# ViTAE-Transformer/MTP

Hardware: AMD Instinct MI355X
Metric: images/sec pretrain step (ViT-L+RVSA, 224^2, bf16) (higher is better)
Workload: dtype bf16; 1 GPU; ViT-L + RVSA backbone fwd+bwd + grad all-reduce + clip + AdamW, 224x224, batch 64 per GPU (BASELINE configs[2]/[3]); global_batch=64, parallelism=dp1, activation_checkpointing=False, heads=sum_i mean(f_i)

## Files before the change

### include/mtp_hip.h

```cpp
#ifndef MTP_HIP_H_
#define MTP_HIP_H_

#include <stddef.h>
#include <stdint.h>

#ifdef __cplusplus
extern "C" {
#endif

typedef void* mtp_stream_t;

typedef enum { MTP_F32 = 0, MTP_BF16 = 1, MTP_F64 = 2  } mtp_dtype;

enum { MTP_OK = 0, MTP_ERR_ARG = -1, MTP_ERR_UNSUPPORTED = -2 };

typedef enum {
    MTP_EPI_BIAS = 0,
    MTP_EPI_BIAS_GELU = 1,
    MTP_EPI_BIAS_RES = 2,
    MTP_EPI_DGELU = 3,
    MTP_EPI_BIAS_GELU_DG = 4,
    MTP_EPI_MUL = 5
} mtp_epilogue;

// ... 66 lines not shown
int mtp_preprocess_patchify(const uint8_t* img, void* cols, int dtype, int64_t B, int64_t H, int64_t W, int64_t P, int64_t pad_divisor,
                            const float* mean, const float* std, int bgr_to_rgb, float pad_value, mtp_stream_t stream);
int mtp_cast(const void* src, int src_dtype, void* dst, int dst_dtype, int64_t n, mtp_stream_t stream);
int mtp_transpose_cast(const float* src, void* dst, int dst_dtype, int64_t R, int64_t C, mtp_stream_t stream);
typedef struct {
    const float* src;
    void* w;
    void* wt;
    int64_t R, C;
    int64_t tile0;
    int32_t f32_out;
    float wd;
} mtp_wimg_desc;
int mtp_weight_images(const mtp_wimg_desc* descs_dev, int n, int64_t total_tiles, int act_dtype, mtp_stream_t stream);
int mtp_adamw_weight_images(const mtp_wimg_desc* descs_dev, int n, int64_t total_tiles, int act_dtype, float* p_base, const float* g_base, float* m_base, float* v_base,
                            const float* hyper, const float* sqnorm, float max_norm, float grad_scale, mtp_stream_t stream);
int mtp_adamw_weight_images_lr(const mtp_wimg_desc* descs_dev, const float* desc_lr, int n, int64_t total_tiles, int act_dtype, float* p_base, const float* g_base,
                               float* m_base, float* v_base, const float* hyper, const float* sqnorm, float max_norm, float grad_scale, mtp_stream_t stream);
int mtp_convt_pack(const float* w, void* wg, void* wgT, int dtype, int64_t Cin, int64_t Cout, mtp_stream_t stream);
int mtp_convt_unpack_grad(const float* dwg, float* dw, int64_t Cin, int64_t Cout, mtp_stream_t stream);
int mtp_tokens_to_nchw(const void* x, int x_dtype, void* out, int out_dtype, int64_t B, int64_t Hp, int64_t Wp, int64_t C, int levels, mtp_stream_t stream);
int mtp_nchw_to_tokens(const void* f, int f_dtype, void* out, int out_dtype, int64_t B, int64_t Hp, int64_t Wp, int64_t C, int levels, mtp_stream_t stream);
int mtp_maxpool2_tokens_fwd(const float* x, void* y, int y_dtype, int64_t B, int64_t Hp, int64_t Wp, int64_t C, mtp_stream_t stream);
int mtp_maxpool2_tokens_bwd(const float* x, const void* dy, int dy_dtype, float* dx, int accumulate, int64_t B, int64_t Hp, int64_t Wp, int64_t C, mtp_stream_t stream);
int mtp_axpy_f32(float* y, const float* x, float alpha, int64_t n, mtp_stream_t stream);
#define MTP_MAX_SEGMENTS 12
int mtp_copy_segments_f32(const float* const* src, float* const* dst, const int64_t* count, int n, mtp_stream_t stream);
int mtp_scale_rows_cast(const float* src, void* dst, int dst_dtype, const float* scale, int64_t rows_per_sample, int64_t rows, int64_t C, mtp_stream_t stream);

int mtp_im2col3x3(const void* x, int x_dtype, int64_t sN, int64_t sH, int64_t sW, int64_t sC, void* cols, int cols_dtype,
                  int64_t N, int64_t H, int64_t W, int64_t Cin, int64_t stride, int64_t Kp, mtp_stream_t stream);
int mtp_col2im3x3(const void* dcols, int cols_dtype, float* dx, int64_t sN, int64_t sH, int64_t sW, int64_t sC,
                  int64_t N, int64_t H, int64_t W, int64_t Cin, int64_t stride, int64_t Kp, int accumulate, mtp_stream_t stream);
int mtp_conv3x3_pack(const float* w, void* w2, void* w2t, int dtype, int64_t Cout, int64_t Cin, int64_t Kp, mtp_stream_t stream);
int mtp_conv3x3_unpack_grad(const float* dw2, float* dw, int64_t Cout, int64_t Cin, int64_t Kp, mtp_stream_t stream);
int mtp_pack_rows_padded(const float* w, void* wp, void* wpt, int dtype, int64_t R, int64_t C, int64_t Rp, mtp_stream_t stream);
int mtp_cast_pad_rows(const float* src, int64_t n, void* dst, int dst_dtype, int64_t ld, int64_t rows, mtp_stream_t stream);
int mtp_copy_rows(const void* src, int64_t src_ld, void* dst, int64_t dst_ld, int dtype, int64_t n, int64_t rows, mtp_stream_t stream);
int mtp_dwconv3x3_fwd(const void* x, const float* w, const float* bias, void* y, int dtype, int64_t N, int64_t H, int64_t W, int64_t C, mtp_stream_t stream);
int mtp_dwconv3x3_bwd_dx(const void* dy, int dtype, const float* w, float* dx, int accumulate, int64_t N, int64_t H, int64_t W, int64_t C, mtp_stream_t stream);
int64_t mtp_dwconv3x3_bwd_dw_partial_rows(int64_t N, int64_t H, int64_t W);
int mtp_dwconv3x3_bwd_dw(const void* dy, const void* x, int dtype, float* part, int64_t N, int64_t H, int64_t W, int64_t C, mtp_stream_t stream);
int mtp_dwconv_fwd(const void* x, const float* w, const float* bias, void* y, int dtype, int64_t N, int64_t H, int64_t W, int64_t C, int k, mtp_stream_t stream);
int mtp_dwconv_bwd_dx(const void* dy, int dtype, const float* w, float* dx, int accumulate, int64_t N, int64_t H, int64_t W, int64_t C, int k, mtp_stream_t stream);
int mtp_dwconv_bwd_dw(const void* dy, const void* x, int dtype, float* dw, float* db, int64_t N, int64_t H, int64_t W, int64_t C, int k, mtp_stream_t stream);
int mtp_center_feature_scale_fwd(const void* y, const void* xp, const void* logits, int64_t ld, void* out, int dtype, int64_t rows, int64_t G, int64_t GC, mtp_stream_t stream);
int mtp_center_feature_scale_bwd(const void* dout, const void* y, const void* xp, const void* logits, int64_t ld, void* dy, float* dxp, void* dlogits, int dtype, int64_t rows,
                                 int64_t G, int64_t GC, mtp_stream_t stream);
int mtp_softmax_groups_fwd(const void* logits, int64_t ld, void* prob, int dtype, int64_t rows, int64_t G, int64_t P, mtp_stream_t stream);
int mtp_softmax_groups_bwd(const void* prob, const float* dprob, void* dlogits, int64_t ld, int dtype, int64_t rows, int64_t G, int64_t P, mtp_stream_t stream);
int mtp_scale_residual_fwd(const float* x, const void* z, int dtype, const float* gamma, const float* sample_scale, int64_t rows_per_sample,
                           float* out, void* out_act, int64_t rows, int64_t C, mtp_stream_t stream);
int64_t mtp_scale_residual_bwd_partial_rows(int64_t rows);
int mtp_scale_residual_bwd(const float* dout, const void* z, int dtype, const float* gamma, const float* sample_scale, int64_t rows_per_sample,
                           void* dz, float* part, int64_t rows, int64_t C, mtp_stream_t stream);

int mtp_full_attn_fwd(const void* qkv, void* o, float* lse, int dtype, const float* rel_h, const float* rel_w,
                      int64_t B, int64_t Hp, int64_t Wp, int64_t heads, int64_t hd, float scale, mtp_stream_t stream);
int64_t mtp_full_attn_bwd_workspace_floats(int64_t B, int64_t Hp, int64_t Wp, int64_t heads);
int mtp_full_attn_bwd(const void* qkv, const void* o, const void* dout, const float* lse, void* dqkv, int dtype,
                      const float* rel_h, const float* rel_w, float* drel_part, float* workspace,
                      int64_t B, int64_t Hp, int64_t Wp, int64_t heads, int64_t hd, float scale, mtp_stream_t stream);

int mtp_rvsa_pool_fwd(const void* x, int dtype, float* avg, float* pooled, int64_t B, int64_t Hp, int64_t Wp, int64_t C, mtp_stream_t stream);
int mtp_rvsa_pool_bwd(const float* dpooled, const float* avg, void* dx, int dtype, int accumulate, int64_t B, int64_t Hp, int64_t Wp, int64_t C, mtp_stream_t stream);
int mtp_rvsa_sampling_fwd(const void* x, int dtype, const float* w, const float* bias, float* avg, float* pooled, float* samp,
                          int64_t B, int64_t Hp, int64_t Wp, int64_t C, int64_t N, mtp_stream_t stream);
int mtp_rvsa_sampling_bwd(const float* dsamp, const float* w, const float* avg, void* dx, int dtype,
                          int64_t B, int64_t Hp, int64_t Wp, int64_t C, int64_t N, mtp_stream_t stream);
int mtp_rvsa_sampling_bwd_win(const float* dsamp, const float* w, const float* avg, float* g, int64_t windows, int64_t C, int64_t N, mtp_stream_t stream);
int mtp_small_linear_fwd(const float* x, const float* w, const float* b, float* y, int64_t R, int64_t N, int64_t K, mtp_stream_t stream);
int mtp_small_linear_bwd(const float* x, const float* w, const float* dy, float* dx, float* dw, float* db, int64_t R, int64_t N, int64_t K, mtp_stream_t stream);
int mtp_small_linear_dw_segments(const float* x, const float* dy, int64_t R, int64_t N, int64_t K, int nseg, const int64_t* seg_rows,
                                 float* const* dw, float* const* db, mtp_stream_t stream);
int mtp_small_linear_dw_segments_batched(const float* const* xs, const float* const* dys, int count, int64_t R, int64_t N, int64_t K, int nseg,
                                         const int64_t* seg_rows, float* const* dw, float* const* db, mtp_stream_t stream);
int mtp_rvsa_attn_fwd(const void* qkv, const float* samp, void* o, float* lse, int dtype,
                      const float* rel_h, const float* rel_w, const float* bias_table,
                      int64_t B, int64_t Hp, int64_t Wp, int64_t heads, int64_t hd, float scale, mtp_stream_t stream);
int mtp_rvsa_attn_bwd(const void* qkv, const float* samp, const void* o, const void* dout, const float* lse,
                      void* dqkv, float* dkv_f32, float* dsamp, float* rel_part, float* tab_part, int dtype,
                      const float* rel_h, const float* rel_w, const float* bias_table,
                      int64_t B, int64_t Hp, int64_t Wp, int64_t heads, int64_t hd, float scale, mtp_stream_t stream);

int mtp_zero_segments_f32(float* base, const int64_t* start, const int64_t* count, int n, mtp_stream_t stream);
int mtp_sqnorm_f32(const float* g, float* out, int64_t n, mtp_stream_t stream);
int mtp_sqnorm_segments_f32(const float* base, const int64_t* start, const int64_t* count, int n, float* out, mtp_stream_t stream);
int mtp_adamw_flat(float* p, const float* g, float* m, float* v, int64_t n, const int64_t* seg_start, const float* seg_wd, int nseg,
                   const float* hyper, const float* sqnorm, float max_norm, float grad_scale, mtp_stream_t stream);
int mtp_adamw_flat_lr(float* p, const float* g, float* m, float* v, int64_t n, const int64_t* seg_start, const float* seg_wd, const float* seg_lr, int nseg,
                      const float* hyper, const float* sqnorm, float max_norm, float grad_scale, mtp_stream_t stream);

typedef struct {
    int64_t N, H, W;
    int kernel_h, kernel_w, stride_h, stride_w, pad_h, pad_w, dilation_h, dilation_w;
    int group, group_channels;
    float offset_scale;
    int im2col_step;
    int remove_center;
    int variant;
} mtp_dcnv3_geom;
int mtp_dcnv3_out_size(const mtp_dcnv3_geom* geom, int64_t* Ho, int64_t* Wo);
int mtp_dcnv3_fwd(const void* input, const void* offset, const void* mask, void* output, int dtype, const mtp_dcnv3_geom* geom, mtp_stream_t stream);
int mtp_dcnv3_bwd(const void* input, const void* offset, const void* mask, const void* grad_output, int dtype, float* grad_input, float* grad_offset,
                  float* grad_mask, const mtp_dcnv3_geom* geom, mtp_stream_t stream);
int mtp_dcnv3_bwd_act(const void* input, const void* offset, const void* mask, const void* grad_output, int dtype, float* grad_input, float* grad_offset,
                      float* grad_mask, void* grad_offset_act, int64_t act_ld, const mtp_dcnv3_geom* geom, mtp_stream_t stream);

const char* mtp_version(void);

int mtp_stream_create_low_priority(mtp_stream_t* stream);
int mtp_stream_create_cu_mask(const uint32_t* mask, int words, mtp_stream_t* stream);
int mtp_probe_placement(int32_t* out, int blocks, int64_t spin_clocks, mtp_stream_t stream);
int mtp_stream_destroy(mtp_stream_t stream);

int mtp_comm_unique_id(void* id128);
int mtp_comm_init(const void* id128, int rank, int world, void** comm);
int mtp_comm_allreduce_bucket(void* comm, float* bucket, int64_t count, mtp_stream_t stream);
int mtp_comm_allreduce_bucket_dt(void* comm, void* bucket, int64_t count, int dtype, mtp_stream_t stream);
int mtp_comm_reduce_scatter_bucket(void* comm, void* bucket, int64_t count_per_rank, int rank, int dtype, mtp_stream_t stream);
int mtp_comm_allgather_bucket(void* comm, void* bucket, int64_t count_per_rank, int rank, int dtype, mtp_stream_t stream);
int mtp_comm_info(void* comm, int* info4);
int mtp_comm_destroy(void* comm);

int64_t mtp_bn_partial_rows(int64_t rows);
int mtp_bn_stats(const void* x, int dtype, int64_t ldx, const float* center, float* part, float* sums, int64_t rows, int64_t C, mtp_stream_t stream);
int mtp_bn_finalize(const float* sums, const float* center, double count, float* running_mean, float* running_var, float momentum, float eps, float* mean, float* rstd,
                    int64_t C, mtp_stream_t stream);
int mtp_bn_apply(const void* x, int x_dtype, int64_t ldx, const float* mean, const float* rstd, const float* gamma, const float* beta, int relu,
                 void* y, int y_dtype, int64_t ldy, int64_t rows, int64_t C, mtp_stream_t stream);
int mtp_bn_bwd_stats(const void* dy, int dy_dtype, int64_t lddy, const void* x, int x_dtype, int64_t ldx, const float* mean, const float* rstd,
                     const float* gamma, const float* beta, int relu, float* part, float* sums, int64_t rows, int64_t C, mtp_stream_t stream);
int mtp_bn_bwd_dx(const void* dy, int dy_dtype, int64_t lddy, const void* x, int x_dtype, int64_t ldx, const float* mean, const float* rstd,
                  const float* gamma, const float* beta, int relu, const float* sums, double count, void* dx, int dx_dtype, int64_t lddx,
                  int64_t rows, int64_t C, mtp_stream_t stream);
int mtp_resize_bilinear_fwd(const void* x, int x_dtype, int64_t ldx, void* y, int y_dtype, int64_t ldy, int64_t N, int64_t Hi, int64_t Wi,
                            int64_t Ho, int64_t Wo, int64_t C, int accumulate, mtp_stream_t stream);
int mtp_resize_bilinear_bwd(const void* dy, int dy_dtype, int64_t lddy, float* dx, int64_t lddx, int64_t N, int64_t Hi, int64_t Wi, int64_t Ho,
                            int64_t Wo, int64_t C, int accumulate, mtp_stream_t stream);
int mtp_adaptive_avg_pool_fwd(const void* x, int x_dtype, int64_t ldx, void* y, int y_dtype, int64_t N, int64_t H, int64_t W, int64_t C,
                              int64_t S, mtp_stream_t stream);
int mtp_adaptive_avg_pool_bwd(const void* dy, int dy_dtype, float* dx, int64_t lddx, int64_t N, int64_t H, int64_t W, int64_t C, int64_t S,
                              int accumulate, mtp_stream_t stream);
int mtp_channel_scale(const void* x, int x_dtype, int64_t ldx, const float* mask, int64_t rows_per_sample, void* y, int y_dtype, int64_t ldy,
                      int64_t rows, int64_t C, mtp_stream_t stream);
int64_t mtp_seg_ce_workspace_bytes(int64_t N, int64_t H, int64_t W, int64_t K);
int mtp_seg_ce(const void* logits, int dtype, int64_t ld, int64_t N, int64_t h, int64_t w, int64_t K, const void* labels, int label_bytes, int64_t H,
               int64_t W, int ignore_index, float loss_weight, float* loss, float* dlogits, int64_t ldd, void* workspace, int64_t workspace_bytes,
               mtp_stream_t stream);

#ifdef __cplusplus
}
#endif
#endif
```

### mtp_amd/_lib.py

```python
import ctypes as C
import os

_HERE = os.path.dirname(os.path.abspath(__file__))
LIB_PATH = os.environ.get("MTP_HIP_LIB") or os.path.join(_HERE, "libmtp_hip.so")

MTP_F32, MTP_BF16, MTP_F64 = 0, 1, 2
EPI_BIAS, EPI_BIAS_GELU, EPI_BIAS_RES, EPI_DGELU, EPI_BIAS_GELU_DG, EPI_MUL = 0, 1, 2, 3, 4, 5

p, i64, i32, f32 = C.c_void_p, C.c_int64, C.c_int, C.c_float


class GemmArgs(C.Structure):
    _fields_ = [("A", p), ("B", p), ("C", p), ("M", i64), ("N", i64), ("K", i64),
                ("lda", i64), ("ldb", i64), ("ldc", i64),
                ("in_dtype", i32), ("out_dtype", i32), ("epilogue", i32),
                ("bias", p), ("bias_mod", i64), ("res", p), ("res_ld", i64), ("res_mod", i64),
                ("rowscale", p), ("rows_per_sample", i64), ("aux", p), ("aux_ld", i64),
                ("split_k", i32), ("variant", i32), ("colsum", p), ("defer_sum", i32), ("pad_", i32),
                ("workspace", p), ("workspace_bytes", i64)]


class WimgDesc(C.Structure):
    _fields_ = [("src", p), ("w", p), ("wt", p), ("R", i64), ("C", i64), ("tile0", i64), ("f32_out", C.c_int32), ("wd", C.c_float)]

# ... 5 lines not shown


SIGNATURES = {
    "mtp_weight_images": (i32, [p, i32, i64, i32, p]),
    "mtp_dwconv_fwd": (i32, [p, p, p, p, i32, i64, i64, i64, i64, i32, p]),
    "mtp_dwconv_bwd_dx": (i32, [p, i32, p, p, i32, i64, i64, i64, i64, i32, p]),
    "mtp_dwconv_bwd_dw": (i32, [p, p, i32, p, p, i64, i64, i64, i64, i32, p]),
    "mtp_center_feature_scale_fwd": (i32, [p, p, p, i64, p, i32, i64, i64, i64, p]),
    "mtp_center_feature_scale_bwd": (i32, [p, p, p, p, i64, p, p, p, i32, i64, i64, i64, p]),
    "mtp_dcnv3_out_size": (i32, [C.POINTER(Dcnv3Geom), C.POINTER(i64), C.POINTER(i64)]),
    "mtp_dcnv3_fwd": (i32, [p, p, p, p, i32, C.POINTER(Dcnv3Geom), p]),
    "mtp_dcnv3_bwd": (i32, [p, p, p, p, i32, p, p, p, C.POINTER(Dcnv3Geom), p]),
    "mtp_dcnv3_bwd_act": (i32, [p, p, p, p, i32, p, p, p, p, i64, C.POINTER(Dcnv3Geom), p]),
    "mtp_gemm_nt": (i32, [C.POINTER(GemmArgs), p]),
    "mtp_gemm_nt_tile": (i32, [C.POINTER(GemmArgs)]),
    "mtp_gemm_nt_workspace_bytes": (i64, []),
    "mtp_gemm_tn": (i32, [C.POINTER(GemmArgs), p]),
    "mtp_gemm_tn_grouped": (i32, [C.POINTER(GemmArgs), i32, p]),
    "mtp_sum_partials_batch": (i32, [p, p, p, p, i32, p]),
    "mtp_layernorm_fwd": (i32, [p, i32, p, p, p, i32, p, p, i64, i64, f32, i32, p]),
    "mtp_layernorm_bwd_partial_rows": (i64, [i64]),
    "mtp_layernorm_bwd": (i32, [p, i32, p, i32, p, p, p, p, i32, p, p, p, i32, p, i32, p, i64, p, p, i64, i64, i64, p]),
    "mtp_reduce_rows_f32": (i32, [p, i64, p, i64, i64, i32, p]),
    "mtp_reduce_rows_batched_f32": (i32, [p, p, i32, i64, i64, i64, i32, p]),
    "mtp_reduce_rows_t_f32": (i32, [p, i64, p, i64, i64, i64, i32, p]),
    "mtp_reduce_rows_t_batched_f32": (i32, [p, p, i32, i64, i64, i64, i64, i32, p]),
    "mtp_copy_segments_f32": (i32, [p, p, p, i32, p]),
    "mtp_colsum": (i32, [p, i32, i64, p, i64, i64, p]),
    "mtp_colsum_acc": (i32, [p, i32, i64, p, i64, i64, p]),
    "mtp_patchify": (i32, [p, p, i32, i64, i64, i64, i64, i64, p]),
    "mtp_preprocess_patchify": (i32, [p, p, i32, i64, i64, i64, i64, i64, C.POINTER(f32), C.POINTER(f32), i32, f32, p]),
    "mtp_unpatchify": (i32, [p, i32, p, i64, i64, i64, i64, i64, p]),
    "mtp_cast": (i32, [p, i32, p, i32, i64, p]),
    "mtp_transpose_cast": (i32, [p, p, i32, i64, i64, p]),
    "mtp_convt_pack": (i32, [p, p, p, i32, i64, i64, p]),
    "mtp_convt_unpack_grad": (i32, [p, p, i64, i64, p]),
    "mtp_tokens_to_nchw": (i32, [p, i32, p, i32, i64, i64, i64, i64, i32, p]),
    "mtp_nchw_to_tokens": (i32, [p, i32, p, i32, i64, i64, i64, i64, i32, p]),
    "mtp_maxpool2_tokens_fwd": (i32, [p, p, i32, i64, i64, i64, i64, p]),
    "mtp_maxpool2_tokens_bwd": (i32, [p, p, i32, p, i32, i64, i64, i64, i64, p]),
    "mtp_axpy_f32": (i32, [p, p, f32, i64, p]),
    "mtp_scale_rows_cast": (i32, [p, p, i32, p, i64, i64, i64, p]),
    "mtp_im2col3x3": (i32, [p, i32, i64, i64, i64, i64, p, i32, i64, i64, i64, i64, i64, i64, p]),
    "mtp_col2im3x3": (i32, [p, i32, p, i64, i64, i64, i64, i64, i64, i64, i64, i64, i64, i32, p]),
    "mtp_conv3x3_pack": (i32, [p, p, p, i32, i64, i64, i64, p]),
    "mtp_conv3x3_unpack_grad": (i32, [p, p, i64, i64, i64, p]),
    "mtp_pack_rows_padded": (i32, [p, p, p, i32, i64, i64, i64, p]),
    "mtp_cast_pad_rows": (i32, [p, i64, p, i32, i64, i64, p]),
    "mtp_copy_rows": (i32, [p, i64, p, i64, i32, i64, i64, p]),
    "mtp_dwconv3x3_fwd": (i32, [p, p, p, p, i32, i64, i64, i64, i64, p]),
    "mtp_dwconv3x3_bwd_dx": (i32, [p, i32, p, p, i32, i64, i64, i64, i64, p]),
    "mtp_dwconv3x3_bwd_dw_partial_rows": (i64, [i64, i64, i64]),
    "mtp_dwconv3x3_bwd_dw": (i32, [p, p, i32, p, i64, i64, i64, i64, p]),
    "mtp_softmax_groups_fwd": (i32, [p, i64, p, i32, i64, i64, i64, p]),
    "mtp_softmax_groups_bwd": (i32, [p, p, p, i64, i32, i64, i64, i64, p]),
    "mtp_scale_residual_fwd": (i32, [p, p, i32, p, p, i64, p, p, i64, i64, p]),
    "mtp_scale_residual_bwd_partial_rows": (i64, [i64]),
    "mtp_scale_residual_bwd": (i32, [p, p, i32, p, p, i64, p, p, i64, i64, p]),
    "mtp_comm_unique_id": (i32, [p]),
    "mtp_comm_init": (i32, [p, i32, i32, C.POINTER(C.c_void_p)]),
    "mtp_comm_allreduce_bucket": (i32, [p, p, i64, p]),
    "mtp_comm_allreduce_bucket_dt": (i32, [p, p, i64, i32, p]),
    "mtp_comm_reduce_scatter_bucket": (i32, [p, p, i64, i32, i32, p]),
    "mtp_comm_allgather_bucket": (i32, [p, p, i64, i32, i32, p]),
    "mtp_comm_info": (i32, [p, p]),
    "mtp_comm_destroy": (i32, [p]),
    "mtp_full_attn_fwd": (i32, [p, p, p, i32, p, p, i64, i64, i64, i64, i64, f32, p]),
    "mtp_full_attn_bwd_workspace_floats": (i64, [i64, i64, i64, i64]),
    "mtp_full_attn_bwd": (i32, [p, p, p, p, p, i32, p, p, p, p, i64, i64, i64, i64, i64, f32, p]),
    "mtp_rvsa_pool_fwd": (i32, [p, i32, p, p, i64, i64, i64, i64, p]),
    "mtp_rvsa_pool_bwd": (i32, [p, p, p, i32, i32, i64, i64, i64, i64, p]),
    "mtp_rvsa_sampling_fwd": (i32, [p, i32, p, p, p, p, p, i64, i64, i64, i64, i64, p]),
    "mtp_rvsa_sampling_bwd": (i32, [p, p, p, p, i32, i64, i64, i64, i64, i64, p]),
    "mtp_rvsa_sampling_bwd_win": (i32, [p, p, p, p, i64, i64, i64, p]),
    "mtp_layernorm_residual_fwd": (i32, [p, i32, p, p, p, p, p, i64, p, p, p, p, i64, i64, f32, p]),
    "mtp_layernorm_residual_bwd": (i32, [p, p, i32, p, p, p, p, p, p, i64, p, p, i64, i64, p]),
    "mtp_layernorm_bwd_win": (i32, [p, i32, p, i32, p, p, p, p, p, p, i32, p, i32, p, i64, p, p, i64, i64, i64, p, i64, i64, i64, p]),
    "mtp_small_linear_fwd": (i32, [p, p, p, p, i64, i64, i64, p]),
    "mtp_small_linear_bwd": (i32, [p, p, p, p, p, p, i64, i64, i64, p]),
    "mtp_small_linear_dw_segments": (i32, [p, p, i64, i64, i64, i32, p, p, p, p]),
    "mtp_small_linear_dw_segments_batched": (i32, [p, p, i32, i64, i64, i64, i32, p, p, p, p]),
    "mtp_rvsa_attn_fwd": (i32, [p, p, p, p, i32, p, p, p, i64, i64, i64, i64, i64, f32, p]),
    "mtp_rvsa_attn_bwd": (i32, [p, p, p, p, p, p, p, p, p, p, i32, p, p, p, i64, i64, i64, i64, i64, f32, p]),
    "mtp_zero_segments_f32": (i32, [p, p, p, i32, p]),
    "mtp_sqnorm_f32": (i32, [p, p, i64, p]),
    "mtp_sqnorm_segments_f32": (i32, [p, p, p, i32, p, p]),
    "mtp_adamw_flat": (i32, [p, p, p, p, i64, p, p, i32, p, p, f32, f32, p]),
    "mtp_adamw_weight_images": (i32, [p, i32, i64, i32, p, p, p, p, p, p, f32, f32, p]),
    "mtp_adamw_flat_lr": (i32, [p, p, p, p, i64, p, p, p, i32, p, p, f32, f32, p]),
    "mtp_adamw_weight_images_lr": (i32, [p, p, i32, i64, i32, p, p, p, p, p, p, f32, f32, p]),
    "mtp_bn_partial_rows": (i64, [i64]),
    "mtp_bn_stats": (i32, [p, i32, i64, p, p, p, i64, i64, p]),
    "mtp_bn_finalize": (i32, [p, p, C.c_double, p, p, f32, f32, p, p, i64, p]),
    "mtp_bn_apply": (i32, [p, i32, i64, p, p, p, p, i32, p, i32, i64, i64, i64, p]),
    "mtp_bn_bwd_stats": (i32, [p, i32, i64, p, i32, i64, p, p, p, p, i32, p, p, i64, i64, p]),
    "mtp_bn_bwd_dx": (i32, [p, i32, i64, p, i32, i64, p, p, p, p, i32, p, C.c_double, p, i32, i64, i64, i64, p]),
    "mtp_resize_bilinear_fwd": (i32, [p, i32, i64, p, i32, i64, i64, i64, i64, i64, i64, i64, i32, p]),
    "mtp_resize_bilinear_bwd": (i32, [p, i32, i64, p, i64, i64, i64, i64, i64, i64, i64, i32, p]),
    "mtp_adaptive_avg_pool_fwd": (i32, [p, i32, i64, p, i32, i64, i64, i64, i64, i64, p]),
    "mtp_adaptive_avg_pool_bwd": (i32, [p, i32, p, i64, i64, i64, i64, i64, i64, i32, p]),
    "mtp_channel_scale": (i32, [p, i32, i64, p, i64, p, i32, i64, i64, i64, p]),
    "mtp_seg_ce_workspace_bytes": (i64, [i64, i64, i64, i64]),
    "mtp_seg_ce": (i32, [p, i32, i64, i64, i64, i64, i64, p, i32, i64, i64, i32, f32, p, p, i64, p, i64, p]),
    "mtp_version": (C.c_char_p, []),
    "mtp_stream_create_low_priority": (i32, [p]),
    "mtp_stream_create_cu_mask": (i32, [p, i32, p]),
    "mtp_probe_placement": (i32, [p, i32, i64, p]),
    "mtp_stream_destroy": (i32, [p]),
}

_lib = None


class MtpHipError(RuntimeError):
    pass


def load():
    global _lib
    if _lib is not None:
        return _lib
    if not os.path.exists(LIB_PATH):
        raise MtpHipError("libmtp_hip.so not found at %s -- build it first (__graft_entry__.build() or make -C mtp_amd/csrc); "
                          "mtp_amd has no CPU/PyTorch fallback" % LIB_PATH)
    lib = C.CDLL(LIB_PATH)
    ab = bool(os.environ.get("MTP_HIP_LIB"))
    for name, (res, args) in SIGNATURES.items():
        if ab and not hasattr(lib, name):
            continue
        fn = getattr(lib, name)
        fn.restype = res
        fn.argtypes = args
    _lib = lib
    return lib


def check(rc, what):
    if rc != 0:
        kind = {-1: "invalid argument", -2: "unsupported configuration"}.get(rc, "hipError_t %d" % rc)
        raise MtpHipError("%s failed: %s" % (what, kind))
```

### mtp_amd/csrc/attn.hip

```cpp
#include <stdlib.h>

#include "attn_mfma.h"
#include "common.h"

namespace {

constexpr int HD = 64;
constexpr int KT = 32;

template <typename T>
__device__ __forceinline__ void load_row(const T* p, float (&r)[HD], float mul = 1.0f) {
#pragma unroll
    for (int i = 0; i < HD / 8; ++i) {
        float t[8];
        load8(p + 8 * i, t);
#pragma unroll
        for (int e = 0; e < 8; ++e) r[8 * i + e] = t[e] * mul;
    }
}
template <typename T>
__device__ __forceinline__ void store_row(T* p, const float (&r)[HD], float mul = 1.0f) {
#pragma unroll
    for (int i = 0; i < HD / 8; ++i) {
        float t[8];
// ... 804 lines not shown
        if (dtype == MTP_BF16) {
            (void)hipFuncSetAttribute((const void*)full_attn_bwdN_q_kernel<bf16_t>, hipFuncAttributeMaxDynamicSharedMemorySize, (int)lds_q);
            hipLaunchKernelGGL((full_attn_bwdN_q_kernel<bf16_t>), gq, block, lds_q, s, (const bf16_t*)qkv, (const bf16_t*)o, (const bf16_t*)dout, lse, (bf16_t*)dqkv,
                               rel_h, rel_w, workspace, N, (int)Hp, (int)Wp, (int)heads, scale);
            hipLaunchKernelGGL((full_attn_bwdN_t_kernel<bf16_t>), gt, block, 0, s, (const bf16_t*)qkv, (const float*)workspace, drel_part, N, (int)Hp, (int)Wp, (int)heads, scale);
            hipLaunchKernelGGL((full_attn_bwdN_k_kernel<bf16_t>), gq, block, lds_k, s, (const bf16_t*)qkv, (const bf16_t*)dout, lse, (bf16_t*)dqkv,
                               (const float*)workspace, N, (int)Hp, (int)Wp, (int)heads, scale);
        } else {
            (void)hipFuncSetAttribute((const void*)full_attn_bwdN_q_kernel<float>, hipFuncAttributeMaxDynamicSharedMemorySize, (int)lds_q);
            hipLaunchKernelGGL((full_attn_bwdN_q_kernel<float>), gq, block, lds_q, s, (const float*)qkv, (const float*)o, (const float*)dout, lse, (float*)dqkv,
                               rel_h, rel_w, workspace, N, (int)Hp, (int)Wp, (int)heads, scale);
            hipLaunchKernelGGL((full_attn_bwdN_t_kernel<float>), gt, block, 0, s, (const float*)qkv, (const float*)workspace, drel_part, N, (int)Hp, (int)Wp, (int)heads, scale);
            hipLaunchKernelGGL((full_attn_bwdN_k_kernel<float>), gq, block, lds_k, s, (const float*)qkv, (const float*)dout, lse, (float*)dqkv,
                               (const float*)workspace, N, (int)Hp, (int)Wp, (int)heads, scale);
        }
        return mtp_launch_status();
    }
    if ((2 * Hp - 1) + (2 * Wp - 1) > 4 * MAXR) return MTP_ERR_UNSUPPORTED;
    const size_t lds = sizeof(float) * (size_t)(2 * (Hp + Wp) * 256 + 512 + 2 * KT * HD);
    if (lds > 160 * 1024) return MTP_ERR_UNSUPPORTED;
    dim3 grid((unsigned)(B * heads)), block(256);
    hipStream_t s = (hipStream_t)stream;
    if (dtype == MTP_BF16) {
        (void)hipFuncSetAttribute((const void*)full_attn_bwd_kernel<bf16_t>, hipFuncAttributeMaxDynamicSharedMemorySize, (int)lds);
        hipLaunchKernelGGL((full_attn_bwd_kernel<bf16_t>), grid, block, lds, s, (const bf16_t*)qkv, (const bf16_t*)o, (const bf16_t*)dout, lse, (bf16_t*)dqkv,
                           rel_h, rel_w, drel_part, N, (int)Hp, (int)Wp, (int)heads, scale);
    } else {
        (void)hipFuncSetAttribute((const void*)full_attn_bwd_kernel<float>, hipFuncAttributeMaxDynamicSharedMemorySize, (int)lds);
        hipLaunchKernelGGL((full_attn_bwd_kernel<float>), grid, block, lds, s, (const float*)qkv, (const float*)o, (const float*)dout, lse, (float*)dqkv,
                           rel_h, rel_w, drel_part, N, (int)Hp, (int)Wp, (int)heads, scale);
    }
    return mtp_launch_status();
}

extern "C" int mtp_rvsa_attn_fwd(const void* qkv, const float* samp, void* o, float* lse, int dtype,
                                 const float* rel_h, const float* rel_w, const float* bias_table,
                                 int64_t B, int64_t Hp, int64_t Wp, int64_t heads, int64_t hd, float scale, mtp_stream_t stream) {
    if (!qkv || !samp || !o || !lse || !rel_h || !rel_w || !bias_table || B <= 0 || Hp < 7 || Wp < 7 || heads <= 0) return MTP_ERR_ARG;
    if (hd != HD) return MTP_ERR_UNSUPPORTED;
    const RvsaGeom g = make_geom(Hp, Wp, heads);
    dim3 grid((unsigned)(B * g.nh * g.nw * heads)), block(64);
    hipStream_t s = (hipStream_t)stream;
    if (dtype == MTP_BF16 && mtp_use_mfma_attn())
        return mtp_rvsa_fwd_mfma_launch(qkv, samp, o, lse, rel_h, rel_w, bias_table, B, Hp, Wp, heads, scale, s);
    if (dtype == MTP_BF16)
        hipLaunchKernelGGL((rvsa_attn_fwd_kernel<bf16_t>), grid, block, 0, s, (const bf16_t*)qkv, samp, (bf16_t*)o, lse, rel_h, rel_w, bias_table, g, scale);
    else
        hipLaunchKernelGGL((rvsa_attn_fwd_kernel<float>), grid, block, 0, s, (const float*)qkv, samp, (float*)o, lse, rel_h, rel_w, bias_table, g, scale);
    return mtp_launch_status();
}

extern "C" int mtp_rvsa_attn_bwd(const void* qkv, const float* samp, const void* o, const void* dout, const float* lse,
                                 void* dqkv, float* dkv_f32, float* dsamp, float* rel_part, float* tab_part, int dtype,
                                 const float* rel_h, const float* rel_w, const float* bias_table,
                                 int64_t B, int64_t Hp, int64_t Wp, int64_t heads, int64_t hd, float scale, mtp_stream_t stream) {
    if (!qkv || !samp || !o || !dout || !lse || !dqkv || !dkv_f32 || !dsamp || !rel_part || !tab_part || !rel_h || !rel_w || !bias_table) return MTP_ERR_ARG;
    if (B <= 0 || Hp < 7 || Wp < 7 || heads <= 0) return MTP_ERR_ARG;
    if (hd != HD) return MTP_ERR_UNSUPPORTED;
    const RvsaGeom g = make_geom(Hp, Wp, heads);
    const int64_t Ttok = B * Hp * Wp, C = heads * HD;
    hipStream_t s = (hipStream_t)stream;
    if (dtype == MTP_BF16 && mtp_use_mfma_attn() && mtp_rvsa_bwd_mfma_scatter_mode(Hp, Wp, heads) == 4)
        return mtp_rvsa_bwd_mfma_launch(qkv, samp, o, dout, lse, dqkv, dkv_f32, dsamp, rel_part, tab_part, rel_h, rel_w, bias_table, B, Hp, Wp, heads, scale, s);
    hipError_t e = hipMemsetAsync(dkv_f32, 0, sizeof(float) * (size_t)(Ttok * 2 * C), s);
    if (e != hipSuccess) return (int)e;
    dim3 grid((unsigned)(B * g.nh * g.nw * heads)), block(64);
    int64_t cb = (Ttok * 2 * C / 4 + 255) / 256;
    dim3 cgrid((unsigned)(cb > 8192 ? 8192 : cb)), cblock(256);
    if (dtype == MTP_BF16 && mtp_use_mfma_attn()) {
        const int rc = mtp_rvsa_bwd_mfma_launch(qkv, samp, o, dout, lse, dqkv, dkv_f32, dsamp, rel_part, tab_part, rel_h, rel_w, bias_table, B, Hp, Wp, heads, scale, s);
        if (rc) return rc;
        hipLaunchKernelGGL((dkv_convert_kernel<bf16_t>), cgrid, cblock, 0, s, dkv_f32, (bf16_t*)dqkv, Ttok, (int)C);
    } else if (dtype == MTP_BF16) {
        hipLaunchKernelGGL((rvsa_attn_bwd_kernel<bf16_t>), grid, block, 0, s, (const bf16_t*)qkv, samp, (const bf16_t*)o, (const bf16_t*)dout, lse, (bf16_t*)dqkv,
                           dkv_f32, dsamp, rel_part, tab_part, rel_h, rel_w, bias_table, g, scale);
        hipLaunchKernelGGL((dkv_convert_kernel<bf16_t>), cgrid, cblock, 0, s, dkv_f32, (bf16_t*)dqkv, Ttok, (int)C);
    } else {
        hipLaunchKernelGGL((rvsa_attn_bwd_kernel<float>), grid, block, 0, s, (const float*)qkv, samp, (const float*)o, (const float*)dout, lse, (float*)dqkv,
                           dkv_f32, dsamp, rel_part, tab_part, rel_h, rel_w, bias_table, g, scale);
        hipLaunchKernelGGL((dkv_convert_kernel<float>), cgrid, cblock, 0, s, dkv_f32, (float*)dqkv, Ttok, (int)C);
    }
    return mtp_launch_status();
}
```

### mtp_amd/csrc/attn_mfma.h

```cpp
#pragma once
#include <hip/hip_runtime.h>
#include <stdint.h>

int mtp_rvsa_fwd_mfma_launch(const void* qkv, const float* samp, void* o, float* lse, const float* rel_h, const float* rel_w, const float* bias_table,
                             int64_t B, int64_t Hp, int64_t Wp, int64_t heads, float scale, hipStream_t s);
int mtp_rvsa_bwd_mfma_launch(const void* qkv, const float* samp, const void* o, const void* dout, const float* lse, void* dqkv, float* dkv, float* dsamp,
                             float* rel_part, float* tab_part, const float* rel_h, const float* rel_w, const float* bias_table,
                             int64_t B, int64_t Hp, int64_t Wp, int64_t heads, float scale, hipStream_t s);
int mtp_rvsa_bwd_mfma_scatter_mode(int64_t Hp, int64_t Wp, int64_t heads);
int mtp_full_fwd_mfma_launch(const void* qkv, void* o, float* lse, const float* rel_h, const float* rel_w,
                             int64_t B, int64_t Hp, int64_t Wp, int64_t heads, float scale, hipStream_t s);
int mtp_full_bwd_mfma_launch(const void* qkv, const void* o, const void* dout, const float* lse, void* dqkv, const float* rel_h, const float* rel_w,
                             float* drel_part, int64_t B, int64_t Hp, int64_t Wp, int64_t heads, float scale, hipStream_t s);
bool mtp_full_v3_fits(int64_t Hp, int64_t Wp);
int mtp_full_v3_fwd_launch(const void* qkv, void* o, float* lse, const float* rel_h, const float* rel_w, int64_t B, int64_t Hp, int64_t Wp, int64_t heads,
                           float scale, hipStream_t s);
int mtp_full_v3_bwd_launch(const void* qkv, const void* o, const void* dout, const float* lse, void* dqkv, const float* rel_h, const float* rel_w,
                           float* drel_part, int64_t B, int64_t Hp, int64_t Wp, int64_t heads, float scale, hipStream_t s);
int mtp_full_bwd_flash_launch(const void* qkv, const void* o, const void* dout, const float* lse, void* dqkv, const float* rel_h, const float* rel_w,
                              float* drel_part, float* workspace, int64_t B, int64_t Hp, int64_t Wp, int64_t heads, float scale, hipStream_t s);

static inline bool mtp_use_mfma_attn() { return true; }
```

### mtp_amd/csrc/attn_rvsa_bwd4.hip

```cpp
#include <stdlib.h>

#include "attn_mfma.h"
#include "common.h"

namespace {

constexpr int HD = 64;
typedef __attribute__((ext_vector_type(2))) __bf16 bf16x2v_t;
constexpr int TP = 136;

struct RvsaGeom {
    int Hp, Wp, He, We, pad_t, pad_l, nh, nw, heads;
    float inv_div_x, inv_div_y;
};
struct Sample {
    float fx, fy;
    int x0, y0;
    float rx, ry, cs, sn, relx, rely;
};

__device__ __forceinline__ Sample make_sample(const RvsaGeom& g, const float* __restrict__ sp, int h, int wi, int wj, int a, int bb) {
    Sample s;
    const int H = g.heads;
    const float offx = sp[2 * h] * g.inv_div_x, offy = sp[2 * h + 1] * g.inv_div_y;
// ... 866 lines not shown
                v3 += (-dgx * sn + dgy * cs) * smp[9 * 64 + kc];
                v4 += dgx * (-rx * sn - ry * cs) + dgy * (-ry * sn + rx * cs);
            }
        }
    }
    v0 = wave_sum(v0); v1 = wave_sum(v1); v2 = wave_sum(v2); v3 = wave_sum(v3); v4 = wave_sum(v4);
    if (lane == 0) {
        vsum[8 * wave + 0] = v0; vsum[8 * wave + 1] = v1; vsum[8 * wave + 2] = v2; vsum[8 * wave + 3] = v3; vsum[8 * wave + 4] = v4;
    }
    __syncthreads();
    if (tid < 5) {
        float* dp = dsamp + (int64_t)bw * 5 * H;
        const float sum = (vsum[tid] + vsum[8 + tid]) + (vsum[16 + tid] + vsum[24 + tid]);
        dp[tid < 2 ? 2 * h + tid : tid < 4 ? 2 * H + 2 * h + (tid - 2) : 4 * H + h] = sum;
    }
    if constexpr (dense_scatter != 4) {
        const char* dKt = R2;
        const char* dVt = R2 + 64 * TP;
        float kx[16], ky[16];
#pragma unroll
        for (int kk = 0; kk < 2; ++kk)
#pragma unroll
            for (int e4 = 0; e4 < 2; ++e4) {
                const int k0 = 32 * kk + 8 * gq + 4 * e4;
                const float4 fxv = *reinterpret_cast<const float4*>(smp + 0 * 64 + k0), fyv = *reinterpret_cast<const float4*>(smp + 1 * 64 + k0);
                const float4 x0v = *reinterpret_cast<const float4*>(smp + 2 * 64 + k0), y0v = *reinterpret_cast<const float4*>(smp + 3 * 64 + k0);
                const int i = 8 * kk + 4 * e4;
                kx[i] = (float)__float_as_int(x0v.x) + fxv.x; kx[i + 1] = (float)__float_as_int(x0v.y) + fxv.y;
                kx[i + 2] = (float)__float_as_int(x0v.z) + fxv.z; kx[i + 3] = (float)__float_as_int(x0v.w) + fxv.w;
                ky[i] = (float)__float_as_int(y0v.x) + fyv.x; ky[i + 1] = (float)__float_as_int(y0v.y) + fyv.y;
                ky[i + 2] = (float)__float_as_int(y0v.z) + fyv.z; ky[i + 3] = (float)__float_as_int(y0v.w) + fyv.w;
            }
        const float iy = (float)__float_as_int(smp[3 * 64 + lane]) + smp[1 * 64 + lane];
        const float ymin = -wave_max(lane < 49 ? -iy : -1e30f), ymax = wave_max(lane < 49 ? iy : -1e30f);
        const int ty_lo = min(max((int)floorf(ymin) - g.pad_t, 0), g.Hp - 1), ty_hi = min(max((int)floorf(ymax) + 1 - g.pad_t, 0), g.Hp - 1);
        const int t_lo = __builtin_amdgcn_readfirstlane((ty_lo * g.Wp) >> 4), t_hi = __builtin_amdgcn_readfirstlane(((ty_hi + 1) * g.Wp - 1) >> 4);
        uint4 bk[4][2], bv[4][2];
#pragma unroll
        for (int dt = 0; dt < 4; ++dt)
#pragma unroll
            for (int kk = 0; kk < 2; ++kk) {
                const int o = (16 * dt + fr) * TP + (32 * kk + 8 * gq) * 2;
                bk[dt][kk] = ld8x2(dKt + o, dKt + o + 8);
                bv[dt][kk] = ld8x2(dVt + o, dVt + o + 8);
            }
        for (int ti = t_lo + wave; ti <= t_hi; ti += 4) {
            const int tok = 16 * ti + fr, tyy = tok / g.Wp, txx = tok - tyy * g.Wp;
            const float X = (float)(txx + g.pad_l), Y = (float)(tyy + g.pad_t);
            const float live = tok < N ? 1.f : 0.f;
            uint4 af[2];
#pragma unroll
            for (int kk = 0; kk < 2; ++kk) {
                float w[8];
#pragma unroll
                for (int e = 0; e < 8; ++e)
                    w[e] = live * fmaxf(0.f, 1.f - fabsf(kx[8 * kk + e] - X)) * fmaxf(0.f, 1.f - fabsf(ky[8 * kk + e] - Y));
                af[kk] = pack_bf16x8(w[0], w[1], w[2], w[3], w[4], w[5], w[6], w[7]);
            }
#pragma unroll
            for (int dt = 0; dt < 4; ++dt) {
                f32x4_t ak = {0.f, 0.f, 0.f, 0.f}, av = {0.f, 0.f, 0.f, 0.f};
#pragma unroll
                for (int kk = 0; kk < 2; ++kk) {
                    ak = mma(af[kk], bk[dt][kk], ak);
                    av = mma(af[kk], bv[dt][kk], av);
                }
#pragma unroll
                for (int r = 0; r < 4; ++r) {
                    const int t2 = 16 * ti + 4 * gq + r;
                    if (t2 < N) {
                        float* drow = dkv + ((int64_t)b * N + t2) * (2 * C) + h * HD + 16 * dt + fr;
                        if (ak[r] != 0.f) atomicAdd(drow, ak[r]);
                        if (av[r] != 0.f) atomicAdd(drow + C, av[r]);
                    }
                }
            }
        }
    }
}

constexpr int SCB = 224;

__global__ __launch_bounds__(256, 2) void rvsa_scatter_gemm_kernel(const bf16_t* __restrict__ dsel, const float* __restrict__ samp, bf16_t* __restrict__ dqkv,
                                                                  RvsaGeom g) {
    __shared__ __attribute__((aligned(16))) char Kimg[SCB * 128];
    __shared__ __attribute__((aligned(16))) char Vimg[SCB * 128];
    __shared__ __attribute__((aligned(16))) float xs[SCB];
    __shared__ __attribute__((aligned(16))) float ys[SCB];
    const int tid = threadIdx.x, lane = tid & 63, wave = tid >> 6, fr = lane & 15, gq = lane >> 4;
    const int H = g.heads, nW = g.nh * g.nw, S = nW * 49;
    const int h = blockIdx.x % H, b = blockIdx.x / H;
    const int C = H * HD, N = g.Hp * g.Wp;
    const int t0 = blockIdx.y * SCB, nt = (N - t0) < SCB ? (N - t0) : SCB;
    const int64_t ld = 3 * (int64_t)C;
    float X[4], Y[4], live[4];
    f32x4_t dk[4][4], dv[4][4];
#pragma unroll
    for (int i = 0; i < 4; ++i) {
        const int tl = 16 * (wave + 4 * i) + fr;
        const int tc = t0 + (tl < nt ? tl : nt - 1);
        const int ty = tc / g.Wp, tx = tc - ty * g.Wp;
        X[i] = (float)(tx + g.pad_l);
        Y[i] = (float)(ty + g.pad_t);
        live[i] = tl < nt ? 1.f : 0.f;
#pragma unroll
        for (int dt = 0; dt < 4; ++dt) {
            dk[i][dt] = f32x4_t{0.f, 0.f, 0.f, 0.f};
            dv[i][dt] = f32x4_t{0.f, 0.f, 0.f, 0.f};
        }
    }
    const int ntile = (nt + 15) / 16;
    const float ylo = (float)(t0 / g.Wp + g.pad_t) - 1.0f, yhi = (float)((t0 + nt - 1) / g.Wp + g.pad_t) + 1.0f;
    for (int c0 = 0; c0 < S; c0 += SCB) {
        __syncthreads();
        int hit = 0;
        if (tid < SCB) {
            const int sg = c0 + tid;
            float x = -1.0e4f, y = -1.0e4f;
            if (sg < S) {
                const int w = sg / 49, k = sg - 49 * w;
                const Sample sa = make_sample(g, samp + (int64_t)(b * nW + w) * 5 * H, h, w / g.nw, w % g.nw, k / 7, k % 7);
                x = (float)sa.x0 + sa.fx;
                y = (float)sa.y0 + sa.fy;
            }
            xs[tid] = x;
            ys[tid] = y;
            hit = (y > ylo && y < yhi) ? 1 : 0;
        }
        if (!__syncthreads_or(hit)) continue;
#pragma unroll
        for (int half = 0; half < 2; ++half) {
            constexpr int IT = 4;
            uint4 kv[IT], vv[IT];
#pragma unroll
            for (int i = 0; i < IT; ++i) {
                const int idx = tid + 256 * (IT * half + i), sl = idx >> 3, ch = idx & 7, sg = c0 + sl;
                const int sc = sg < S ? sg : S - 1;
                const int w = sc / 49, k = sc - 49 * w;
                const bf16_t* src = dsel + ((int64_t)(b * nW + w) * H + h) * (2 * 49 * HD) + k * HD + 8 * ch;
                kv[i] = ldg16(src);
                vv[i] = ldg16(src + 49 * HD);
            }
#pragma unroll
            for (int i = 0; i < IT; ++i) {
                const int idx = tid + 256 * (IT * half + i), sl = idx >> 3, ch = idx & 7, sg = c0 + sl;
                if (idx < SCB * 8) {
                    const bool ok = sg < S;
                    *reinterpret_cast<uint4*>(Kimg + swz(sl, ch)) = ok ? kv[i] : make_uint4(0u, 0u, 0u, 0u);
                    *reinterpret_cast<uint4*>(Vimg + swz(sl, ch)) = ok ? vv[i] : make_uint4(0u, 0u, 0u, 0u);
                }
            }
        }
        __syncthreads();
        for (int kk = 0; kk < SCB / 32; ++kk) {
            const int s0 = 32 * kk + 4 * gq;
            const float4 xa = *reinterpret_cast<const float4*>(xs + s0), xb = *reinterpret_cast<const float4*>(xs + s0 + 16);
            const float4 ya = *reinterpret_cast<const float4*>(ys + s0), yb = *reinterpret_cast<const float4*>(ys + s0 + 16);
            const float sx[8] = {xa.x, xa.y, xa.z, xa.w, xb.x, xb.y, xb.z, xb.w}, sy[8] = {ya.x, ya.y, ya.z, ya.w, yb.x, yb.y, yb.z, yb.w};
            uint4 kf[4], vf[4];
#pragma unroll
            for (int dt = 0; dt < 4; ++dt) {
                kf[dt] = rows_frag_tr(Kimg, s0, dt, fr);
                vf[dt] = rows_frag_tr(Vimg, s0, dt, fr);
            }
#pragma unroll
            for (int i = 0; i < 4; ++i) {
                if (wave + 4 * i < ntile) {
                    float w[8];
#pragma unroll
                    for (int e = 0; e < 8; ++e) w[e] = live[i] * fmaxf(0.f, 1.f - fabsf(sx[e] - X[i])) * fmaxf(0.f, 1.f - fabsf(sy[e] - Y[i]));
                    const uint4 wf = pack_bf16x8(w[0], w[1], w[2], w[3], w[4], w[5], w[6], w[7]);
#pragma unroll
                    for (int dt = 0; dt < 4; ++dt) {
                        dk[i][dt] = mma(kf[dt], wf, dk[i][dt]);
                        dv[i][dt] = mma(vf[dt], wf, dv[i][dt]);
                    }
                }
            }
        }
    }
    __syncthreads();
#pragma unroll
    for (int i = 0; i < 4; ++i) {
        const int tl = 16 * (wave + 4 * i) + fr;
        if (tl < nt) {
#pragma unroll
            for (int dt = 0; dt < 4; ++dt) {
                const int o = tl * 128 + (((2 * dt + (gq >> 1)) ^ (tl & 7)) << 4) + (gq & 1) * 8;
                *reinterpret_cast<uint2*>(Kimg + o) = make_uint2(pack_bf16x2(dk[i][dt][0], dk[i][dt][1]), pack_bf16x2(dk[i][dt][2], dk[i][dt][3]));
                *reinterpret_cast<uint2*>(Vimg + o) = make_uint2(pack_bf16x2(dv[i][dt][0], dv[i][dt][1]), pack_bf16x2(dv[i][dt][2], dv[i][dt][3]));
            }
        }
    }
    __syncthreads();
    for (int idx = tid; idx < nt * 16; idx += 256) {
        const int tl = idx >> 4, m = (idx >> 3) & 1, ch = idx & 7;
        const uint4 v = *reinterpret_cast<const uint4*>((m ? Vimg : Kimg) + swz(tl, ch));
        *reinterpret_cast<uint4*>(dqkv + ((int64_t)b * N + t0 + tl) * ld + (1 + m) * C + h * HD + 8 * ch) = v;
    }
}

RvsaGeom make_geom(int64_t Hp, int64_t Wp, int64_t heads) {
    RvsaGeom g;
    const int pad_h = (int)((7 - Hp % 7) % 7), pad_w = (int)((7 - Wp % 7) % 7);
    g.Hp = (int)Hp; g.Wp = (int)Wp;
    g.pad_t = pad_h / 2; g.pad_l = pad_w / 2;
    g.He = (int)Hp + pad_h; g.We = (int)Wp + pad_w;
    g.nh = g.He / 7; g.nw = g.We / 7;
    g.heads = (int)heads;
    g.inv_div_x = 1.0f / (float)(Hp / 7);
    g.inv_div_y = 1.0f / (float)(Wp / 7);
    return g;
}

}

int mtp_rvsa_bwd_mfma_scatter_mode(int64_t Hp, int64_t Wp, int64_t heads) {
    static const bool dense = []() { const char* e = getenv("MTP_RVSA_SCATTER"); return e && e[0] == 'd'; }();
    if (dense) return 1;
    const RvsaGeom g = make_geom(Hp, Wp, heads);
    const int64_t N = Hp * Wp, nW = (int64_t)g.nh * g.nw;
    const bool fits = Hp <= 64 && Wp <= 64 && nW * (2 * 49 * HD * 2) <= N * 2 * HD * 4;
    return fits ? 4 : 1;
}

int mtp_rvsa_bwd_mfma_launch(const void* qkv, const float* samp, const void* o, const void* dout, const float* lse, void* dqkv, float* dkv, float* dsamp,
                             float* rel_part, float* tab_part, const float* rel_h, const float* rel_w, const float* bias_table,
                             int64_t B, int64_t Hp, int64_t Wp, int64_t heads, float scale, hipStream_t s) {
    const RvsaGeom g = make_geom(Hp, Wp, heads);
    const int mode = mtp_rvsa_bwd_mfma_scatter_mode(Hp, Wp, heads);
    const dim3 grid((unsigned)(B * g.nh * g.nw * heads));
    if (mode == 4) {
        static const bool old4 = []() { const char* e = getenv("MTP_RVSA_BWD"); return e && e[0] == '4'; }();
        if (old4)
            hipLaunchKernelGGL(rvsa_bwd4_mfma_kernel<4>, grid, dim3(256), 0, s, (const bf16_t*)qkv, samp, (const bf16_t*)o, (const bf16_t*)dout, lse,
                               (bf16_t*)dqkv, dkv, dsamp, rel_part, tab_part, rel_h, rel_w, bias_table, g, scale);
        else
            hipLaunchKernelGGL(rvsa_bwd5_mfma_kernel, grid, dim3(256), 0, s, (const bf16_t*)qkv, samp, (const bf16_t*)o, (const bf16_t*)dout, lse,
                               (bf16_t*)dqkv, dkv, dsamp, rel_part, tab_part, rel_h, rel_w, bias_table, g, scale);
        const int64_t N = Hp * Wp;
        hipLaunchKernelGGL(rvsa_scatter_gemm_kernel, dim3((unsigned)(B * heads), (unsigned)((N + SCB - 1) / SCB)), dim3(256), 0, s, (const bf16_t*)dkv, samp, (bf16_t*)dqkv, g);
    } else {
        hipLaunchKernelGGL(rvsa_bwd4_mfma_kernel<1>, grid, dim3(256), 0, s, (const bf16_t*)qkv, samp, (const bf16_t*)o, (const bf16_t*)dout, lse,
                           (bf16_t*)dqkv, dkv, dsamp, rel_part, tab_part, rel_h, rel_w, bias_table, g, scale);
    }
    return mtp_launch_status();
}
```

### mtp_amd/csrc/common.h

```cpp
#pragma once
#include <hip/hip_runtime.h>
#include <stdint.h>

#include "../../include/mtp_hip.h"

#define MTP_WAVE 64

typedef __attribute__((ext_vector_type(8))) __bf16 bf16x8_t;
typedef __attribute__((ext_vector_type(4))) float f32x4_t;

struct bf16_t {
    uint16_t bits;
};

__device__ __forceinline__ float bf16_bits_to_f32(uint32_t b) { return __uint_as_float(b << 16); }
__device__ __forceinline__ uint32_t f32_to_bf16_bits(float f) {
    uint32_t u = __float_as_uint(f);
    if ((u & 0x7fffffffu) > 0x7f800000u) return (u >> 16) | 0x40u;
    return (u + 0x7fffu + ((u >> 16) & 1u)) >> 16;
}
typedef __attribute__((ext_vector_type(2))) __bf16 bf16x2_t;
typedef __attribute__((ext_vector_type(2))) float f32x2_t;
__device__ __forceinline__ uint32_t pack_bf16x2(float lo, float hi) {
    f32x2_t v = {lo, hi};
    return __builtin_bit_cast(uint32_t, __builtin_convertvector(v, bf16x2_t));
}
__device__ __forceinline__ uint4 pack_bf16x8(float a, float b, float c, float d, float e, float f, float g, float h) {
    return make_uint4(pack_bf16x2(a, b), pack_bf16x2(c, d), pack_bf16x2(e, f), pack_bf16x2(g, h));
}

template <typename T>
struct Elem;
template <>
struct Elem<float> {
    static constexpr int kPerChunk = 4;
    static constexpr int kDtype = MTP_F32;
    __device__ static __forceinline__ float load(const float* p) { return *p; }
    __device__ static __forceinline__ void store(float* p, float v) { *p = v; }
};
template <>
struct Elem<bf16_t> {
    static constexpr int kPerChunk = 8;
    static constexpr int kDtype = MTP_BF16;
    __device__ static __forceinline__ float load(const bf16_t* p) { return bf16_bits_to_f32(p->bits); }
    __device__ static __forceinline__ void store(bf16_t* p, float v) { p->bits = (uint16_t)f32_to_bf16_bits(v); }
};

__device__ __forceinline__ float4 load4(const float* p) { return *reinterpret_cast<const float4*>(p); }
__device__ __forceinline__ float4 load4(const bf16_t* p) {
    uint2 v = *reinterpret_cast<const uint2*>(p);
    return make_float4(bf16_bits_to_f32(v.x & 0xffffu), bf16_bits_to_f32(v.x >> 16), bf16_bits_to_f32(v.y & 0xffffu), bf16_bits_to_f32(v.y >> 16));
}
__device__ __forceinline__ void store4(float* p, float4 v) { *reinterpret_cast<float4*>(p) = v; }
__device__ __forceinline__ void store4(bf16_t* p, float4 v) {
    *reinterpret_cast<uint2*>(p) = make_uint2(pack_bf16x2(v.x, v.y), pack_bf16x2(v.z, v.w));
}
__device__ __forceinline__ void load8(const float* p, float (&o)[8]) {
    float4 a = load4(p), b = load4(p + 4);
    o[0] = a.x; o[1] = a.y; o[2] = a.z; o[3] = a.w; o[4] = b.x; o[5] = b.y; o[6] = b.z; o[7] = b.w;
}
__device__ __forceinline__ void load8(const bf16_t* p, float (&o)[8]) {
    uint4 v = *reinterpret_cast<const uint4*>(p);
    o[0] = bf16_bits_to_f32(v.x & 0xffffu); o[1] = bf16_bits_to_f32(v.x >> 16);
    o[2] = bf16_bits_to_f32(v.y & 0xffffu); o[3] = bf16_bits_to_f32(v.y >> 16);
    o[4] = bf16_bits_to_f32(v.z & 0xffffu); o[5] = bf16_bits_to_f32(v.z >> 16);
    o[6] = bf16_bits_to_f32(v.w & 0xffffu); o[7] = bf16_bits_to_f32(v.w >> 16);
}
__device__ __forceinline__ void store8(float* p, const float (&o)[8]) {
    store4(p, make_float4(o[0], o[1], o[2], o[3]));
    store4(p + 4, make_float4(o[4], o[5], o[6], o[7]));
}
__device__ __forceinline__ void store8(bf16_t* p, const float (&o)[8]) {
    *reinterpret_cast<uint4*>(p) = make_uint4(pack_bf16x2(o[0], o[1]), pack_bf16x2(o[2], o[3]), pack_bf16x2(o[4], o[5]), pack_bf16x2(o[6], o[7]));
}

__device__ __forceinline__ uint4 ldg16(const void* p) {
#if defined(__HIP_DEVICE_COMPILE__)
    typedef __attribute__((ext_vector_type(4))) unsigned int u32x4_t;
    const u32x4_t v = *(const __attribute__((address_space(1))) u32x4_t*)(uintptr_t)p;
    return make_uint4(v[0], v[1], v[2], v[3]);
#else
    return *reinterpret_cast<const uint4*>(p);
#endif
}

__device__ __forceinline__ uint4 ldg16_at(const void* base, uint32_t byte_off) {
#if defined(__HIP_DEVICE_COMPILE__)
    typedef __attribute__((ext_vector_type(4))) unsigned int u32x4_t;
    const u32x4_t v = *(const __attribute__((address_space(1))) u32x4_t*)((uintptr_t)base + (uintptr_t)byte_off);
    return make_uint4(v[0], v[1], v[2], v[3]);
#else
    return *reinterpret_cast<const uint4*>(reinterpret_cast<const char*>(base) + byte_off);
#endif
}

__device__ __forceinline__ float erf_as(float z, float& e) {
    const float az = fabsf(z);
    const float t = __builtin_amdgcn_rcpf(1.0f + 0.3275911f * az);
    const float y = ((((1.061405429f * t - 1.453152027f) * t + 1.421413741f) * t - 0.284496736f) * t + 0.254829592f) * t;
    e = __builtin_amdgcn_exp2f(-1.4426950408889634f * az * az);
    return copysignf(1.0f - y * e, z);
}
__device__ __forceinline__ float gelu_f(float x) {
    float e;
    return 0.5f * x * (1.0f + erf_as(x * 0.70710678118654752440f, e));
}
__device__ __forceinline__ void gelu_pair_f(float x, float& g, float& dg) {
    float e;
    const float cdf = 0.5f * (1.0f + erf_as(x * 0.70710678118654752440f, e));
    g = x * cdf;
    dg = cdf + x * 0.39894228040143267794f * e;
}
__device__ __forceinline__ float dgelu_f(float x) {
    float e;
    const float er = erf_as(x * 0.70710678118654752440f, e);
    return 0.5f * (1.0f + er) + x * 0.39894228040143267794f * e;
}

template <int CTRL>
__device__ __forceinline__ float dpp_mov(float v) {
    return __int_as_float(__builtin_amdgcn_update_dpp(0, __float_as_int(v), CTRL, 0xF, 0xF, true));
}
template <int M>
__device__ __forceinline__ float lane_xor(float v) {
    static_assert(M == 1 || M == 2 || M == 4 || M == 8, "in-row partners only");
    if constexpr (M == 1) return dpp_mov<0xB1>(v);
    else if constexpr (M == 2) return dpp_mov<0x4E>(v);
    else if constexpr (M == 4) return dpp_mov<0x1B>(dpp_mov<0x141>(v));
    else return dpp_mov<0x141>(dpp_mov<0x140>(v));
}
__device__ __forceinline__ float xor16_sum(float v) {
    const auto r = __builtin_amdgcn_permlane16_swap(__float_as_uint(v), __float_as_uint(v), false, false);
    return __uint_as_float(r[0]) + __uint_as_float(r[1]);
}
__device__ __forceinline__ float xor32_sum(float v) {
    const auto r = __builtin_amdgcn_permlane32_swap(__float_as_uint(v), __float_as_uint(v), false, false);
    return __uint_as_float(r[0]) + __uint_as_float(r[1]);
}
__device__ __forceinline__ float xor16_max(float v) {
    const auto r = __builtin_amdgcn_permlane16_swap(__float_as_uint(v), __float_as_uint(v), false, false);
    return fmaxf(__uint_as_float(r[0]), __uint_as_float(r[1]));
}
__device__ __forceinline__ float xor32_max(float v) {
    const auto r = __builtin_amdgcn_permlane32_swap(__float_as_uint(v), __float_as_uint(v), false, false);
    return fmaxf(__uint_as_float(r[0]), __uint_as_float(r[1]));
}
__device__ __forceinline__ float rows_sum(float v) { return xor32_sum(xor16_sum(v)); }
__device__ __forceinline__ float rows_max(float v) { return xor32_max(xor16_max(v)); }
__device__ __forceinline__ float wave_sum(float v) {
    v = xor32_sum(v); v = xor16_sum(v);
    v += lane_xor<8>(v); v += lane_xor<4>(v); v += lane_xor<2>(v); v += lane_xor<1>(v);
    return v;
}
__device__ __forceinline__ float wave_max(float v) {
    v = xor32_max(v); v = xor16_max(v);
    v = fmaxf(v, lane_xor<8>(v)); v = fmaxf(v, lane_xor<4>(v)); v = fmaxf(v, lane_xor<2>(v)); v = fmaxf(v, lane_xor<1>(v));
    return v;
}
// ... 23 lines not shown
```

### mtp_amd/csrc/elementwise.hip

```cpp
#include "common.h"
#include <atomic>
#include <mutex>

namespace {

inline unsigned blocks_for(int64_t n, int per_block, int64_t cap = 1 << 20) {
    int64_t b = (n + per_block - 1) / per_block;
    return (unsigned)(b < 1 ? 1 : (b > cap ? cap : b));
}

template <typename T, bool INVERSE>
__global__ __launch_bounds__(256) void patchify_kernel(float* __restrict__ img, T* __restrict__ cols, int B, int Cin, int H, int W, int P, int Hp, int Wp) {
    const int K4 = Cin * P * P / 4, P4 = P / 4;
    const int64_t total = (int64_t)B * Hp * Wp * K4;
    for (int64_t i = (int64_t)blockIdx.x * 256 + threadIdx.x; i < total; i += (int64_t)gridDim.x * 256) {
        const int k4 = (int)(i % K4);
        const int64_t t = i / K4;
        const int kx4 = k4 % P4, ky = (k4 / P4) % P, c = k4 / (P4 * P);
        const int px = (int)(t % Wp), py = (int)((t / Wp) % Hp), b = (int)(t / ((int64_t)Wp * Hp));
        float* ip = img + (((int64_t)b * Cin + c) * H + py * P + ky) * W + px * P + kx4 * 4;
        T* cp = cols + t * (K4 * 4) + k4 * 4;
        if (INVERSE)
            *reinterpret_cast<float4*>(ip) = load4(cp);
        else
// ... 1051 lines not shown
        *reinterpret_cast<float4*>(pl + 4 * c4) = p;
    }
    __syncthreads();
    const int nper = ((N + (int)gridDim.y - 1) / (int)gridDim.y + 3) / 4 * 4, nlo = (int)blockIdx.y * nper, nhi = (nlo + nper) < N ? (nlo + nper) : N;
    for (int n0 = nlo + 4 * wave; n0 < nhi; n0 += 16) {
        float acc[4] = {0.f, 0.f, 0.f, 0.f};
        for (int k0 = lane * 4; k0 < C; k0 += 1024) {
            float4 ww[4][4], a[4];
#pragma unroll
            for (int kk = 0; kk < 4; ++kk) {
                const int k = k0 + 256 * kk, kc = k < C ? k : 0;
                a[kk] = k < C ? *reinterpret_cast<const float4*>(pl + kc) : make_float4(0.f, 0.f, 0.f, 0.f);
#pragma unroll
                for (int q = 0; q < 4; ++q) {
                    const int n = n0 + q < N ? n0 + q : N - 1;
                    ww[kk][q] = load4(w + (int64_t)n * C + kc);
                }
            }
#pragma unroll
            for (int kk = 0; kk < 4; ++kk)
#pragma unroll
                for (int q = 0; q < 4; ++q) acc[q] += a[kk].x * ww[kk][q].x + a[kk].y * ww[kk][q].y + a[kk].z * ww[kk][q].z + a[kk].w * ww[kk][q].w;
        }
#pragma unroll
        for (int q = 0; q < 4; ++q) {
            const float t = wave_sum(acc[q]);
            if (lane == 0 && n0 + q < nhi) samp[(int64_t)win * N + n0 + q] = t + (bias ? bias[n0 + q] : 0.f);
        }
    }
}

template <typename T>
__global__ __launch_bounds__(256) void rvsa_sampling_bwd_kernel(const float* __restrict__ dsamp, const float* __restrict__ w, const float* __restrict__ avg,
                                                               T* __restrict__ dx, int Hp, int Wp, int C, int N, int pad_t, int pad_l, int nh, int nw) {
    extern __shared__ __attribute__((aligned(16))) float ds[];
    __shared__ float4 part[4][64];
    const int win = blockIdx.x;
    const int j = win % nw, i = (win / nw) % nh, b = win / (nw * nh);
    const int lane = threadIdx.x & 63, q = threadIdx.x >> 6;
    const int c4 = blockIdx.y * 64 + lane;
    const bool live = c4 < C / 4;
    for (int n = threadIdx.x; n < N; n += 256) ds[n] = dsamp[(int64_t)win * N + n];
    __syncthreads();
    const int nq = (N + 3) / 4, n0 = q * nq, n1 = (n0 + nq) < N ? (n0 + nq) : N;
    float4 d = make_float4(0, 0, 0, 0);
    if (live) {
#pragma unroll 4
        for (int n = n0; n < n1; ++n) {
            const float4 ww = load4(w + (int64_t)n * C + 4 * c4);
            const float t = ds[n];
            d.x += t * ww.x; d.y += t * ww.y; d.z += t * ww.z; d.w += t * ww.w;
        }
    }
    part[q][lane] = d;
    __syncthreads();
    if (!live) return;
    const float4 p0 = part[0][lane], p1 = part[1][lane], p2 = part[2][lane], p3 = part[3][lane];
    d = make_float4((p0.x + p1.x) + (p2.x + p3.x), (p0.y + p1.y) + (p2.y + p3.y), (p0.z + p1.z) + (p2.z + p3.z), (p0.w + p1.w) + (p2.w + p3.w));
    const float4 a = load4(avg + (int64_t)win * C + 4 * c4);
    const float k = 1.0f / 49.0f;
    const float4 g = make_float4(d.x * (a.x > 0 ? k : 0.01f * k), d.y * (a.y > 0 ? k : 0.01f * k), d.z * (a.z > 0 ? k : 0.01f * k), d.w * (a.w > 0 ? k : 0.01f * k));
#pragma unroll 1
    for (int aa = q; aa < 7; aa += 4) {
        const int y = i * 7 + aa - pad_t;
        if (y < 0 || y >= Hp) continue;
        float4 o[7];
#pragma unroll
        for (int bb = 0; bb < 7; ++bb) {
            const int xx = j * 7 + bb - pad_l;
            const int xc = (xx >= 0 && xx < Wp) ? xx : 0;
            o[bb] = load4(dx + (((int64_t)b * Hp + y) * Wp + xc) * C + 4 * c4);
        }
#pragma unroll
        for (int bb = 0; bb < 7; ++bb) {
            const int xx = j * 7 + bb - pad_l;
            if (xx >= 0 && xx < Wp)
                store4(dx + (((int64_t)b * Hp + y) * Wp + xx) * C + 4 * c4, make_float4(o[bb].x + g.x, o[bb].y + g.y, o[bb].z + g.z, o[bb].w + g.w));
        }
    }
}

__global__ __launch_bounds__(256) void rvsa_sampling_bwd_win_kernel(const float* __restrict__ dsamp, const float* __restrict__ w, const float* __restrict__ avg,
                                                                   float* __restrict__ g, int C, int N) {
    extern __shared__ __attribute__((aligned(16))) float ds[];
    __shared__ float4 part[4][64];
    const int win = blockIdx.x;
    const int lane = threadIdx.x & 63, q = threadIdx.x >> 6;
    const int c4 = blockIdx.y * 64 + lane;
    const bool live = c4 < C / 4;
    for (int n = threadIdx.x; n < N; n += 256) ds[n] = dsamp[(int64_t)win * N + n];
    __syncthreads();
    const int nq = (N + 3) / 4, n0 = q * nq, n1 = (n0 + nq) < N ? (n0 + nq) : N;
    float4 d = make_float4(0, 0, 0, 0);
    if (live) {
#pragma unroll 10
        for (int n = n0; n < n1; ++n) {
            const float4 ww = load4(w + (int64_t)n * C + 4 * c4);
            const float t = ds[n];
            d.x += t * ww.x; d.y += t * ww.y; d.z += t * ww.z; d.w += t * ww.w;
        }
    }
    part[q][lane] = d;
    __syncthreads();
    if (!live || q) return;
    const float4 p0 = part[0][lane], p1 = part[1][lane], p2 = part[2][lane], p3 = part[3][lane];
    d = make_float4((p0.x + p1.x) + (p2.x + p3.x), (p0.y + p1.y) + (p2.y + p3.y), (p0.z + p1.z) + (p2.z + p3.z), (p0.w + p1.w) + (p2.w + p3.w));
    const float4 a = load4(avg + (int64_t)win * C + 4 * c4);
    const float k = 1.0f / 49.0f;
    *reinterpret_cast<float4*>(g + (int64_t)win * C + 4 * c4) =
        make_float4(d.x * (a.x > 0 ? k : 0.01f * k), d.y * (a.y > 0 ? k : 0.01f * k), d.z * (a.z > 0 ? k : 0.01f * k), d.w * (a.w > 0 ? k : 0.01f * k));
}

extern "C" int mtp_rvsa_sampling_bwd_win(const float* dsamp, const float* w, const float* avg, float* g, int64_t windows, int64_t C, int64_t N, mtp_stream_t stream) {
    if (!dsamp || !w || !avg || !g || windows <= 0 || C <= 0 || (C % 4) || N <= 0 || N > 4096) return MTP_ERR_ARG;
    const dim3 grid((unsigned)windows, (unsigned)((C / 4 + 63) / 64)), block(256);
    hipLaunchKernelGGL(rvsa_sampling_bwd_win_kernel, grid, block, sizeof(float) * (size_t)N, (hipStream_t)stream, dsamp, w, avg, g, (int)C, (int)N);
    return mtp_launch_status();
}

extern "C" int mtp_rvsa_sampling_fwd(const void* x, int dtype, const float* w, const float* bias, float* avg, float* pooled, float* samp,
                                     int64_t B, int64_t Hp, int64_t Wp, int64_t C, int64_t N, mtp_stream_t stream) {
    if (!x || !w || !avg || !pooled || !samp || B <= 0 || Hp <= 0 || Wp <= 0 || C <= 0 || (C % 4) || C > 8192 || N <= 0) return MTP_ERR_ARG;
    int pt, pl, nh, nw;
    rvsa_geom(Hp, Wp, pt, pl, nh, nw);
    constexpr int ysplit = 2;
    const dim3 grid((unsigned)(B * nh * nw), (unsigned)(N >= 16 * ysplit ? ysplit : 1)), block(256);
    const size_t lds = sizeof(float) * (size_t)C;
    if (dtype == MTP_BF16)
        hipLaunchKernelGGL((rvsa_sampling_fwd_kernel<bf16_t>), grid, block, lds, (hipStream_t)stream, (const bf16_t*)x, w, bias, avg, pooled, samp, (int)Hp, (int)Wp, (int)C, (int)N, pt, pl, nh, nw);
    else if (dtype == MTP_F32)
        hipLaunchKernelGGL((rvsa_sampling_fwd_kernel<float>), grid, block, lds, (hipStream_t)stream, (const float*)x, w, bias, avg, pooled, samp, (int)Hp, (int)Wp, (int)C, (int)N, pt, pl, nh, nw);
    else return MTP_ERR_UNSUPPORTED;
    return mtp_launch_status();
}
extern "C" int mtp_rvsa_sampling_bwd(const float* dsamp, const float* w, const float* avg, void* dx, int dtype,
                                     int64_t B, int64_t Hp, int64_t Wp, int64_t C, int64_t N, mtp_stream_t stream) {
    if (!dsamp || !w || !avg || !dx || B <= 0 || Hp <= 0 || Wp <= 0 || C <= 0 || (C % 4) || N <= 0 || N > 4096) return MTP_ERR_ARG;
    int pt, pl, nh, nw;
    rvsa_geom(Hp, Wp, pt, pl, nh, nw);
    const dim3 grid((unsigned)(B * nh * nw), (unsigned)((C / 4 + 63) / 64)), block(256);
    const size_t lds = sizeof(float) * (size_t)N;
    if (dtype == MTP_BF16)
        hipLaunchKernelGGL((rvsa_sampling_bwd_kernel<bf16_t>), grid, block, lds, (hipStream_t)stream, dsamp, w, avg, (bf16_t*)dx, (int)Hp, (int)Wp, (int)C, (int)N, pt, pl, nh, nw);
    else if (dtype == MTP_F32)
        hipLaunchKernelGGL((rvsa_sampling_bwd_kernel<float>), grid, block, lds, (hipStream_t)stream, dsamp, w, avg, (float*)dx, (int)Hp, (int)Wp, (int)C, (int)N, pt, pl, nh, nw);
    else return MTP_ERR_UNSUPPORTED;
    return mtp_launch_status();
}

extern "C" int mtp_rvsa_pool_fwd(const void* x, int dtype, float* avg, float* pooled, int64_t B, int64_t Hp, int64_t Wp, int64_t C, mtp_stream_t stream) {
    if (!x || !avg || !pooled || B <= 0 || (C % 4)) return MTP_ERR_ARG;
    int pt, pl, nh, nw;
    rvsa_geom(Hp, Wp, pt, pl, nh, nw);
    dim3 grid((unsigned)(B * nh * nw), (unsigned)((C / 4 + 255) / 256)), block(256);
    if (dtype == MTP_BF16)
        hipLaunchKernelGGL((rvsa_pool_fwd_kernel<bf16_t>), grid, block, 0, (hipStream_t)stream, (const bf16_t*)x, avg, pooled, (int)Hp, (int)Wp, (int)C, pt, pl, nh, nw);
    else
        hipLaunchKernelGGL((rvsa_pool_fwd_kernel<float>), grid, block, 0, (hipStream_t)stream, (const float*)x, avg, pooled, (int)Hp, (int)Wp, (int)C, pt, pl, nh, nw);
    return mtp_launch_status();
}
extern "C" int mtp_rvsa_pool_bwd(const float* dpooled, const float* avg, void* dx, int dtype, int accumulate, int64_t B, int64_t Hp, int64_t Wp, int64_t C, mtp_stream_t stream) {
    if (!dpooled || !avg || !dx || B <= 0 || (C % 4)) return MTP_ERR_ARG;
    int pt, pl, nh, nw;
    rvsa_geom(Hp, Wp, pt, pl, nh, nw);
    dim3 grid(blocks_for(B * Hp * Wp * C / 4, 256, 8192)), block(256);
    if (dtype == MTP_BF16)
        hipLaunchKernelGGL((rvsa_pool_bwd_kernel<bf16_t>), grid, block, 0, (hipStream_t)stream, dpooled, avg, (bf16_t*)dx, accumulate, (int)B, (int)Hp, (int)Wp, (int)C, pt, pl, nh, nw);
    else
        hipLaunchKernelGGL((rvsa_pool_bwd_kernel<float>), grid, block, 0, (hipStream_t)stream, dpooled, avg, (float*)dx, accumulate, (int)B, (int)Hp, (int)Wp, (int)C, pt, pl, nh, nw);
    return mtp_launch_status();
}

extern "C" int mtp_small_linear_fwd(const float* x, const float* w, const float* b, float* y, int64_t R, int64_t N, int64_t K, mtp_stream_t stream) {
    if (!x || !w || !y || R <= 0 || N <= 0 || (K % 4)) return MTP_ERR_ARG;
    if (K <= 1024)
        hipLaunchKernelGGL((small_linear_fwd_kernel<4, 4>), dim3((unsigned)((R + 3) / 4)), dim3(256), 0, (hipStream_t)stream, x, w, b, y, (int)R, (int)N, (int)K);
    else if (K <= 2048)
        hipLaunchKernelGGL((small_linear_fwd_kernel<2, 8>), dim3((unsigned)((R + 1) / 2)), dim3(256), 0, (hipStream_t)stream, x, w, b, y, (int)R, (int)N, (int)K);
    else
        hipLaunchKernelGGL(small_linear_fwd_generic_kernel, dim3((unsigned)R), dim3(256), 0, (hipStream_t)stream, x, w, b, y, (int)N, (int)K);
    return mtp_launch_status();
}
extern "C" int mtp_small_linear_bwd(const float* x, const float* w, const float* dy, float* dx, float* dw, float* db, int64_t R, int64_t N, int64_t K, mtp_stream_t stream) {
    if (!x || !w || !dy || R <= 0 || N <= 0 || (K % 4)) return MTP_ERR_ARG;
    hipStream_t s = (hipStream_t)stream;
    if (dx) hipLaunchKernelGGL(small_linear_dx_kernel, dim3((unsigned)((K + 1023) / 1024), (unsigned)((R + 3) / 4)), dim3(256), 0, s, dy, w, dx, (int)R, (int)N, (int)K);
    if (dw) {
        if (db == dw + N * K) {
            (void)hipMemsetAsync(dw, 0, sizeof(float) * (size_t)(N * K + N), s);
        } else {
            (void)hipMemsetAsync(dw, 0, sizeof(float) * (size_t)(N * K), s);
            if (db) (void)hipMemsetAsync(db, 0, sizeof(float) * (size_t)N, s);
        }
        hipLaunchKernelGGL(small_linear_dw_kernel<false>, dim3((unsigned)((K + 255) / 256), (unsigned)((N + 7) / 8), (unsigned)((R + 4 * SL_DW_ROWS - 1) / (4 * SL_DW_ROWS))), dim3(256), 0, s,
                           dy, x, dw, db, (int)R, (int)N, (int)K, SlSegs{});
    }
    return mtp_launch_status();
}
extern "C" int mtp_small_linear_dw_segments(const float* x, const float* dy, int64_t R, int64_t N, int64_t K, int nseg, const int64_t* seg_rows,
// ... 223 lines not shown
```

### mtp_amd/csrc/gemm.hip

```cpp
#include "gemm_common.h"

namespace {

constexpr int BM = 128;
constexpr int BN = 128;
constexpr int NT_THREADS = 256;
constexpr int ROW_BYTES = 128;
constexpr int OPER_BYTES = BM * ROW_BYTES;
constexpr int STAGE_BYTES = 2 * OPER_BYTES;
constexpr int LDS_BYTES = 2 * STAGE_BYTES;

__device__ __forceinline__ int lds_off(int row, int chunk) { return row * ROW_BYTES + ((chunk ^ (row & 7)) << 4); }

__global__ __launch_bounds__(256) void sum_partials_kernel(const float* __restrict__ part, float* __restrict__ out, int64_t n4, int split) {
    for (int64_t i = (int64_t)blockIdx.x * 256 + threadIdx.x; i < n4; i += (int64_t)gridDim.x * 256) {
        float4 s = *reinterpret_cast<const float4*>(part + 4 * i);
        for (int z = 1; z < split; ++z) {
            const float4 v = *reinterpret_cast<const float4*>(part + 4 * (i + (int64_t)z * n4));
            s.x += v.x; s.y += v.y; s.z += v.z; s.w += v.w;
        }
        *reinterpret_cast<float4*>(out + 4 * i) = s;
    }
}

// ... 387 lines not shown
        const char* ga = p.A + (t * p.lda + ca) * 2;
        const char* gb = p.B + (t * p.ldb + cb) * 2;
        __builtin_amdgcn_global_load_lds((const __attribute__((address_space(1))) void*)ga,
                                         (__attribute__((address_space(3))) void*)(sA + rbase * TR_ROW_BYTES), 16, 0, 0);
        __builtin_amdgcn_global_load_lds((const __attribute__((address_space(1))) void*)gb,
                                         (__attribute__((address_space(3))) void*)(sB + rbase * TR_ROW_BYTES), 16, 0, 0);
    }
}

__device__ __forceinline__ uint4 tr_frag(const char* s, int off) {
    const tr_v4s lo = __builtin_amdgcn_ds_read_tr16_b64_v4i16((__attribute__((address_space(3))) tr_v4s*)(s + off));
    const tr_v4s hi = __builtin_amdgcn_ds_read_tr16_b64_v4i16((__attribute__((address_space(3))) tr_v4s*)(s + off + 4 * TR_ROW_BYTES));
    const uint2 l = __builtin_bit_cast(uint2, lo), h = __builtin_bit_cast(uint2, hi);
    return make_uint4(l.x, l.y, h.x, h.y);
}

__device__ __forceinline__ void compute_stage_tr(const char* sA, const char* sB, f32x4_t (&acc)[4][4], int wm, int wn, int lane) {
    const int i = lane & 15, g = lane >> 4;
    const int f = (i >> 2) | ((g & 1) << 2);
    const int rowoff = (8 * g + (i >> 2)) * TR_ROW_BYTES + ((i >> 1) & 1) * 16 + (i & 1) * 8;
#pragma unroll
    for (int ks = 0; ks < 2; ++ks) {
        uint4 a[4], b[4];
#pragma unroll
        for (int q = 0; q < 4; ++q) {
            a[q] = tr_frag(sA, rowoff + (((q | (wm << 2)) ^ f) << 5) + ks * 32 * TR_ROW_BYTES);
            b[q] = tr_frag(sB, rowoff + (((q | (wn << 2)) ^ f) << 5) + ks * 32 * TR_ROW_BYTES);
        }
#pragma unroll
        for (int ni = 0; ni < 4; ++ni)
#pragma unroll
            for (int mi = 0; mi < 4; ++mi) Mma<bf16_t>::run(acc[ni][mi], b[ni], a[mi]);
    }
}

__global__ __launch_bounds__(NT_THREADS) __attribute__((amdgpu_waves_per_eu(4, 4))) void gemm_tn_tr_kernel(KArgs p) {
    extern __shared__ __attribute__((aligned(16))) char smem[];
    const int tid = threadIdx.x, lane = tid & 63, wave = __builtin_amdgcn_readfirstlane(tid >> 6);
    const int wm = wave >> 1, wn = wave & 1;
    const int tile = (p.order & 1) ? (int)blockIdx.x : xcd_remap(blockIdx.x, gridDim.x);
    const int tiles_m = (int)gridDim.x / p.tiles_n;
    const int m0 = ((p.order & 2) ? tile % tiles_m : tile / p.tiles_n) * BM, n0 = ((p.order & 2) ? tile / tiles_m : tile % p.tiles_n) * BN;
    const int kt0 = blockIdx.y * p.k_tiles_per_split;
    int kt1 = kt0 + p.k_tiles_per_split;
    kt1 = kt1 < p.k_tiles ? kt1 : p.k_tiles;
    if (kt0 >= kt1) return;
    p.C += (int64_t)blockIdx.y * p.split_stride * (int64_t)sizeof(float);
    f32x4_t acc[4][4];
#pragma unroll
    for (int i = 0; i < 4; ++i)
#pragma unroll
        for (int j = 0; j < 4; ++j) acc[i][j] = f32x4_t{0.f, 0.f, 0.f, 0.f};
    const bool do_colsum = p.colsum != nullptr && n0 == 0;
    float cs[8] = {0.f, 0.f, 0.f, 0.f, 0.f, 0.f, 0.f, 0.f};
    for (int kt = kt0; kt < kt1; ++kt) {
        stage_tn_glds(p, smem, smem + OPER_BYTES, m0, n0, kt, wave, lane);
        asm volatile("s_waitcnt vmcnt(0)" ::: "memory");
        __syncthreads();
        compute_stage_tr(smem, smem + OPER_BYTES, acc, wm, wn, lane);
        if (do_colsum) {
#pragma unroll
            for (int j = 0; j < 4; ++j) {
                const uint4 v = *reinterpret_cast<const uint4*>(smem + ((tid >> 4) + 16 * j) * TR_ROW_BYTES + (tid & 15) * 16);
                const uint32_t w[4] = {v.x, v.y, v.z, v.w};
#pragma unroll
                for (int e = 0; e < 4; ++e) {
                    cs[2 * e] += __uint_as_float(w[e] << 16);
                    cs[2 * e + 1] += __uint_as_float(w[e] & 0xffff0000u);
                }
            }
        }
        __syncthreads();
    }
    if (do_colsum) {
        float* red = reinterpret_cast<float*>(smem);
        const int rg = tid >> 4, f = (rg & 3) | ((rg >> 1) & 4), chunk = (tid & 15) ^ (f << 1);
        *reinterpret_cast<float4*>(red + rg * BM + chunk * 8) = make_float4(cs[0], cs[1], cs[2], cs[3]);
        *reinterpret_cast<float4*>(red + rg * BM + chunk * 8 + 4) = make_float4(cs[4], cs[5], cs[6], cs[7]);
        __syncthreads();
        if (tid < BM) {
            float s = 0.f;
#pragma unroll
            for (int r = 0; r < 16; ++r) s += red[r * BM + tid];
            if (m0 + tid < p.M) atomicAdd(p.colsum + m0 + tid, s);
        }
    }
    epilogue<float, MTP_EPI_BIAS, 4>(p, acc, m0 + wm * 64, n0 + wn * 64, lane);
}

template <typename T>
int fill_common(const mtp_gemm_args* a, KArgs& k) {
    constexpr int E = Elem<T>::kPerChunk;
    if (!a->A || !a->B || !a->C || a->M <= 0 || a->N <= 0 || a->K <= 0) return MTP_ERR_ARG;
    if (a->M > INT32_MAX || a->N > INT32_MAX || a->K > INT32_MAX) return MTP_ERR_ARG;
    if ((a->lda % E) || (a->ldb % E) || (a->ldc % 4) || (a->N % 4)) return MTP_ERR_ARG;
    if (((uintptr_t)a->A | (uintptr_t)a->B | (uintptr_t)a->C) & 15) return MTP_ERR_ARG;
    k.A = (const char*)a->A; k.B = (const char*)a->B; k.C = (char*)a->C;
    k.M = (int)a->M; k.N = (int)a->N; k.K = (int)a->K;
    k.lda = a->lda; k.ldb = a->ldb; k.ldc = a->ldc;
    k.bias = a->bias; k.bias_mod = (int)a->bias_mod;
    k.res = a->res; k.res_ld = a->res_ld; k.res_mod = (int)a->res_mod;
    k.rowscale = a->rowscale; k.rows_per_sample = (int)(a->rows_per_sample > 0 ? a->rows_per_sample : 1);
    k.aux = (char*)a->aux; k.aux_ld = a->aux_ld;
    k.tiles_n = (int)((a->N + BN - 1) / BN);
    k.k_tiles = (int)((a->K + 8 * E - 1) / (8 * E));
    k.k_tiles_per_split = k.k_tiles;
    k.atomic_out = 0;
    k.order = (a->variant >> 1) & 3;
    k.split_stride = 0;
    k.colsum = nullptr;
    return 0;
}

int nt_p8_mode(const mtp_gemm_args* a, const KArgs& k, int cus) {
    if (a->in_dtype != MTP_BF16 || (a->variant & 1024) || !mtp_nt_p8_fits(k, a->out_dtype, a->epilogue)) return 0;
    const int forced = (a->variant >> 8) & 3;
    if (forced) return forced;
    const int64_t tiles = ((a->M + 255) / 256) * ((a->N + 255) / 256) * 256 / cus;
    return (tiles >= 72 || (tiles >= 40 && a->K >= 1536)) ? 1 : 0;
}

int nt_s8_mode(const mtp_gemm_args* a, const KArgs& k, int cus) {
    if (a->in_dtype != MTP_BF16 || (a->variant & (1024 | (1 << 18))) || ((a->variant >> 8) & 3) || !mtp_nt_s8_fits(k, a->out_dtype, a->epilogue)) return 0;
    if (a->variant & (1 << 17)) return 1;
    const int64_t tiles = ((a->M + 255) / 256) * ((a->N + 255) / 256) * 256 / cus;
    return tiles >= 40 && tiles <= 128;
}

template <typename T, typename Tout, int EPI>
int launch_nt(const mtp_gemm_args* a, hipStream_t stream) {
    constexpr int E = Elem<T>::kPerChunk;
    KArgs k;
    int rc = fill_common<T>(a, k);
    if (rc) return rc;
    if (a->K % E) return MTP_ERR_ARG;
    if (EPI == MTP_EPI_BIAS_RES && (!a->res || (a->res_ld % 4))) return MTP_ERR_ARG;
    if ((EPI == MTP_EPI_BIAS_GELU || EPI == MTP_EPI_DGELU || EPI == MTP_EPI_BIAS_GELU_DG || EPI == MTP_EPI_MUL) && (!a->aux || (a->aux_ld % 4))) return MTP_ERR_ARG;
    if (a->bias && a->bias_mod > 0 && (a->bias_mod % 4)) return MTP_ERR_ARG;
    if constexpr (sizeof(T) == 2) {
        const int cus = mtp_stream_cus(stream);
        if (nt_s8_mode(a, k, cus)) return mtp_nt_s8_launch(k, a->out_dtype, EPI, ((((a->variant >> 1) & 3) == 1) ? 2 : 0), stream);
        const int p8 = nt_p8_mode(a, k, cus);
        if (p8) return mtp_nt_p8_launch(k, a->out_dtype, EPI, (p8 == 2 ? 1 : p8 == 3 ? 4 : 0) | ((((a->variant >> 1) & 3) == 1) ? 2 : 0) | (((a->variant >> 15) & 3) << 8) | (((a->variant >> 20) & 3) << 13), stream);
    }
    const int tiles_m = (k.M + BM - 1) / BM;
    dim3 grid(tiles_m * k.tiles_n), block(NT_THREADS);
    const bool glds = ((a->variant & 1) == 0) && (a->K % (8 * E) == 0);
    const int ord = (a->variant >> 1) & 3;
    k.order = ord == 0 ? (k.tiles_n > 8 ? 2 : 0) : ord == 1 ? 1 : ord == 2 ? 2 : 0;
    if (!glds) k.order = ord;
    const int tiles_m8 = (k.M + NT8_BM - 1) / NT8_BM;
    const bool one_round = tiles_m8 * k.tiles_n >= 256 && tiles_m8 * k.tiles_n <= 512;
    if (glds && ((a->variant & 32) || (one_round && !(a->variant & 64)))) {
        if (ord == 0) k.order = k.tiles_n > 8 ? 2 : 0;
        hipLaunchKernelGGL((gemm_nt_sb8_kernel<T, Tout, EPI>), dim3(tiles_m8 * k.tiles_n), dim3(NT8_THREADS), NT8_STAGE_BYTES, stream, k);
        return mtp_launch_status();
    }
    if (glds)
        hipLaunchKernelGGL((gemm_nt_sb_kernel<T, Tout, EPI>), grid, block, STAGE_BYTES, stream, k);
    else
        hipLaunchKernelGGL((gemm_nt_kernel<T, Tout, EPI, false>), grid, block, LDS_BYTES, stream, k);
    return mtp_launch_status();
}

template <typename T>
int launch_tn(const mtp_gemm_args* a, hipStream_t stream) {
    constexpr int E = Elem<T>::kPerChunk;
    KArgs k;
    int rc = fill_common<T>(a, k);
    if (rc) return rc;
    if (a->out_dtype != MTP_F32 || (a->M % E) || (a->N % E)) return MTP_ERR_ARG;
    k.bias = nullptr;
    int split = a->split_k > 1 ? a->split_k : 1;
    if (split > k.k_tiles) split = k.k_tiles;
    k.k_tiles_per_split = (k.k_tiles + split - 1) / split;
    split = (k.k_tiles + k.k_tiles_per_split - 1) / k.k_tiles_per_split;
    const bool use_ws = split > 1 && a->aux != nullptr;
    k.atomic_out = split > 1 && !use_ws;
    k.split_stride = 0;
    if (split > 1) {
        if (a->ldc != a->N) return MTP_ERR_ARG;
        if (use_ws) {
            if ((uintptr_t)a->aux & 15) return MTP_ERR_ARG;
            k.C = (char*)a->aux;
            k.split_stride = (int64_t)a->M * a->N;
        } else {
            hipError_t e = hipMemsetAsync(a->C, 0, sizeof(float) * (size_t)a->M * (size_t)a->N, stream);
            if (e != hipSuccess) return (int)e;
        }
    }
    const int tiles_m = (k.M + BM - 1) / BM;
    dim3 grid(tiles_m * k.tiles_n, split), block(NT_THREADS);
    const bool full = (a->K % (8 * E) == 0) && (a->M % BM == 0) && (a->N % BN == 0);
    const bool tr = sizeof(T) == 2 && !(a->variant & 16) && (full || ((a->K % 64 == 0) && (a->M % 8 == 0) && (a->N % 8 == 0) && a->M >= 8 && a->N >= 8 && !(a->variant & 32768)));
    if (a->colsum && !tr) {
        rc = mtp_colsum_acc(a->A, a->in_dtype, a->lda, a->colsum, a->K, a->M, stream);
        if (rc) return rc;
    }
    if (tr) {
        k.colsum = a->colsum;
        const int ord = (a->variant >> 1) & 3;
        k.order = ord == 0 ? (a->N > a->M ? 2 : 0) : ord == 1 ? 1 : ord == 2 ? 2 : 0;
        hipLaunchKernelGGL(gemm_tn_tr_kernel, grid, block, STAGE_BYTES, stream, k);
    } else if (full && (a->variant & 8))
        hipLaunchKernelGGL((gemm_tn_sb_kernel<T, true>), grid, block, STAGE_BYTES, stream, k);
    else if (full)
        hipLaunchKernelGGL((gemm_tn_kernel<T, true>), grid, block, LDS_BYTES, stream, k);
    else
        hipLaunchKernelGGL((gemm_tn_kernel<T, false>), grid, block, LDS_BYTES, stream, k);
    if (use_ws && !a->defer_sum) {
        const int64_t n4 = (int64_t)a->M * a->N / 4;
        int64_t nb = (n4 + 255) / 256;
        hipLaunchKernelGGL(sum_partials_kernel, dim3((unsigned)(nb > 4096 ? 4096 : nb)), dim3(256), 0, stream, (const float*)a->aux, (float*)a->C, n4, split);
    }
    return mtp_launch_status();
}

struct SumJobs {
    const float* part[MTP_MAX_SEGMENTS];
    float* out[MTP_MAX_SEGMENTS];
    int64_t n4[MTP_MAX_SEGMENTS];
    int split[MTP_MAX_SEGMENTS];
};
__global__ __launch_bounds__(256) void sum_partials_batch_kernel(SumJobs t) {
    const int j = blockIdx.y;
    const float* __restrict__ part = t.part[j];
    float* __restrict__ out = t.out[j];
    const int64_t n4 = t.n4[j];
    const int split = t.split[j];
    for (int64_t i = (int64_t)blockIdx.x * 256 + threadIdx.x; i < n4; i += (int64_t)gridDim.x * 256) {
        float4 s = *reinterpret_cast<const float4*>(part + 4 * i);
        for (int z = 1; z < split; ++z) {
            const float4 v = *reinterpret_cast<const float4*>(part + 4 * (i + (int64_t)z * n4));
            s.x += v.x; s.y += v.y; s.z += v.z; s.w += v.w;
        }
        *reinterpret_cast<float4*>(out + 4 * i) = s;
    }
}

template <typename T, typename Tout>
int dispatch_epi(const mtp_gemm_args* a, hipStream_t s) {
    switch (a->epilogue) {
        case MTP_EPI_BIAS: return launch_nt<T, Tout, MTP_EPI_BIAS>(a, s);
        case MTP_EPI_BIAS_GELU: return launch_nt<T, Tout, MTP_EPI_BIAS_GELU>(a, s);
        case MTP_EPI_DGELU: return launch_nt<T, Tout, MTP_EPI_DGELU>(a, s);
        case MTP_EPI_BIAS_GELU_DG: return launch_nt<T, Tout, MTP_EPI_BIAS_GELU_DG>(a, s);
        case MTP_EPI_MUL: return launch_nt<T, Tout, MTP_EPI_MUL>(a, s);
        default: return MTP_ERR_UNSUPPORTED;
    }
}

}

extern "C" int mtp_gemm_nt(const mtp_gemm_args* a, mtp_stream_t stream) {
    if (!a) return MTP_ERR_ARG;
    hipStream_t s = (hipStream_t)stream;
    if (a->epilogue == MTP_EPI_BIAS_RES) {
        if (a->out_dtype != MTP_F32) return MTP_ERR_ARG;
        return a->in_dtype == MTP_BF16 ? launch_nt<bf16_t, float, MTP_EPI_BIAS_RES>(a, s)
                                      : launch_nt<float, float, MTP_EPI_BIAS_RES>(a, s);
    }
    if (a->in_dtype == MTP_BF16 && a->out_dtype == MTP_BF16) return dispatch_epi<bf16_t, bf16_t>(a, s);
    if (a->in_dtype == MTP_F32 && a->out_dtype == MTP_F32) return dispatch_epi<float, float>(a, s);
    if (a->in_dtype == MTP_BF16 && a->out_dtype == MTP_F32 && a->epilogue == MTP_EPI_BIAS) return launch_nt<bf16_t, float, MTP_EPI_BIAS>(a, s);
    return MTP_ERR_UNSUPPORTED;
}

extern "C" int64_t mtp_gemm_nt_workspace_bytes(void) { return 0; }

extern "C" int mtp_gemm_nt_tile(const mtp_gemm_args* a) {
    if (!a || !a->A || !a->B || !a->C || a->M <= 0 || a->N <= 0 || a->K <= 0) return MTP_ERR_ARG;
    if (a->in_dtype != MTP_BF16) return 128;
    KArgs k;
    if (fill_common<bf16_t>(a, k)) return MTP_ERR_ARG;
    const int cus = mtp_stream_cus(nullptr);
    if (nt_s8_mode(a, k, cus)) return 64;
    return nt_p8_mode(a, k, cus) ? 256 : 128;
}

// ... 20 lines not shown
```

### mtp_amd/csrc/gemm_tn_p8.hip

```cpp
#include "gemm_p8.h"

namespace {

typedef short tr_v4s_t __attribute__((ext_vector_type(4)));
typedef __attribute__((address_space(3))) char lds_char_t;
constexpr int TN_MAX_PROBLEMS = MTP_MAX_GROUPED_GEMMS;

struct TnProb {
    const char* A;
    const char* B;
    float* C;
    float* colsum;
    float* sqn;
    int M, N, K;
    int lda, ldb, ldc;
    int tile0, tiles_m, tiles_n;
    int splits;
    int kchunk;
    int pad_;
};
struct TnGroup {
    TnProb p[TN_MAX_PROBLEMS];
    int nprob, ntiles, plain;
};

struct T8Ctx {
    lds_char_t* smem;
    uint32_t offA[2][4];
    uint32_t offB[2][2];
    uint32_t voffA[2], voffB[2];
    uint32_t kstepA, kstepB;
    const char* pA[2][2];
    const char* pB[2][2];
    uint32_t m0base;
    bool colsum;
    uint32_t csoff;
    float cs[2][8];
};

__device__ __forceinline__ u32x4_t tr_frag8(lds_char_t* s) {
    const tr_v4s_t lo = __builtin_amdgcn_ds_read_tr16_b64_v4i16((__attribute__((address_space(3))) tr_v4s_t*)(s));
    const tr_v4s_t hi = __builtin_amdgcn_ds_read_tr16_b64_v4i16((__attribute__((address_space(3))) tr_v4s_t*)(s + 1024));
    const uint2 l = __builtin_bit_cast(uint2, lo), h = __builtin_bit_cast(uint2, hi);
    return u32x4_t{l.x, l.y, h.x, h.y};
}

struct TnOps {
    typedef T8Ctx Ctx;
    static constexpr int kLoadsPerPiecePair = 2;
    static constexpr int kMi1 = 4;
    template <int K, int BUF>
    static __device__ __forceinline__ void read_a(Ctx& c, u32x4_t (&a)[2][4]) {
        lds_char_t* s = c.smem + K * P8_HALF;
#pragma unroll
        for (int ks = 0; ks < 2; ++ks)
#pragma unroll
            for (int mi = 0; mi < 4; ++mi) a[ks][mi] = tr_frag8(s + c.offA[BUF][mi] + ks * 8192);
    }
    template <int K, int BUF>
    static __device__ __forceinline__ void read_b(Ctx& c, u32x4_t (&b)[2][2]) {
        lds_char_t* s = c.smem + K * P8_HALF;
#pragma unroll
        for (int ks = 0; ks < 2; ++ks)
#pragma unroll
            for (int ni = 0; ni < 2; ++ni) b[ks][ni] = tr_frag8(s + c.offB[BUF][ni] + ks * 8192);
    }
    template <int K, int BUF, int KS, int MI>
    static __device__ __forceinline__ void read_a_frag(Ctx& c, u32x4_t (&a)[2][4]) { a[KS][MI] = tr_frag8(c.smem + K * P8_HALF + c.offA[BUF][MI] + KS * 8192); }
    template <int K, int BUF, int KS, int NI>
    static __device__ __forceinline__ void read_b_frag(Ctx& c, u32x4_t (&b)[2][2]) { b[KS][NI] = tr_frag8(c.smem + K * P8_HALF + c.offB[BUF][NI] + KS * 8192); }
    template <int SK, int SBUF>
    static __device__ __forceinline__ void stage(Ctx& c) {
        constexpr int h = (SK == KA1 || SK == KB1) ? 1 : 0;
        const uint32_t l0 = c.m0base + SBUF * P8_BUF + SK * P8_HALF;
        if constexpr (SK == KA0 || SK == KA1)
            glds2(c.voffA[h], c.pA[h][0], c.pA[h][1], l0, l0 + 1024);
        else
            glds2(c.voffB[h], c.pB[h][0], c.pB[h][1], l0, l0 + 1024);
    }
    template <int K, int BUF>
    static __device__ __forceinline__ void retire_a(Ctx& c, u32x4_t (&)[2][4]) {
        if (c.colsum) {
            constexpr int h = K == KA1 ? 1 : 0;
            typedef __attribute__((address_space(3))) const u32x4_t lds_u32x4_t;
            const u32x4_t w0 = *reinterpret_cast<lds_u32x4_t*>(c.smem + BUF * P8_BUF + K * P8_HALF + c.csoff);
            const u32x4_t w1 = *reinterpret_cast<lds_u32x4_t*>(c.smem + BUF * P8_BUF + K * P8_HALF + c.csoff + 8192);
#pragma unroll
            for (int e = 0; e < 4; ++e) {
                c.cs[h][2 * e] += __uint_as_float(w0[e] << 16) + __uint_as_float(w1[e] << 16);
                c.cs[h][2 * e + 1] += __uint_as_float(w0[e] & 0xffff0000u) + __uint_as_float(w1[e] & 0xffff0000u);
            }
        }
        asm volatile("s_waitcnt lgkmcnt(0)" ::: "memory");
    }
    static __device__ __forceinline__ void retire_b(u32x4_t (&)[2][2]) { asm volatile("s_waitcnt lgkmcnt(0)" ::: "memory"); }
    static __device__ __forceinline__ void next_ktile(Ctx& c) {
        c.voffA[0] += c.kstepA; c.voffA[1] += c.kstepA;
        c.voffB[0] += c.kstepB; c.voffB[1] += c.kstepB;
    }
};

template <int XP, int RA = 1>
// ... 26 lines not shown
        for (int b = 0; b < 2; ++b) {
#pragma unroll
            for (int mi = 0; mi < 4; ++mi) c.offA[b][mi] = b * P8_BUF + rowoff + (uint32_t)((((wr * 4 + mi) ^ fr_)) << 5);
#pragma unroll
            for (int ni = 0; ni < 2; ++ni) c.offB[b][ni] = b * P8_BUF + rowoff + (uint32_t)((((wc * 2 + ni) ^ fr_)) << 5);
        }
        c.m0base = lds0 + wave * 2048;
        const int fd = (lane >> 4) | ((wave & 1) << 2);
        const int ch = (lane & 15) ^ (fd << 1);
        const int cbA[2] = {m0, m0 + 128 < q.M ? m0 + 128 : m0}, cbB[2] = {n0, n0 + 128 < q.N ? n0 + 128 : n0};
#pragma unroll
        for (int h = 0; h < 2; ++h) {
            c.voffA[h] = (uint32_t)((lane >> 4) * q.lda * 2 + (cbA[h] + ch * 8 < q.M ? ch * 16 : 0));
            c.voffB[h] = (uint32_t)((lane >> 4) * q.ldb * 2 + (cbB[h] + ch * 8 < q.N ? ch * 16 : 0));
        }
        c.kstepA = (uint32_t)(64 * q.lda * 2);
        c.kstepB = (uint32_t)(64 * q.ldb * 2);
#pragma unroll
        for (int h = 0; h < 2; ++h)
#pragma unroll
            for (int pc = 0; pc < 2; ++pc) {
                c.pA[h][pc] = q.A + ((int64_t)(k0 + wave * 8 + pc * 4) * q.lda + cbA[h]) * 2;
                c.pB[h][pc] = q.B + ((int64_t)(k0 + wave * 8 + pc * 4) * q.ldb + cbB[h]) * 2;
            }
        c.colsum = q.colsum != nullptr && tn == 0;
        c.csoff = (uint32_t)((tid >> 4) * 256 + (tid & 15) * 16);
#pragma unroll
        for (int h = 0; h < 2; ++h)
#pragma unroll
            for (int e = 0; e < 8; ++e) c.cs[h][e] = 0.f;
    }

    u32x4_t a[2][4], b0[2][2], b1[2][2];
    f32x4_t acc[4][8];
#pragma unroll
    for (int i = 0; i < 4; ++i)
#pragma unroll
        for (int j = 0; j < 8; ++j) acc[i][j] = f32x4_t{0.f, 0.f, 0.f, 0.f};

    TnOps::stage<KB1, 0>(c); TnOps::stage<KA0, 0>(c); TnOps::stage<KB0, 0>(c); TnOps::stage<KA1, 0>(c);
    TnOps::next_ktile(c);
    TnOps::stage<KB0, 1>(c); TnOps::stage<KA0, 1>(c); TnOps::stage<KB1, 1>(c); TnOps::stage<KA1, 1>(c);
    TnOps::next_ktile(c);
    if constexpr (RA) wait_vm<10>(); else wait_vm<12>();
    __builtin_amdgcn_sched_barrier(0);
    __builtin_amdgcn_s_barrier();
    __builtin_amdgcn_sched_barrier(0);
    TnOps::read_b<KB1, 0>(c, b1);
    if constexpr (RA) TnOps::read_a<KA0, 0>(c, a);
    TnOps::retire_b(b1);
    __builtin_amdgcn_sched_barrier(0);
    __builtin_amdgcn_s_barrier();
    if (!(XP & 2) && wr == 1) __builtin_amdgcn_s_barrier();
    __builtin_amdgcn_sched_barrier(0);

    if constexpr (RA) {
        for (int it = 0; it < pairs - 1; ++it) two_tiles_ra<TnOps, false>(c, a, b0, b1, acc);
        two_tiles_ra<TnOps, true>(c, a, b0, b1, acc);
    } else {
        for (int it = 0; it < pairs - 1; ++it) two_tiles<TnOps, false, XP>(c, a, b0, b1, acc);
        two_tiles<TnOps, true, XP>(c, a, b0, b1, acc);
    }

    __builtin_amdgcn_sched_barrier(0);
    if (!(XP & 2) && wr == 0) __builtin_amdgcn_s_barrier();
    __builtin_amdgcn_sched_barrier(0);

    if (c.colsum) {
        float* red = reinterpret_cast<float*>(smem);
        const int rg = tid >> 4;
        const int f = (rg & 3) | ((rg >> 1) & 4);
        const int ch = (tid & 15) ^ (f << 1);
#pragma unroll
        for (int h = 0; h < 2; ++h) {
            *reinterpret_cast<float4*>(red + (h * 32 + rg) * 128 + ch * 8) = make_float4(c.cs[h][0], c.cs[h][1], c.cs[h][2], c.cs[h][3]);
            *reinterpret_cast<float4*>(red + (h * 32 + rg) * 128 + ch * 8 + 4) = make_float4(c.cs[h][4], c.cs[h][5], c.cs[h][6], c.cs[h][7]);
        }
        __syncthreads();
        if (tid < 256) {
            const int h = tid >> 7, x = tid & 127;
            float s = 0.f;
#pragma unroll 8
            for (int r = 0; r < 32; ++r) s += red[(h * 32 + r) * 128 + x];
            if (m0 + h * 128 + x < q.M) atomicAdd(q.colsum + m0 + h * 128 + x, s);
        }
        __syncthreads();
    }

    if (q.sqn) {
        const int fr = lane & 15, gq = lane >> 4;
        const bool full = m0 + P8_BM <= q.M && n0 + P8_BN <= q.N;
        float ss = 0.f;
#pragma unroll
        for (int nf = 0; nf < 4; ++nf)
#pragma unroll
            for (int hm = 0; hm < 8; ++hm)
#pragma unroll
                for (int e = 0; e < 4; ++e) {
                    const float v = acc[nf][hm][e];
                    if (full) {
                        ss += v * v;
                    } else {
                        const int row = m0 + wr * 64 + (hm >> 2) * 128 + (hm & 3) * 16 + fr;
                        const int cc = nf * 16 + gq * 4 + e, col = n0 + wc * 32 + (cc >> 5) * 128 + (cc & 31);
                        ss += (row < q.M && col < q.N) ? v * v : 0.f;
                    }
                }
        ss = wave_sum(ss);
        if (lane == 0) atomicAdd(q.sqn, ss);
    }

    KArgs o = {};
    o.C = reinterpret_cast<char*>(q.C + (int64_t)piece * q.M * q.ldc);
    o.M = q.M; o.N = q.N; o.ldc = q.ldc;
    epilogue_lds<float, MTP_EPI_BIAS, 128, 128>(o, acc, smem + wave * P8_HALF, m0 + wr * 64, n0 + wc * 32, lane);
}

}

extern "C" int mtp_gemm_tn_grouped(const mtp_gemm_args* args, int count, mtp_stream_t stream) {
    if (!args || count <= 0) return MTP_ERR_ARG;
    if (count > TN_MAX_PROBLEMS) return MTP_ERR_UNSUPPORTED;
    TnGroup g = {};
    int64_t tiles = 0;
    for (int i = 0; i < count; ++i) {
        const mtp_gemm_args& a = args[i];
        if (!a.A || !a.B || !a.C || a.M <= 0 || a.N <= 0 || a.K <= 0) return MTP_ERR_ARG;
        if (((uintptr_t)a.A | (uintptr_t)a.B | (uintptr_t)a.C) & 15) return MTP_ERR_ARG;
        if (a.in_dtype != MTP_BF16 || a.out_dtype != MTP_F32) return MTP_ERR_UNSUPPORTED;
        if ((a.M % 8) || (a.N % 8) || (a.K % 128) || (a.lda % 8) || (a.ldb % 8) || (a.ldc % 4) || a.lda < a.M || a.ldb < a.N || a.ldc < a.N) return MTP_ERR_UNSUPPORTED;
        if ((uint64_t)a.K * (uint64_t)a.lda * 2 >= (1ull << 32) || (uint64_t)a.K * (uint64_t)a.ldb * 2 >= (1ull << 32)) return MTP_ERR_UNSUPPORTED;
        int splits = a.split_k > 1 ? a.split_k : 1;
        int64_t kchunk = a.K;
        if (splits > 1) {
            if (!a.aux || ((uintptr_t)a.aux & 15)) return MTP_ERR_ARG;
            if (!a.defer_sum && a.ldc != a.N) return MTP_ERR_UNSUPPORTED;
            kchunk = ((a.K / 128 + splits - 1) / splits) * 128;
            splits = (int)((a.K + kchunk - 1) / kchunk);
        }
        TnProb& q = g.p[i];
        q.A = (const char*)a.A; q.B = (const char*)a.B; q.C = splits > 1 ? (float*)a.aux : (float*)a.C; q.colsum = a.colsum;
        if (a.workspace && splits > 1) return MTP_ERR_UNSUPPORTED;
        if (a.workspace && (a.workspace_bytes < 4 || ((uintptr_t)a.workspace & 3))) return MTP_ERR_ARG;
        q.sqn = (float*)a.workspace;
        q.M = (int)a.M; q.N = (int)a.N; q.K = (int)a.K;
        q.lda = (int)a.lda; q.ldb = (int)a.ldb; q.ldc = (int)a.ldc;
        q.tiles_m = (int)((a.M + P8_BM - 1) / P8_BM); q.tiles_n = (int)((a.N + P8_BN - 1) / P8_BN);
        q.splits = splits; q.kchunk = (int)kchunk;
        q.tile0 = (int)tiles;
        tiles += (int64_t)q.tiles_m * q.tiles_n * splits;
        if (tiles >= (1 << 30)) return MTP_ERR_UNSUPPORTED;
    }
    g.nprob = count;
    g.ntiles = (int)tiles;
    g.plain = (args[0].variant >> 1) & 1;
    const int plain_phase = (args[0].variant >> 19) & 1;
    void (*kern)(TnGroup) = plain_phase ? gemm_tn_p8_kernel<0, 0> : gemm_tn_p8_kernel<0, 1>;
    static unsigned long long optin[2] = {0, 0};
    if (const int e = mtp_optin_lds((const void*)kern, P8_LDS, optin[plain_phase])) return e;
    hipLaunchKernelGGL(kern, dim3((unsigned)tiles), dim3(P8_THREADS), P8_LDS, (hipStream_t)stream, g);
    int rc = mtp_launch_status();
    const float* parts[12];
    float* outs[12];
    int64_t numel[12];
    int nsplit[12], n = 0;
    for (int i = 0; i < count && rc == 0; ++i) {
        if (g.p[i].splits > 1 && !args[i].defer_sum) {
            parts[n] = (const float*)args[i].aux; outs[n] = (float*)args[i].C; numel[n] = args[i].M * args[i].N; nsplit[n] = g.p[i].splits;
            ++n;
        }
        if (n == 12 || (n > 0 && i == count - 1)) {
            rc = mtp_sum_partials_batch(parts, outs, numel, nsplit, n, stream);
            n = 0;
        }
    }
    return rc;
}
```

### mtp_amd/engine.py

```python
import os

import torch

from . import ops

F32 = torch.float32


class _Blk:
    __slots__ = ("window", "pre", "wqkv", "wqkvT", "wproj", "wprojT", "w1", "w1T", "w2", "w2T", "wsamp", "bsamp", "bproj", "b2", "wproj_s", "w2_s")


class BackboneEngine:
    def __init__(self, module, act_dtype=torch.bfloat16):
        self.m = module
        self.act = act_dtype
        self.C = module.embed_dim
        self.depth = len(module.blocks)
        self.heads = module.num_heads
        self.hd = self.C // self.heads
        self.scale = module.qk_scale if module.qk_scale is not None else self.hd ** -0.5
        self.window = [bool(w) for w in module.window_blocks]
        self.out_indices = list(module.out_indices)
        self._key = None
# ... 16 lines not shown
    def prepare_weights(self, force=False):
        P = self.params()
        key = self._weights_key(P)
        if not force and key == self._key:
            return
        ptrs = (self.act,) + tuple(p.data_ptr() for p in P.values())
        if self._wimg is None or ptrs != self._wimg_ptrs:
            self._build_weight_images(P)
            self._wimg_ptrs = ptrs
        with torch.no_grad():
            for pre, b in self._ls:
                g1, g2 = P[pre + "gamma_1"].detach(), P[pre + "gamma_2"].detach()
                torch.mul(P[pre + "attn.proj.weight"].detach(), g1[:, None], out=b.wproj_s)
                torch.mul(P[pre + "mlp.fc2.weight"].detach(), g2[:, None], out=b.w2_s)
                torch.mul(P[pre + "attn.proj.bias"].detach(), g1, out=b.bproj)
                torch.mul(P[pre + "mlp.fc2.bias"].detach(), g2, out=b.b2)
        if force or getattr(self, "_images_fresh", None) != key:
            self._wimg.refresh()
        self._images_fresh = None
        for name, (wg, wgT) in self._fpn.items():
            ops.convt_pack(P[name + ".weight"].detach().contiguous(), wg, wgT)
        self._key = key

    def mark_images_fresh(self):
        self._images_fresh = self._weights_key(self.params())
        self._key = None

    def _build_weight_images(self, P):
        dev = P["patch_embed.proj.weight"].device
        act, H, C = self.act, self.heads, self.C
        entries = []

        def both(w2d):
            w2d = w2d.detach()
            assert w2d.is_contiguous()
            R, Cc = w2d.shape
            wt = torch.empty(Cc, R, device=dev, dtype=act)
            w = w2d if act == F32 else torch.empty(R, Cc, device=dev, dtype=act)
            entries.append((w2d, None if act == F32 else w, wt, False))
            return w, wt

        ls = getattr(self.m, "init_values", None) is not None
        self._ls = []

        blks = []
        for i in range(self.depth):
            b = _Blk()
            b.window = self.window[i]
            b.pre = pre = "blocks.%d." % i
            b.wqkv, b.wqkvT = both(P[pre + "attn.qkv.weight"])
            b.bproj, b.b2 = P[pre + "attn.proj.bias"].detach(), P[pre + "mlp.fc2.bias"].detach()
            if ls:
                b.wproj_s, b.w2_s = torch.empty_like(P[pre + "attn.proj.weight"]), torch.empty_like(P[pre + "mlp.fc2.weight"])
                b.bproj, b.b2 = torch.empty_like(P[pre + "attn.proj.bias"]), torch.empty_like(P[pre + "mlp.fc2.bias"])
                self._ls.append((pre, b))
                b.wproj, b.wprojT = both(b.wproj_s)
            else:
                b.wproj, b.wprojT = both(P[pre + "attn.proj.weight"])
            b.w1, b.w1T = both(P[pre + "mlp.fc1.weight"])
            b.w2, b.w2T = both(b.w2_s if ls else P[pre + "mlp.fc2.weight"])
            if b.window:
                b.wsamp = torch.empty(5 * H, C, device=dev, dtype=F32)
                b.bsamp = torch.empty(5 * H, device=dev, dtype=F32)
                r0 = 0
                for head, rows in (("sampling_offsets", 2 * H), ("sampling_scales", 2 * H), ("sampling_angles", H)):
                    entries.append((P[pre + "attn.%s.2.weight" % head].detach().view(rows, C), b.wsamp[r0:r0 + rows], None, True))
                    entries.append((P[pre + "attn.%s.2.bias" % head].detach().view(1, rows), b.bsamp[r0:r0 + rows], None, True))
                    r0 += rows
            blks.append(b)
        self._blk = blks
        wpe = P["patch_embed.proj.weight"].detach()
        self._pe = both(wpe.view(wpe.shape[0], -1))
        fpn = {}
        for name in ("fpn1.0", "fpn1.3", "fpn2.0"):
            if name + ".weight" in P:
                Cin, Cout = P[name + ".weight"].shape[:2]
                fpn[name] = (torch.empty(4 * Cout, Cin, device=dev, dtype=act), torch.empty(Cin, 4 * Cout, device=dev, dtype=act))
        self._fpn = fpn
        self._wimg = ops.WeightImages(entries, act)

    wgrad_side_stream = True
    wgrad_max_jobs = 8
    wgrad_keep = 2

    def _wgrad_stream(self):
        if not self.wgrad_side_stream:
            return None
        import mtp_amd
        note = mtp_amd.hw_queue_note()
        if note:
            import warnings
            warnings.warn(note, RuntimeWarning, stacklevel=2)
        if int(self.wgrad_side_stream) == 2:
            return ops.low_priority_stream(self.dev)
        st = getattr(self, "_wstream", None)
        if st is None or st.device != self.dev:
            st = self._wstream = torch.cuda.Stream(device=self.dev)
        return st

    def warm_streams(self, device):
        self.dev = torch.device(device)
        st = self._wgrad_stream()
        if st is not None:
            with torch.cuda.stream(st):
                torch.zeros(1, device=self.dev).add_(1.0)
            st.synchronize()

    def _e(self, *shape, dtype=None):
        return torch.empty(*shape, device=self.dev, dtype=dtype or self.act)

    @staticmethod
    def _colsum(dy, out):
        return ops.colsum(dy, out, accumulate=True)

    def _ln_bwd(self, *args, **kw):
        return ops.layernorm_bwd(*args, accumulate=True, defer=self._ln_parts, **kw)

    def _ln_flush(self):
        if self._ln_parts:
            ops.reduce_rows_deferred(self._ln_parts)
        if self._sl_jobs:
            ops.small_linear_dw_segments_flush(self._sl_jobs)

    def _full_rel(self, pre, Hp, Wp):
        h = self.P.get(pre + "attn.full_attn_rel_pos_h")
        if h is not None:
            w = self.P[pre + "attn.full_attn_rel_pos_w"]
            if h.shape[0] < 2 * Hp - 1 or w.shape[0] < 2 * Wp - 1:
                raise ValueError("%sattn.full_attn_rel_pos_h/w have %d / %d rows, a %d x %d token grid needs %d / %d (resize them like "
                                 "init_weights does, or build the model for this input size)" % (pre, h.shape[0], w.shape[0], Hp, Wp, 2 * Hp - 1, 2 * Wp - 1))
            return h[:2 * Hp - 1], w[:2 * Wp - 1]
        key = (Hp, Wp)
        if self._zero_rel.get(key) is None:
            self._zero_rel[key] = (torch.zeros(2 * Hp - 1, self.hd, device=self.dev, dtype=F32),
                                   torch.zeros(2 * Wp - 1, self.hd, device=self.dev, dtype=F32))
        return self._zero_rel[key]

    def _drop_scales(self, B, training):
        rates = [float(self.m.drop_path_rates[i]) for i in range(self.depth)]
        live = [training and r > 0.0 and self.m.blocks[i].training for i, r in enumerate(rates)]
        if not any(live):
            return [(None, None)] * self.depth
        keep = torch.tensor([1.0 - r for r in rates], dtype=F32).to(self.dev, non_blocking=True).view(self.depth, 1, 1)
        s = torch.floor(keep + torch.rand(self.depth, 2, B, device=self.dev, dtype=F32)) / keep
        return [(s[i, 0], s[i, 1]) if live[i] else (None, None) for i in range(self.depth)]

    def _block_fwd(self, i, x, B, Hp, Wp, dps, save):
        P, b, C, T, N = self.P, self._blk[i], self.C, x.shape[0], Hp * Wp
        pre = b.pre
        s = {}
        mean1, rstd1 = self._e(T, dtype=F32), self._e(T, dtype=F32)
        ln1 = ops.layernorm_fwd(x, P[pre + "norm1.weight"], P[pre + "norm1.bias"], self._e(T, C), mean1, rstd1)
        if b.window:
            nh, nw = ops.rvsa_windows(Hp, Wp)
            R = B * nh * nw
            avg, pooled = self._e(R, C, dtype=F32), self._e(R, C, dtype=F32)
            samp = ops.rvsa_sampling_fwd(ln1, b.wsamp, b.bsamp, avg, pooled, self._e(R, 5 * self.heads, dtype=F32), B, Hp, Wp)
        qkv = ops.gemm_nt(ln1, b.wqkv, self._e(T, 3 * C), bias=P[pre + "attn.qkv.bias"])
        o = self._e(T, C)
        if b.window:
            lse = self._e(R * self.heads * 49, dtype=F32)
            ops.rvsa_attn_fwd(qkv, samp, o, lse, P[pre + "attn.rel_pos_h"], P[pre + "attn.rel_pos_w"],
                              P[pre + "attn.relative_position_bias_table"], B, Hp, Wp, self.heads, self.scale)
            s.update(avg=avg, pooled=pooled, samp=samp)
        else:
            lse = self._e(B * self.heads * N, dtype=F32)
            rel_h, rel_w = self._full_rel(pre, Hp, Wp)
            ops.full_attn_fwd(qkv, o, lse, rel_h, rel_w, B, Hp, Wp, self.heads, self.scale)
        x1 = ops.gemm_nt(o, b.wproj, self._e(T, C, dtype=F32), epi=ops.EPI_BIAS_RES, bias=b.bproj, res=x,
                         rowscale=dps[0], rows_per_sample=N)
        mean2, rstd2 = self._e(T, dtype=F32), self._e(T, dtype=F32)
        ln2 = ops.layernorm_fwd(x1, P[pre + "norm2.weight"], P[pre + "norm2.bias"], self._e(T, C), mean2, rstd2)
        u = self._e(T, 4 * C)
        h = ops.gemm_nt(ln2, b.w1, self._e(T, 4 * C), epi=ops.EPI_BIAS_GELU_DG, bias=P[pre + "mlp.fc1.bias"], aux=u)
        x2 = ops.gemm_nt(h, b.w2, self._e(T, C, dtype=F32), epi=ops.EPI_BIAS_RES, bias=b.b2, res=x1,
                         rowscale=dps[1], rows_per_sample=N)
        if save:
            s.update(x=x, mean1=mean1, rstd1=rstd1, ln1=ln1, qkv=qkv, o=o, lse=lse, x1=x1, mean2=mean2, rstd2=rstd2, ln2=ln2, u=u, h=h)
        return x2, s

    def _layer_scale_grads(self, pre, lin, gname, G):
        P = self.P
        gw, gb, gam = G[pre + lin + ".weight"], G[pre + lin + ".bias"], P[pre + gname]
        G[pre + gname].add_((gw * P[pre + lin + ".weight"]).sum(1) + gb * P[pre + lin + ".bias"])
        gw.mul_(gam[:, None])
        gb.mul_(gam)

    def _block_bwd(self, i, s, dx2, dx2_act, B, Hp, Wp, dps, G, extra, prev_scale):
        P, b, C, N = self.P, self._blk[i], self.C, Hp * Wp
        pre = b.pre
        T = dx2.shape[0]
        wq = self._wq
        ls = pre + "gamma_1" in G
        wq.add(dx2_act, s["h"], G[pre + "mlp.fc2.weight"], G[pre + "mlp.fc2.bias"], after=(lambda: self._layer_scale_grads(pre, "mlp.fc2", "gamma_2", G)) if ls else None,
               norm_ok=not ls)
        du = ops.gemm_nt(dx2_act, b.w2T, self._e(T, 4 * C), epi=ops.EPI_MUL, aux=s["u"])
        wq.add(du, s["ln2"], G[pre + "mlp.fc1.weight"], G[pre + "mlp.fc1.bias"])
        dln2 = ops.gemm_nt(du, b.w1T, self._e(T, C))
        del du
        dx1, dx1_act = self._e(T, C, dtype=F32), self._e(T, C)
        self._ln_bwd(dln2, s["x1"], s["mean2"], s["rstd2"], P[pre + "norm2.weight"], dx1, G[pre + "norm2.weight"], G[pre + "norm2.bias"],
                          dres=dx2, dx_copy=dx1_act, copy_scale=dps[0], rows_per_sample=N)
        wq.add(dx1_act, s["o"], G[pre + "attn.proj.weight"], G[pre + "attn.proj.bias"], after=(lambda: self._layer_scale_grads(pre, "attn.proj", "gamma_1", G)) if ls else None,
               norm_ok=not ls)
        do = ops.gemm_nt(dx1_act, b.wprojT, self._e(T, C))
        dqkv = self._e(T, 3 * C)
        if b.window:
            nh, nw = ops.rvsa_windows(Hp, Wp)
            R = B * nh * nw
            H = self.heads
            dsamp = self._e(R, 5 * H, dtype=F32)
            ops.rvsa_attn_bwd(s["qkv"], s["samp"], s["o"], do, s["lse"], dqkv, dsamp,
                              P[pre + "attn.rel_pos_h"], P[pre + "attn.rel_pos_w"], P[pre + "attn.relative_position_bias_table"],
                              G[pre + "attn.rel_pos_h"], G[pre + "attn.rel_pos_w"], G[pre + "attn.relative_position_bias_table"],
                              B, Hp, Wp, H, self.scale, accumulate=True, defer=self._ln_parts)
            names = ("sampling_offsets", "sampling_scales", "sampling_angles")
            self._sl_jobs.append((s["pooled"], dsamp, [G[pre + "attn.%s.2.weight" % n].view(-1, C) for n in names],
                                  [G[pre + "attn.%s.2.bias" % n] for n in names]))
        else:
            rel_h, rel_w = self._full_rel(pre, Hp, Wp)
            if pre + "attn.full_attn_rel_pos_h" in G:
                drel_h, drel_w = G[pre + "attn.full_attn_rel_pos_h"][:2 * Hp - 1], G[pre + "attn.full_attn_rel_pos_w"][:2 * Wp - 1]
            else:
                drel_h, drel_w = self._e(*rel_h.shape, dtype=F32), self._e(*rel_w.shape, dtype=F32)
            ops.full_attn_bwd(s["qkv"], s["o"], do, s["lse"], dqkv, rel_h, rel_w, drel_h, drel_w, B, Hp, Wp, self.heads, self.scale,
                              accumulate=True, defer=self._ln_parts)
        wq.add(dqkv, s["ln1"], G[pre + "attn.qkv.weight"], G[pre + "attn.qkv.bias"])
        win_add = None
        if b.window:
            win_add = ops.rvsa_sampling_bwd_win(dsamp, b.wsamp, s["avg"], self._e(*s["avg"].shape, dtype=F32))
        dln1 = ops.gemm_nt(dqkv, b.wqkvT, self._e(T, C))
        dx0, dx0_act = self._e(T, C, dtype=F32), self._e(T, C)
        self._ln_bwd(dln1, s["x"], s["mean1"], s["rstd1"], P[pre + "norm1.weight"], dx0, G[pre + "norm1.weight"], G[pre + "norm1.bias"],
                          dres=dx1, extra=extra, dx_copy=dx0_act, copy_scale=prev_scale, rows_per_sample=N,
                          **(dict(win_add=win_add, grid=(B, Hp, Wp)) if win_add is not None else {}))
        return dx0, dx0_act

    def forward(self, img, training=False, need_grad=False, feature_dtype=None):
        m = self.m
        self.dev = img.device
        self.prepare_weights()
        self.P = P = {k: v.detach() for k, v in self.params().items()}
        C, act = self.C, self.act
        ps = m.patch_size
        fdt = feature_dtype or act
        if img.dtype == torch.uint8:
            pp = getattr(m, "data_preprocessor", None)
            if pp is None:
                raise ValueError("uint8 input needs ViT_Win_RVSA_V3_WSZ7.set_data_preprocessor(mean, std, ...)")
            B, H, W, Cin = img.shape
            Hp, Wp = ops.padded_grid(H, W, ps, pp["pad_size_divisor"])
            N, T = Hp * Wp, B * Hp * Wp
            cols = ops.preprocess_patchify(img.contiguous(), self._e(T, Cin * ps * ps), ps, pp["mean"], pp["std"], pp["bgr_to_rgb"],
                                           pp["pad_size_divisor"], pp["pad_value"])
            H, W = Hp * ps, Wp * ps
        else:
            B, Cin, H, W = img.shape
            Hp, Wp = H // ps, W // ps
            N, T = Hp * Wp, B * Hp * Wp
            img = img.contiguous()
            if img.dtype != F32:
                img = img.float()
            cols = ops.patchify(img, self._e(T, Cin * ps * ps), ps)
        pos = P.get("pos_embed")
        if pos is not None:
            assert pos.shape[1] == N, "pos_embed does not match the input size"
            x = ops.gemm_nt(cols, self._pe[0], self._e(T, C, dtype=F32), epi=ops.EPI_BIAS_RES, bias=P["patch_embed.proj.bias"],
                            res=pos.reshape(N, C), res_mod=N)
        else:
            x = ops.gemm_nt(cols, self._pe[0], self._e(T, C, dtype=F32), bias=P["patch_embed.proj.bias"])
        dps = self._drop_scales(B, training)
        ckpt = bool(m.use_checkpoint) and need_grad
        saved, taps = [], {}
        vitdet = bool(getattr(m, "_vitdet", False))
        last = self.depth - 1 if vitdet else max(self.out_indices)
        for i in range(self.depth):
            if i > last:
                break
            xin = x
            x, s = self._block_fwd(i, x, B, Hp, Wp, dps[i], save=need_grad and not ckpt)
            saved.append(s if (need_grad and not ckpt) else ({"x": xin} if need_grad else None))
            if i in self.out_indices:
                taps[i] = x
        final = None
        if vitdet:
            fm, fr = self._e(T, dtype=F32), self._e(T, dtype=F32)
            xn = ops.layernorm_fwd(x, P["norm.weight"], P["norm.bias"], self._e(T, C, dtype=F32), fm, fr)
            final = (x, fm, fr)
            tap_list = [xn, xn, xn, xn]
        else:
            tap_list = [taps[i] for i in self.out_indices]
        if getattr(m, "_taps_only", False):
            feats = [ops.tokens_to_nchw(t, self._e(B, C, Hp, Wp, dtype=fdt), B, Hp, Wp, 0) for t in tap_list]
            fctx = {"taps_only": True}
        else:
            feats, fctx = self._fpn_fwd(tap_list, B, Hp, Wp, fdt, need_grad)
        ctx = None
        if need_grad:
            ctx = dict(saved=saved, dps=dps, fctx=fctx, cols=cols, geom=(B, Cin, H, W, Hp, Wp), ckpt=ckpt, last=last, final=final)
        return feats, ctx

    def _fpn_fwd(self, taps, B, Hp, Wp, fdt, need_grad):
        P, C, T = self.P, self.C, B * Hp * Wp
        m = self.m
        feats, fctx = [], {}
        if m.patch_size == 8:
            t0 = taps[0] if self.act == F32 else ops.cast(taps[0], self._e(T, C))
            z = ops.gemm_nt(t0, self._fpn["fpn1.0"][0], self._e(T, 4 * C), bias=P["fpn1.0.bias"], bias_mod=C)
            feats.append(ops.tokens_to_nchw(z.view(4 * T, C), self._e(B, C, 2 * Hp, 2 * Wp, dtype=fdt), B, Hp, Wp, 1))
            feats.append(ops.tokens_to_nchw(taps[1], self._e(B, C, Hp, Wp, dtype=fdt), B, Hp, Wp, 0))
            H2, W2, H4, W4 = Hp // 2, Wp // 2, Hp // 4, Wp // 4
            p3 = ops.maxpool2_tokens_fwd(taps[2], self._e(B * H2 * W2, C), B, Hp, Wp)
            feats.append(ops.tokens_to_nchw(p3, self._e(B, C, H2, W2, dtype=fdt), B, H2, W2, 0))
            q1 = ops.maxpool2_tokens_fwd(taps[3], self._e(B * H2 * W2, C, dtype=F32), B, Hp, Wp)
            q2 = ops.maxpool2_tokens_fwd(q1, self._e(B * H4 * W4, C), B, H2, W2)
            feats.append(ops.tokens_to_nchw(q2, self._e(B, C, H4, W4, dtype=fdt), B, H4, W4, 0))
            if need_grad:
                fctx = dict(p8=True, t0=t0, tap2=taps[2], tap3=taps[3], q1=q1)
            return feats, fctx
        if m.patch_size != 16:
            raise NotImplementedError("the reference defines the FPN tail for patch_size 16 and 8 only (VIT:640-670)")
        t0 = taps[0] if self.act == F32 else ops.cast(taps[0], self._e(T, C))
        y1 = ops.gemm_nt(t0, self._fpn["fpn1.0"][0], self._e(T, 4 * C), bias=P["fpn1.0.bias"], bias_mod=C)
        mean, rstd = self._e(4 * T, dtype=F32), self._e(4 * T, dtype=F32)
        g1 = ops.layernorm_fwd(y1.view(4 * T, C), P["fpn1.1.ln.weight"], P["fpn1.1.ln.bias"], self._e(4 * T, C), mean, rstd, gelu=True)
        y2 = ops.gemm_nt(g1, self._fpn["fpn1.3"][0], self._e(4 * T, 4 * C), bias=P["fpn1.3.bias"], bias_mod=C)
        feats.append(ops.tokens_to_nchw(y2.view(16 * T, C), self._e(B, C, 4 * Hp, 4 * Wp, dtype=fdt), B, Hp, Wp, 2))
        t1 = taps[1] if self.act == F32 else ops.cast(taps[1], self._e(T, C))
        z = ops.gemm_nt(t1, self._fpn["fpn2.0"][0], self._e(T, 4 * C), bias=P["fpn2.0.bias"], bias_mod=C)
        feats.append(ops.tokens_to_nchw(z.view(4 * T, C), self._e(B, C, 2 * Hp, 2 * Wp, dtype=fdt), B, Hp, Wp, 1))
        feats.append(ops.tokens_to_nchw(taps[2], self._e(B, C, Hp, Wp, dtype=fdt), B, Hp, Wp, 0))
        Ho, Wo = Hp // 2, Wp // 2
        pooled = ops.maxpool2_tokens_fwd(taps[3], self._e(B * Ho * Wo, C), B, Hp, Wp)
        feats.append(ops.tokens_to_nchw(pooled, self._e(B, C, Ho, Wo, dtype=fdt), B, Ho, Wo, 0))
        if need_grad:
            fctx = dict(t0=t0, y1=y1, mean=mean, rstd=rstd, g1=g1, t1=t1, tap3=taps[3])
        return feats, fctx

    def _convt_wgrad(self, dy, x, gw):
        dwg = self._e(dy.shape[1], x.shape[1], dtype=F32)
        self._wq.add(dy, x, dwg, after=lambda: ops.convt_unpack_grad(dwg, gw), norm_of=gw)

    def _fpn_bwd(self, dfeats, fctx, B, Hp, Wp, G):
        P, C, T, act = self.P, self.C, B * Hp * Wp, self.act
        out = [None] * 4

        def as_in(df):
            df = df.contiguous()
            return df if df.dtype in (F32, torch.bfloat16) else df.float()

        if fctx.get("p8"):
            H2, W2, H4, W4 = Hp // 2, Wp // 2, Hp // 4, Wp // 4
            if dfeats[0] is not None:
                dz = ops.nchw_to_tokens(as_in(dfeats[0]), self._e(4 * T, C), B, Hp, Wp, 1)
                self._convt_wgrad(dz.view(T, 4 * C), fctx["t0"], G["fpn1.0.weight"])
                self._colsum(dz, G["fpn1.0.bias"])
                out[0] = ops.gemm_nt(dz.view(T, 4 * C), self._fpn["fpn1.0"][1], self._e(T, C, dtype=F32))
            if dfeats[1] is not None:
                out[1] = ops.nchw_to_tokens(as_in(dfeats[1]), self._e(T, C, dtype=F32), B, Hp, Wp, 0)
            if dfeats[2] is not None:
                dp = ops.nchw_to_tokens(as_in(dfeats[2]), self._e(B * H2 * W2, C, dtype=F32), B, H2, W2, 0)
                out[2] = ops.maxpool2_tokens_bwd(fctx["tap2"], dp, self._e(T, C, dtype=F32), B, Hp, Wp)
            if dfeats[3] is not None:
                dq2 = ops.nchw_to_tokens(as_in(dfeats[3]), self._e(B * H4 * W4, C, dtype=F32), B, H4, W4, 0)
                dq1 = ops.maxpool2_tokens_bwd(fctx["q1"], dq2, self._e(B * H2 * W2, C, dtype=F32), B, H2, W2)
                out[3] = ops.maxpool2_tokens_bwd(fctx["tap3"], dq1, self._e(T, C, dtype=F32), B, Hp, Wp)
            return out

        if dfeats[0] is not None:
            dy2 = ops.nchw_to_tokens(as_in(dfeats[0]), self._e(16 * T, C), B, Hp, Wp, 2)
            self._convt_wgrad(dy2.view(4 * T, 4 * C), fctx["g1"], G["fpn1.3.weight"])
            self._colsum(dy2, G["fpn1.3.bias"])
            dg1 = ops.gemm_nt(dy2.view(4 * T, 4 * C), self._fpn["fpn1.3"][1], self._e(4 * T, C))
            dy1 = self._e(4 * T, C)
            self._ln_bwd(dg1, fctx["y1"].view(4 * T, C), fctx["mean"], fctx["rstd"], P["fpn1.1.ln.weight"], dy1,
                              G["fpn1.1.ln.weight"], G["fpn1.1.ln.bias"], beta=P["fpn1.1.ln.bias"], gelu=True)
            self._convt_wgrad(dy1.view(T, 4 * C), fctx["t0"], G["fpn1.0.weight"])
            self._colsum(dy1, G["fpn1.0.bias"])
            out[0] = ops.gemm_nt(dy1.view(T, 4 * C), self._fpn["fpn1.0"][1], self._e(T, C, dtype=F32))
        if dfeats[1] is not None:
            dz = ops.nchw_to_tokens(as_in(dfeats[1]), self._e(4 * T, C), B, Hp, Wp, 1)
            self._convt_wgrad(dz.view(T, 4 * C), fctx["t1"], G["fpn2.0.weight"])
            self._colsum(dz, G["fpn2.0.bias"])
            out[1] = ops.gemm_nt(dz.view(T, 4 * C), self._fpn["fpn2.0"][1], self._e(T, C, dtype=F32))
        if dfeats[2] is not None:
            out[2] = ops.nchw_to_tokens(as_in(dfeats[2]), self._e(T, C, dtype=F32), B, Hp, Wp, 0)
        if dfeats[3] is not None:
            Ho, Wo = Hp // 2, Wp // 2
            dp = ops.nchw_to_tokens(as_in(dfeats[3]), self._e(B * Ho * Wo, C, dtype=F32), B, Ho, Wo, 0)
            out[3] = ops.maxpool2_tokens_bwd(fctx["tap3"], dp, self._e(T, C, dtype=F32), B, Hp, Wp)
        return out

    def backward(self, ctx, dfeats, G, need_input_grad=False, on_block_done=None, split_last=False, sqn=None):
        B, Cin, H, W, Hp, Wp = ctx["geom"]
        C, N, T = self.C, Hp * Wp, B * Hp * Wp
        P = self.P
        self.dev = ctx["cols"].device
        self._ln_parts = []
        self._sl_jobs = []
        self._wq = wq = ops.WgradQueue(stream=self._wgrad_stream())
        wq.max_jobs = self.wgrad_max_jobs if wq.stream is not None else 0
        wq.sqn = sqn
        self.norm_covered = wq.covered
        if ctx["fctx"].get("taps_only"):
            dtaps = [None if d is None else ops.nchw_to_tokens((d.contiguous() if d.dtype in (F32, torch.bfloat16) else d.float().contiguous()),
                                                               self._e(T, C, dtype=F32), B, Hp, Wp, 0) for d in dfeats]
        else:
            dtaps = self._fpn_bwd(dfeats, ctx["fctx"], B, Hp, Wp, G)
        tapgrad = {}
        last, dps, saved = ctx["last"], ctx["dps"], ctx["saved"]
        if ctx.get("final") is not None:
            dsum = None
            for d in dtaps:
                if d is None:
                    continue
                if dsum is None:
                    dsum = d
                else:
                    ops.axpy(dsum, d)
            if dsum is not None:
                xl, fm, fr = ctx["final"]
                tapgrad[last] = self._ln_bwd(dsum, xl, fm, fr, P["norm.weight"], self._e(T, C, dtype=F32), G["norm.weight"], G["norm.bias"])
        else:
            for idx, d in zip(self.out_indices, dtaps):
                if d is None:
                    continue
                if idx in tapgrad:
                    ops.axpy(tapgrad[idx], d)
                else:
                    tapgrad[idx] = d
        self._ln_flush()
        if on_block_done is not None and not wq.jobs:
            on_block_done(self.depth)
        if last not in tapgrad:
            tapgrad[last] = torch.zeros(T, C, device=self.dev, dtype=F32)
        dx = tapgrad[last]
        dx_act = self._scaled_copy(dx, dps[last][1], N)
        waiting = []
        pending = []
        for i in range(last, -1, -1):
            s = saved[i]
            if ctx["ckpt"]:
                _, s = self._block_fwd(i, s["x"], B, Hp, Wp, dps[i], save=True)
            extra = tapgrad.get(i - 1) if i > 0 else None
            prev_scale = dps[i - 1][1] if i > 0 else None
            dx, dx_act = self._block_bwd(i, s, dx, dx_act, B, Hp, Wp, dps[i], G, extra, prev_scale)
            saved[i] = None
            waiting.append(i)
            if i == 0:
                wq.add(dx_act, ctx["cols"], G["patch_embed.proj.weight"].view(C, -1), G["patch_embed.proj.bias"])
            if i == 0 or wq.should_flush() or not wq.jobs or (split_last and i == 1):
                wq.flush()
                self._ln_flush()
                if wq.stream is None:
                    if on_block_done is not None:
                        on_block_done(waiting[-1])
                else:
                    pending.append((waiting[-1], wq.launched))
                    wq.wait(keep=self.wgrad_keep)
                    while pending and pending[0][1] <= wq.launched - len(wq.inflight):
                        g = pending.pop(0)[0]
                        if on_block_done is not None:
                            on_block_done(g)
                waiting = []
        wq.wait()
        if pending and on_block_done is not None:
# ... 14 lines not shown
```

### mtp_amd/ops.py

```python
import ctypes as C

import torch

from . import _lib
from ._lib import (EPI_BIAS, EPI_BIAS_GELU, EPI_BIAS_GELU_DG, EPI_BIAS_RES, EPI_DGELU, EPI_MUL, MTP_BF16, MTP_F32, GemmArgs,
                   check)

_DT = {torch.float32: MTP_F32, torch.bfloat16: MTP_BF16}
def lib():
    return _lib.load()


def _dt(t):
    try:
        return _DT[t.dtype]
    except KeyError:
        raise TypeError("mtp_amd ops take float32 / bfloat16 tensors, got %s" % t.dtype)


def _p(t):
    if t is None:
        return None
    if not t.is_cuda:
        raise RuntimeError("mtp_amd ops run only on an MI355X device tensor (no CPU fallback)")
    if not t.is_contiguous():
        raise RuntimeError("mtp_amd ops need contiguous tensors")
    if t.device.index != torch.cuda.current_device():
        raise RuntimeError("mtp_amd ops: tensor on %s but the current device is cuda:%d -- call torch.cuda.set_device(%d) (or use "
                           "`with torch.cuda.device(...)`) before running the backbone" % (t.device, torch.cuda.current_device(), t.device.index))
    return t.data_ptr()


def _s():
    return torch.cuda.current_stream().cuda_stream


def _scratch(shape, device, dtype):
    return torch.empty(shape, device=device, dtype=dtype)


def _f32(t):
    if t is not None and t.dtype != torch.float32:
        raise TypeError("expected a float32 tensor")
    return _p(t)


def _nt_args(a, w, out, epi, bias, bias_mod, res, res_mod, rowscale, rows_per_sample, aux, variant, n=None):
    M, K = a.shape
    N = w.shape[0] if n is None else n
    assert w.shape[1] == K and out.shape[0] == M and out.shape[1] >= N and w.shape[0] >= N and a.dtype == w.dtype
    assert n is not None or out.shape[1] == N
    g = GemmArgs()
    g.A, g.B, g.C = _p(a), _p(w), _p(out)
    g.M, g.N, g.K = M, N, K
    g.lda, g.ldb, g.ldc = K, K, out.shape[1]
    g.in_dtype, g.out_dtype, g.epilogue = _dt(a), _dt(out), epi
    g.bias, g.bias_mod = _f32(bias), bias_mod
    g.res, g.res_ld, g.res_mod = _f32(res), (res.shape[-1] if res is not None else 0), res_mod
    g.rowscale, g.rows_per_sample = _f32(rowscale), rows_per_sample
    g.aux, g.aux_ld = _p(aux), (aux.shape[-1] if aux is not None else 0)
    if aux is not None:
        assert aux.dtype == out.dtype and tuple(aux.shape) == (M, N) and out.shape[1] == N
    g.split_k, g.variant = 1, variant
    return g


def gemm_nt(a, w, out, epi=EPI_BIAS, bias=None, bias_mod=0, res=None, res_mod=0, rowscale=None, rows_per_sample=0,
            aux=None, variant=0, n=None):
    g = _nt_args(a, w, out, epi, bias, bias_mod, res, res_mod, rowscale, rows_per_sample, aux, variant, n)
    check(lib().mtp_gemm_nt(C.byref(g), _s()), "mtp_gemm_nt")
    return out


def gemm_nt_tile(a, w, out, epi=EPI_BIAS, bias=None, bias_mod=0, res=None, res_mod=0, rowscale=None, rows_per_sample=0,
                 aux=None, variant=0, n=None):
    g = _nt_args(a, w, out, epi, bias, bias_mod, res, res_mod, rowscale, rows_per_sample, aux, variant, n)
    rc = lib().mtp_gemm_nt_tile(C.byref(g))
    if rc < 0:
        check(rc, "mtp_gemm_nt_tile")
    return rc


def pick_split_k(M, N, K):
    tiles = ((M + 127) // 128) * ((N + 127) // 128)
    split = max(1, min(16, round(512 / tiles)))
    if split > 1 and split % 2:
        split += 1
    return max(1, min(split, K // 1024))


def effective_split_k(K, dtype, split):
    k_tiles = -(-K // (64 if dtype == torch.bfloat16 else 32))
    split = max(1, min(int(split), k_tiles))
    per = -(-k_tiles // split)
    return -(-k_tiles // per)


def gemm_tn(a, b, out, split_k=None, use_workspace=True, variant=0, colsum=None, defer=None, m=None):
    K, M = a.shape
    lda = M
    if m is not None:
        assert m <= M
        M = m
    N = b.shape[1]
    assert b.shape[0] == K and out.dtype == torch.float32 and out.numel() == M * N and a.dtype == b.dtype
    g = GemmArgs()
    if colsum is not None:
        assert colsum.dtype == torch.float32 and colsum.numel() == M and colsum.is_contiguous()
        g.colsum = _p(colsum)
    g.A, g.B, g.C = _p(a), _p(b), _p(out)
    g.M, g.N, g.K = M, N, K
    g.lda, g.ldb, g.ldc = lda, N, N
    g.in_dtype, g.out_dtype, g.epilogue = _dt(a), MTP_F32, EPI_BIAS
    g.split_k = effective_split_k(K, a.dtype, pick_split_k(M, N, K) if split_k is None else split_k)
    g.variant = variant
    if g.split_k > 1 and use_workspace:
        ws = _scratch((g.split_k * M * N,), out.device, torch.float32)
        g.aux = _p(ws)
        if defer is not None:
            g.defer_sum = 1
            defer.append((ws, out, M * N, g.split_k))
    check(lib().mtp_gemm_tn(C.byref(g), _s()), "mtp_gemm_tn")
    return out


MAX_GROUPED = 32


def grouped_tiles(M, N):
    return -(-M // 256) * -(-N // 256) if M % 8 == 0 and N % 8 == 0 and M >= 8 and N >= 8 else 0


def grouped_splits(K, tiles):
    if K < 16384:
        return 1
    return max(1, min(64, K // 4096, 256 // tiles))


_low_streams = {}


def low_priority_stream(device):
    device = torch.device(device)
    idx = device.index if device.index is not None else torch.cuda.current_device()
    st = _low_streams.get(idx)
    if st is None:
        h = C.c_void_p()
        with torch.cuda.device(idx):
            check(lib().mtp_stream_create_low_priority(C.byref(h)), "mtp_stream_create_low_priority")
        st = _low_streams[idx] = torch.cuda.ExternalStream(h.value, device=torch.device("cuda", idx))
    return st


_mask_streams = {}


def cu_mask_words(kind, part, parts=2, cus_per_xcc=32, xccs=8):
    words = [0] * (cus_per_xcc * xccs // 32)
    for i in range(cus_per_xcc * xccs):
        j = i // xccs
        mine = (j % parts == part) if kind == "interleaved" else (j * parts // cus_per_xcc == part)
        if mine:
            words[i // 32] |= 1 << (i % 32)
    return words


def cu_mask_stream(device, words):
    device = torch.device(device)
    idx = device.index if device.index is not None else torch.cuda.current_device()
    key = (idx, tuple(words))
    st = _mask_streams.get(key)
    if st is None:
        h = C.c_void_p()
        arr = (C.c_uint32 * len(words))(*words)
        with torch.cuda.device(idx):
            check(lib().mtp_stream_create_cu_mask(arr, len(words), C.byref(h)), "mtp_stream_create_cu_mask")
        st = _mask_streams[key] = torch.cuda.ExternalStream(h.value, device=torch.device("cuda", idx))
    return st


class WgradQueue:

    def __init__(self, cus=256, variant=0, stream=None):
        self.jobs, self.tiles, self.cus, self.variant = [], 0, cus, variant
        self.stream, self.inflight = stream, []
        self.max_jobs = 0
        self.launched = 0
        self.after = []
        self.sqn, self.covered = None, []

    def add(self, dy, x, dw, colsum=None, after=None, norm_of=None, norm_ok=True):
        K, M = dy.shape
        N = x.shape[1]
        t = grouped_tiles(M, N)
        fits = (K * M * 2 < (1 << 32) and K * N * 2 < (1 << 32) and dy.data_ptr() % 16 == 0 and x.data_ptr() % 16 == 0 and dw.data_ptr() % 16 == 0
                and dy.is_contiguous() and x.is_contiguous())
        if t == 0 or K % 128 or dy.dtype != torch.bfloat16 or x.dtype != torch.bfloat16 or not fits:
            gemm_tn(dy, x, dw, colsum=colsum)
            if after is not None:
                after()
            return False
        assert x.shape[0] == K and dw.dtype == torch.float32 and dw.numel() == M * N and dw.is_contiguous()
        splits = grouped_splits(K, t)
        part = _scratch((splits, M, N), dw.device, torch.float32) if splits > 1 else None
        use_sqn = self.sqn is not None and splits == 1 and norm_ok
        self.jobs.append((dy, x, dw, colsum, splits, part, use_sqn))
        if use_sqn:
            self.covered.append(dw if norm_of is None else norm_of)
        if after is not None:
            self.after.append(after)
        self.tiles += t * splits
        return True

    def should_flush(self, next_tiles=0, next_jobs=4):
        if not self.jobs:
            return False
        if len(self.jobs) + next_jobs > MAX_GROUPED or (self.max_jobs and len(self.jobs) >= self.max_jobs):
            return True
        rounds = -(-self.tiles // self.cus)
        return self.tiles / (rounds * self.cus) >= 0.93

    def flush(self):
        if self.stream is None or not self.jobs:
            return self._launch()
        ready = torch.cuda.Event()
        ready.record()
        held = list(self.jobs)
        with torch.cuda.stream(self.stream):
            self.stream.wait_event(ready)
            self._launch()
            done = torch.cuda.Event()
            done.record()
        self.inflight.append((done, held))
        self.launched += 1

    def wait(self, keep=0):
        while len(self.inflight) > keep:
            done, _ = self.inflight.pop(0)
            torch.cuda.current_stream().wait_event(done)

    def _launch(self):
        while self.jobs:
            chunk, self.jobs = self.jobs[:MAX_GROUPED], self.jobs[MAX_GROUPED:]
            arr = (GemmArgs * len(chunk))()
            for g, (dy, x, dw, cs, splits, part, use_sqn) in zip(arr, chunk):
                K, M = dy.shape
                N = x.shape[1]
                g.A, g.B, g.C = _p(dy), _p(x), _p(dw)
                g.M, g.N, g.K = M, N, K
                g.lda, g.ldb, g.ldc = M, N, N
                g.in_dtype, g.out_dtype, g.variant = MTP_BF16, MTP_F32, self.variant
                if splits > 1:
                    g.split_k, g.aux = splits, _p(part)
                if use_sqn:
                    g.workspace, g.workspace_bytes = _p(self.sqn), 4
                if cs is not None:
                    assert cs.dtype == torch.float32 and cs.numel() == M and cs.is_contiguous()
                    g.colsum = _p(cs)
            check(lib().mtp_gemm_tn_grouped(arr, len(chunk), _s()), "mtp_gemm_tn_grouped")
        after, self.after = self.after, []
        for fn in after:
            fn()
        self.tiles = 0


def sum_partials(jobs):
    while jobs:
        chunk, jobs[:] = jobs[:12], jobs[12:]
        n = len(chunk)
        P = C.c_void_p * n
        parts, outs = P(*[j[0].data_ptr() for j in chunk]), P(*[j[1].data_ptr() for j in chunk])
        numel, splits = (C.c_int64 * n)(*[j[2] for j in chunk]), (C.c_int * n)(*[j[3] for j in chunk])
        check(lib().mtp_sum_partials_batch(parts, outs, numel, splits, n, _s()), "mtp_sum_partials_batch")


def layernorm_fwd(x, gamma, beta, y, mean=None, rstd=None, eps=1e-6, gelu=False):
    rows, Cc = x.shape
    check(lib().mtp_layernorm_fwd(_p(x), _dt(x), _f32(gamma), _f32(beta), _p(y), _dt(y), _f32(mean), _f32(rstd),
                                  rows, Cc, eps, int(gelu), _s()), "mtp_layernorm_fwd")
    return y


def layernorm_bwd(dy, x, mean, rstd, gamma, dx, dgamma, dbeta, beta=None, gelu=False, dres=None, extra=None,
                  dx_copy=None, copy_scale=None, rows_per_sample=0, accumulate=False, defer=None, win_add=None, grid=None):
    rows, Cc = x.shape
    nblk = lib().mtp_layernorm_bwd_partial_rows(rows)
    part = _scratch((nblk, 2 * Cc), x.device, torch.float32)
    if win_add is not None:
        B, Hp, Wp = grid
        nh, nw = rvsa_windows(Hp, Wp)
        assert not gelu and tuple(win_add.shape) == (B * nh * nw, Cc) and B * Hp * Wp == rows
        check(lib().mtp_layernorm_bwd_win(_p(dy), _dt(dy), _p(x), _dt(x), _f32(mean), _f32(rstd), _f32(gamma), _f32(dres), _f32(extra), _p(dx), _dt(dx),
                                          _p(dx_copy), (_dt(dx_copy) if dx_copy is not None else 0), _f32(copy_scale), rows_per_sample,
                                          part.data_ptr(), part.data_ptr() + 4 * Cc, 2 * Cc, rows, Cc, _f32(win_add), B, Hp, Wp, _s()), "mtp_layernorm_bwd_win")
    else:
        check(lib().mtp_layernorm_bwd(_p(dy), _dt(dy), _p(x), _dt(x), _f32(mean), _f32(rstd), _f32(gamma), _f32(beta), int(gelu),
                                      _f32(dres), _f32(extra), _p(dx), _dt(dx), _p(dx_copy), (_dt(dx_copy) if dx_copy is not None else 0),
                                      _f32(copy_scale), rows_per_sample, part.data_ptr(), part.data_ptr() + 4 * Cc, 2 * Cc, rows, Cc, _s()),
              "mtp_layernorm_bwd")
    if defer is not None and _adjacent(dgamma, dbeta) and dgamma.numel() == Cc:
        defer.append((part, dgamma, accumulate))
    else:
        _reduce_pair(part, Cc, dgamma, dbeta, accumulate)
    return dx


def layernorm_residual_fwd(h, gamma, beta, x, layer_scale, out, out_act, mean, rstd, sample_scale=None, rows_per_sample=0, eps=1e-6):
    rows, Cc = h.shape
    check(lib().mtp_layernorm_residual_fwd(_p(h), _dt(h), _f32(gamma), _f32(beta), _f32(x), _f32(layer_scale), _f32(sample_scale), rows_per_sample,
                                           _f32(out), _p(out_act), _f32(mean), _f32(rstd), rows, Cc, eps, _s()), "mtp_layernorm_residual_fwd")
    return out


def layernorm_residual_bwd(dout, h, mean, rstd, gamma, beta, layer_scale, dh, dgamma, dbeta, dls, sample_scale=None, rows_per_sample=0, defer=None):
    rows, Cc = h.shape
    nblk = lib().mtp_layernorm_bwd_partial_rows(rows)
    part = _scratch((nblk, 3 * Cc), h.device, torch.float32)
    check(lib().mtp_layernorm_residual_bwd(_f32(dout), _p(h), _dt(h), _f32(mean), _f32(rstd), _f32(gamma), _f32(beta), _f32(layer_scale), _f32(sample_scale),
                                           rows_per_sample, _p(dh), part.data_ptr(), rows, Cc, _s()), "mtp_layernorm_residual_bwd")
    pair = _adjacent(dgamma, dbeta) and dgamma.numel() == Cc
    if defer is not None and pair:
        defer.append((part[:, :2 * Cc], dgamma, True))
        defer.append((part[:, 2 * Cc:], dls, True))
    else:
        _reduce_pair(part[:, :2 * Cc], Cc, dgamma, dbeta, True)
        reduce_rows(part[:, 2 * Cc:], dls, True)
    return dh


REDUCE_BATCH_MAX = 32


def reduce_rows_deferred(items):
    groups = {}
    for it in items:
        part, out, acc = it[:3]
        tr = it[3] if len(it) > 3 else None
        groups.setdefault((tuple(part.shape), part.stride(0), bool(acc), tr), []).append((part, out))
    for ((rows, cols), ld, acc, tr), g in groups.items():
        for i0 in range(0, len(g), REDUCE_BATCH_MAX):
            chunk = g[i0:i0 + REDUCE_BATCH_MAX]
# ... 245 lines not shown
    _reduce_pair(part, (2 * Hp - 1) * hd, drel_h, drel_w, accumulate)
    return dqkv


def rvsa_windows(Hp, Wp):
    nh = (Hp + (7 - Hp % 7) % 7) // 7
    nw = (Wp + (7 - Wp % 7) % 7) // 7
    return nh, nw


def rvsa_pool_fwd(x, avg, pooled, B, Hp, Wp):
    check(lib().mtp_rvsa_pool_fwd(_p(x), _dt(x), _f32(avg), _f32(pooled), B, Hp, Wp, x.shape[-1], _s()), "mtp_rvsa_pool_fwd")


def rvsa_pool_bwd(dpooled, avg, dx, B, Hp, Wp, accumulate=True):
    check(lib().mtp_rvsa_pool_bwd(_f32(dpooled), _f32(avg), _p(dx), _dt(dx), int(accumulate), B, Hp, Wp, dx.shape[-1], _s()), "mtp_rvsa_pool_bwd")


def rvsa_sampling_fwd(x, w, b, avg, pooled, samp, B, Hp, Wp):
    check(lib().mtp_rvsa_sampling_fwd(_p(x), _dt(x), _f32(w), _f32(b), _f32(avg), _f32(pooled), _f32(samp), B, Hp, Wp, x.shape[-1], w.shape[0], _s()),
          "mtp_rvsa_sampling_fwd")
    return samp


def rvsa_sampling_bwd(dsamp, w, avg, dx, B, Hp, Wp):
    check(lib().mtp_rvsa_sampling_bwd(_f32(dsamp), _f32(w), _f32(avg), _p(dx), _dt(dx), B, Hp, Wp, dx.shape[-1], w.shape[0], _s()), "mtp_rvsa_sampling_bwd")
    return dx


def rvsa_sampling_bwd_win(dsamp, w, avg, g):
    R, Cc = avg.shape
    check(lib().mtp_rvsa_sampling_bwd_win(_f32(dsamp), _f32(w), _f32(avg), _f32(g), R, Cc, w.shape[0], _s()), "mtp_rvsa_sampling_bwd_win")
    return g


def small_linear_fwd(x, w, b, y):
    R, K = x.shape
    check(lib().mtp_small_linear_fwd(_f32(x), _f32(w), _f32(b), _f32(y), R, w.shape[0], K, _s()), "mtp_small_linear_fwd")
    return y


def small_linear_bwd(x, w, dy, dx, dw, db):
    R, K = x.shape
    check(lib().mtp_small_linear_bwd(_f32(x), _f32(w), _f32(dy), _f32(dx), _f32(dw), _f32(db), R, w.shape[0], K, _s()), "mtp_small_linear_bwd")


def small_linear_dw_segments(x, dy, dws, dbs):
    R, K = x.shape
    n = len(dws)
    assert 0 < n <= 4 and len(dbs) == n and sum(d.shape[0] for d in dws) == dy.shape[1]
    rows = (C.c_int64 * n)(*[d.shape[0] for d in dws])
    P = C.c_void_p * n
    check(lib().mtp_small_linear_dw_segments(_f32(x), _f32(dy), R, dy.shape[1], K, n, rows, P(*[_f32(d) for d in dws]), P(*[_f32(d) for d in dbs]), _s()),
          "mtp_small_linear_dw_segments")


SL_BATCH = 8


def small_linear_dw_segments_flush(jobs):
    groups = {}
    for x, dy, dws, dbs in jobs:
        groups.setdefault((tuple(x.shape), tuple(dy.shape), tuple(d.shape[0] for d in dws)), []).append((x, dy, dws, dbs))
    for ((R, K), (_, N), rows_), g in groups.items():
        nseg = len(rows_)
        rows = (C.c_int64 * nseg)(*rows_)
        for i0 in range(0, len(g), SL_BATCH):
            chunk = g[i0:i0 + SL_BATCH]
            n = len(chunk)
            P, PS = C.c_void_p * n, C.c_void_p * (n * nseg)
            check(lib().mtp_small_linear_dw_segments_batched(P(*[_f32(c[0]) for c in chunk]), P(*[_f32(c[1]) for c in chunk]), n, R, N, K, nseg, rows,
                                                             PS(*[_f32(d) for c in chunk for d in c[2]]), PS(*[_f32(d) for c in chunk for d in c[3]]), _s()),
                  "mtp_small_linear_dw_segments_batched")
    del jobs[:]


def rvsa_attn_fwd(qkv, samp, o, lse, rel_h, rel_w, table, B, Hp, Wp, heads, scale):
    hd = qkv.shape[1] // (3 * heads)
    check(lib().mtp_rvsa_attn_fwd(_p(qkv), _f32(samp), _p(o), _f32(lse), _dt(qkv), _f32(rel_h), _f32(rel_w), _f32(table),
                                  B, Hp, Wp, heads, hd, scale, _s()), "mtp_rvsa_attn_fwd")
    return o, lse


def rvsa_attn_bwd(qkv, samp, o, dout, lse, dqkv, dsamp, rel_h, rel_w, table, drel_h, drel_w, dtable, B, Hp, Wp, heads, scale, accumulate=False, defer=None):
    hd = qkv.shape[1] // (3 * heads)
    T, C3 = qkv.shape
    Cc = C3 // 3
    nh, nw = rvsa_windows(Hp, Wp)
    nblk = B * nh * nw * heads
    dev = qkv.device
    dkv = _scratch((T, 2 * Cc), dev, torch.float32)
    rel_part = _scratch((nblk, 26 * hd), dev, torch.float32)
    tab_part = _scratch((B * nh * nw, heads * 169), dev, torch.float32)
    check(lib().mtp_rvsa_attn_bwd(_p(qkv), _f32(samp), _p(o), _p(dout), _f32(lse), _p(dqkv), _p(dkv), _f32(dsamp), _p(rel_part), _p(tab_part),
                                  _dt(qkv), _f32(rel_h), _f32(rel_w), _f32(table), B, Hp, Wp, heads, hd, scale, _s()), "mtp_rvsa_attn_bwd")
    if defer is not None and _adjacent(drel_h, drel_w) and drel_h.numel() == 13 * hd:
        defer.append((rel_part, drel_h, accumulate))
        defer.append((tab_part, dtable, accumulate, (heads, 169)))
        return dqkv
    _reduce_pair(rel_part, 13 * hd, drel_h, drel_w, accumulate)
    check(lib().mtp_reduce_rows_t_f32(_p(tab_part), tab_part.shape[1], _f32(dtable), tab_part.shape[0], heads, 169, int(accumulate), _s()),
          "mtp_reduce_rows_t_f32")
    return dqkv


def zero_segments(base, start, count):
    assert base.dtype == torch.float32 and start.dtype == torch.int64 and count.dtype == torch.int64 and start.numel() == count.numel()
    check(lib().mtp_zero_segments_f32(_p(base), start.data_ptr(), count.data_ptr(), start.numel(), _s()), "mtp_zero_segments_f32")


def sqnorm(g, out):
    check(lib().mtp_sqnorm_f32(_f32(g), _f32(out), g.numel(), _s()), "mtp_sqnorm_f32")
    return out


def sqnorm_segments(base, start, count, out):
    assert base.dtype == torch.float32 and start.dtype == torch.int64 and count.dtype == torch.int64 and start.numel() == count.numel()
    check(lib().mtp_sqnorm_segments_f32(_p(base), start.data_ptr(), count.data_ptr(), start.numel(), _f32(out), _s()), "mtp_sqnorm_segments_f32")
    return out


def adamw_flat(p, g, m, v, seg_start, seg_wd, hyper, sqn=None, max_norm=0.0, grad_scale=1.0):
    assert seg_start.dtype == torch.int64 and seg_start.is_cuda
    check(lib().mtp_adamw_flat(_f32(p), _f32(g), _f32(m), _f32(v), p.numel(), seg_start.data_ptr(), _f32(seg_wd), seg_start.numel(),
                               _f32(hyper), _f32(sqn), max_norm, grad_scale, _s()), "mtp_adamw_flat")


def adamw_flat_lr(p, g, m, v, seg_start, seg_wd, seg_lr, hyper, sqn=None, max_norm=0.0, grad_scale=1.0):
    assert seg_start.dtype == torch.int64 and seg_start.is_cuda and seg_lr.numel() == seg_start.numel() == seg_wd.numel()
    check(lib().mtp_adamw_flat_lr(_f32(p), _f32(g), _f32(m), _f32(v), p.numel(), seg_start.data_ptr(), _f32(seg_wd), _f32(seg_lr), seg_start.numel(),
                                  _f32(hyper), _f32(sqn), max_norm, grad_scale, _s()), "mtp_adamw_flat_lr")


def pad8(n):
    return (n + 7) // 8 * 8


def conv_out(h, stride):
    return (h - 1) // stride + 1


def im2col3x3(x, strides, cols, N, H, W, Cin, stride):
    Kp = cols.shape[1]
    assert cols.shape[0] == N * conv_out(H, stride) * conv_out(W, stride) and Kp >= 9 * Cin
    sN, sH, sW, sC = strides
    if not x.is_cuda:
        raise RuntimeError("mtp_amd ops run only on an MI355X device tensor (no CPU fallback)")
    check(lib().mtp_im2col3x3(x.data_ptr(), _dt(x), sN, sH, sW, sC, _p(cols), _dt(cols), N, H, W, Cin, stride, Kp, _s()), "mtp_im2col3x3")
    return cols


def col2im3x3(dcols, dx, strides, N, H, W, Cin, stride, accumulate=False):
    sN, sH, sW, sC = strides
    assert dx.dtype == torch.float32 and dx.is_cuda
    check(lib().mtp_col2im3x3(_p(dcols), _dt(dcols), dx.data_ptr(), sN, sH, sW, sC, N, H, W, Cin, stride, dcols.shape[1], int(accumulate), _s()), "mtp_col2im3x3")
    return dx


def conv3x3_pack(w, w2, w2t):
    Cout, Cin = w.shape[:2]
    img = w2 if w2 is not None else w2t
    Kp = w2.shape[1] if w2 is not None else w2t.shape[0]
    check(lib().mtp_conv3x3_pack(_f32(w), _p(w2), _p(w2t), _dt(img), Cout, Cin, Kp, _s()), "mtp_conv3x3_pack")


def conv3x3_unpack_grad(dw2, dw):
    Cout, Cin = dw.shape[:2]
    check(lib().mtp_conv3x3_unpack_grad(_f32(dw2), _f32(dw), Cout, Cin, dw2.shape[1], _s()), "mtp_conv3x3_unpack_grad")
    return dw


def pack_rows_padded(w, wp, wpt):
    R, Cc = w.shape
    img = wp if wp is not None else wpt
    Rp = wp.shape[0] if wp is not None else wpt.shape[1]
    check(lib().mtp_pack_rows_padded(_f32(w), _p(wp), _p(wpt), _dt(img), R, Cc, Rp, _s()), "mtp_pack_rows_padded")


# ... 190 lines not shown
```

Before: 1893 images/sec.

## Fuse RVSA window-factor backward into scatter kernel and fold conv-transpose bias colsum into wgrad

Adds extra blocks to the RVSA backward scatter-GEMM launch that compute the per-window sampling gradient factor, removing a separate sampling_bwd_win kernel launch per windowed block. The fused path reuses the kernel's shared memory and reads dsamp directly instead of staging it in LDS. Separately, FPN conv-transpose bias gradients are now accumulated inside the wgrad GEMM's colsum via a modulo index, replacing standalone colsum kernels. The modulo path adds atomics contention onto fewer bias entries.

```diff
diff --git a/include/mtp_hip.h b/include/mtp_hip.h
--- a/include/mtp_hip.h
+++ b/include/mtp_hip.h
@@ -172,6 +172,11 @@
                       void* dqkv, float* dkv_f32, float* dsamp, float* rel_part, float* tab_part, int dtype,
                       const float* rel_h, const float* rel_w, const float* bias_table,
                       int64_t B, int64_t Hp, int64_t Wp, int64_t heads, int64_t hd, float scale, mtp_stream_t stream);
+int mtp_rvsa_attn_bwd_win(const void* qkv, const float* samp, const void* o, const void* dout, const float* lse,
+                          void* dqkv, float* dkv_f32, float* dsamp, float* rel_part, float* tab_part, int dtype,
+                          const float* rel_h, const float* rel_w, const float* bias_table,
+                          int64_t B, int64_t Hp, int64_t Wp, int64_t heads, int64_t hd, float scale,
+                          const float* w, const float* avg, float* g, mtp_stream_t stream);
 
 int mtp_zero_segments_f32(float* base, const int64_t* start, const int64_t* count, int n, mtp_stream_t stream);
 int mtp_sqnorm_f32(const float* g, float* out, int64_t n, mtp_stream_t stream);
diff --git a/mtp_amd/_lib.py b/mtp_amd/_lib.py
--- a/mtp_amd/_lib.py
+++ b/mtp_amd/_lib.py
@@ -111,6 +111,7 @@
     "mtp_small_linear_dw_segments_batched": (i32, [p, p, i32, i64, i64, i64, i32, p, p, p, p]),
     "mtp_rvsa_attn_fwd": (i32, [p, p, p, p, i32, p, p, p, i64, i64, i64, i64, i64, f32, p]),
     "mtp_rvsa_attn_bwd": (i32, [p, p, p, p, p, p, p, p, p, p, i32, p, p, p, i64, i64, i64, i64, i64, f32, p]),
+    "mtp_rvsa_attn_bwd_win": (i32, [p, p, p, p, p, p, p, p, p, p, i32, p, p, p, i64, i64, i64, i64, i64, f32, p, p, p, p]),
     "mtp_zero_segments_f32": (i32, [p, p, p, i32, p]),
     "mtp_sqnorm_f32": (i32, [p, p, i64, p]),
     "mtp_sqnorm_segments_f32": (i32, [p, p, p, i32, p, p]),
diff --git a/mtp_amd/csrc/attn.hip b/mtp_amd/csrc/attn.hip
--- a/mtp_amd/csrc/attn.hip
+++ b/mtp_amd/csrc/attn.hip
@@ -910,3 +910,20 @@
     }
     return mtp_launch_status();
 }
+
+extern "C" int mtp_rvsa_attn_bwd_win(const void* qkv, const float* samp, const void* o, const void* dout, const float* lse,
+                                     void* dqkv, float* dkv_f32, float* dsamp, float* rel_part, float* tab_part, int dtype,
+                                     const float* rel_h, const float* rel_w, const float* bias_table,
+                                     int64_t B, int64_t Hp, int64_t Wp, int64_t heads, int64_t hd, float scale,
+                                     const float* w, const float* avg, float* g, mtp_stream_t stream) {
+    if (!qkv || !samp || !o || !dout || !lse || !dqkv || !dkv_f32 || !dsamp || !rel_part || !tab_part || !rel_h || !rel_w || !bias_table || !w || !avg || !g) return MTP_ERR_ARG;
+    if (B <= 0 || Hp < 7 || Wp < 7 || heads <= 0) return MTP_ERR_ARG;
+    if (hd != HD) return MTP_ERR_UNSUPPORTED;
+    if (dtype == MTP_BF16 && mtp_use_mfma_attn() && mtp_rvsa_bwd_mfma_scatter_mode(Hp, Wp, heads) == 4 && 5 * heads <= 4096)
+        return mtp_rvsa_bwd_mfma_launch(qkv, samp, o, dout, lse, dqkv, dkv_f32, dsamp, rel_part, tab_part, rel_h, rel_w, bias_table, B, Hp, Wp, heads, scale, (hipStream_t)stream,
+                                        w, avg, g);
+    const int rc = mtp_rvsa_attn_bwd(qkv, samp, o, dout, lse, dqkv, dkv_f32, dsamp, rel_part, tab_part, dtype, rel_h, rel_w, bias_table, B, Hp, Wp, heads, hd, scale, stream);
+    if (rc) return rc;
+    const RvsaGeom gm = make_geom(Hp, Wp, heads);
+    return mtp_rvsa_sampling_bwd_win(dsamp, w, avg, g, B * gm.nh * gm.nw, heads * HD, 5 * heads, stream);
+}
diff --git a/mtp_amd/csrc/attn_mfma.h b/mtp_amd/csrc/attn_mfma.h
--- a/mtp_amd/csrc/attn_mfma.h
+++ b/mtp_amd/csrc/attn_mfma.h
@@ -6,7 +6,8 @@
                              int64_t B, int64_t Hp, int64_t Wp, int64_t heads, float scale, hipStream_t s);
 int mtp_rvsa_bwd_mfma_launch(const void* qkv, const float* samp, const void* o, const void* dout, const float* lse, void* dqkv, float* dkv, float* dsamp,
                              float* rel_part, float* tab_part, const float* rel_h, const float* rel_w, const float* bias_table,
-                             int64_t B, int64_t Hp, int64_t Wp, int64_t heads, float scale, hipStream_t s);
+                             int64_t B, int64_t Hp, int64_t Wp, int64_t heads, float scale, hipStream_t s,
+                             const float* wsamp = nullptr, const float* avg = nullptr, float* gwin = nullptr);
 int mtp_rvsa_bwd_mfma_scatter_mode(int64_t Hp, int64_t Wp, int64_t heads);
 int mtp_full_fwd_mfma_launch(const void* qkv, void* o, float* lse, const float* rel_h, const float* rel_w,
                              int64_t B, int64_t Hp, int64_t Wp, int64_t heads, float scale, hipStream_t s);
diff --git a/mtp_amd/csrc/attn_rvsa_bwd4.hip b/mtp_amd/csrc/attn_rvsa_bwd4.hip
--- a/mtp_amd/csrc/attn_rvsa_bwd4.hip
+++ b/mtp_amd/csrc/attn_rvsa_bwd4.hip
@@ -972,11 +972,19 @@
 constexpr int SCB = 224;
 
 __global__ __launch_bounds__(256, 2) void rvsa_scatter_gemm_kernel(const bf16_t* __restrict__ dsel, const float* __restrict__ samp, bf16_t* __restrict__ dqkv,
-                                                                  RvsaGeom g) {
+                                                                  RvsaGeom g, const float* __restrict__ dsamp, const float* __restrict__ wsamp,
+                                                                  const float* __restrict__ avg, float* __restrict__ gwin, int nscat, int wcy) {
     __shared__ __attribute__((aligned(16))) char Kimg[SCB * 128];
     __shared__ __attribute__((aligned(16))) char Vimg[SCB * 128];
     __shared__ __attribute__((aligned(16))) float xs[SCB];
     __shared__ __attribute__((aligned(16))) float ys[SCB];
+    if ((int)blockIdx.x >= nscat) {
+        if (blockIdx.y == 0) {
+            const int e = (int)blockIdx.x - nscat;
+            rvsa_win_factor(dsamp, wsamp, avg, gwin, e / wcy, e % wcy, g.heads * HD, 5 * g.heads, reinterpret_cast<float4(*)[64]>(Vimg));
+        }
+        return;
+    }
     const int tid = threadIdx.x, lane = tid & 63, wave = tid >> 6, fr = lane & 15, gq = lane >> 4;
     const int H = g.heads, nW = g.nh * g.nw, S = nW * 49;
     const int h = blockIdx.x % H, b = blockIdx.x / H;
@@ -1116,9 +1124,10 @@
 
 int mtp_rvsa_bwd_mfma_launch(const void* qkv, const float* samp, const void* o, const void* dout, const float* lse, void* dqkv, float* dkv, float* dsamp,
                              float* rel_part, float* tab_part, const float* rel_h, const float* rel_w, const float* bias_table,
-                             int64_t B, int64_t Hp, int64_t Wp, int64_t heads, float scale, hipStream_t s) {
+                             int64_t B, int64_t Hp, int64_t Wp, int64_t heads, float scale, hipStream_t s, const float* wsamp, const float* avg, float* gwin) {
     const RvsaGeom g = make_geom(Hp, Wp, heads);
     const int mode = mtp_rvsa_bwd_mfma_scatter_mode(Hp, Wp, heads);
+    if (gwin && (mode != 4 || !wsamp || !avg)) return MTP_ERR_UNSUPPORTED;
     const dim3 grid((unsigned)(B * g.nh * g.nw * heads));
     if (mode == 4) {
         static const bool old4 = []() { const char* e = getenv("MTP_RVSA_BWD"); return e && e[0] == '4'; }();
@@ -1129,7 +1138,10 @@
             hipLaunchKernelGGL(rvsa_bwd5_mfma_kernel, grid, dim3(256), 0, s, (const bf16_t*)qkv, samp, (const bf16_t*)o, (const bf16_t*)dout, lse,
                                (bf16_t*)dqkv, dkv, dsamp, rel_part, tab_part, rel_h, rel_w, bias_table, g, scale);
         const int64_t N = Hp * Wp;
-        hipLaunchKernelGGL(rvsa_scatter_gemm_kernel, dim3((unsigned)(B * heads), (unsigned)((N + SCB - 1) / SCB)), dim3(256), 0, s, (const bf16_t*)dkv, samp, (bf16_t*)dqkv, g);
+        const int wcy = (int)((heads * HD / 4 + 63) / 64);
+        const int64_t extra = gwin ? B * g.nh * g.nw * wcy : 0;
+        hipLaunchKernelGGL(rvsa_scatter_gemm_kernel, dim3((unsigned)(B * heads + extra), (unsigned)((N + SCB - 1) / SCB)), dim3(256), 0, s, (const bf16_t*)dkv, samp, (bf16_t*)dqkv, g,
+                           dsamp, wsamp, avg, gwin, (int)(B * heads), wcy);
     } else {
         hipLaunchKernelGGL(rvsa_bwd4_mfma_kernel<1>, grid, dim3(256), 0, s, (const bf16_t*)qkv, samp, (const bf16_t*)o, (const bf16_t*)dout, lse,
                            (bf16_t*)dqkv, dkv, dsamp, rel_part, tab_part, rel_h, rel_w, bias_table, g, scale);
diff --git a/mtp_amd/csrc/common.h b/mtp_amd/csrc/common.h
--- a/mtp_amd/csrc/common.h
+++ b/mtp_amd/csrc/common.h
@@ -74,6 +74,33 @@
     *reinterpret_cast<uint4*>(p) = make_uint4(pack_bf16x2(o[0], o[1]), pack_bf16x2(o[2], o[3]), pack_bf16x2(o[4], o[5]), pack_bf16x2(o[6], o[7]));
 }
 
+__device__ __forceinline__ void rvsa_win_factor(const float* __restrict__ dsamp, const float* __restrict__ w, const float* __restrict__ avg, float* __restrict__ g,
+                                                int win, int cy, int C, int N, float4 (*part)[64]) {
+    const int lane = threadIdx.x & 63, q = threadIdx.x >> 6;
+    const int c4 = cy * 64 + lane;
+    const bool live = c4 < C / 4;
+    const float4 a = load4(avg + (int64_t)win * C + 4 * (live ? c4 : 0));
+    const float* __restrict__ drow = dsamp + (int64_t)win * N;
+    const int nq = (N + 3) / 4, n0 = q * nq, n1 = (n0 + nq) < N ? (n0 + nq) : N;
+    float4 d = make_float4(0, 0, 0, 0);
+    if (live) {
+#pragma unroll 10
+        for (int n = n0; n < n1; ++n) {
+            const float4 ww = load4(w + (int64_t)n * C + 4 * c4);
+            const float t = drow[n];
+            d.x += t * ww.x; d.y += t * ww.y; d.z += t * ww.z; d.w += t * ww.w;
+        }
+    }
+    part[q][lane] = d;
+    __syncthreads();
+    if (!live || q) return;
+    const float4 p0 = part[0][lane], p1 = part[1][lane], p2 = part[2][lane], p3 = part[3][lane];
+    d = make_float4((p0.x + p1.x) + (p2.x + p3.x), (p0.y + p1.y) + (p2.y + p3.y), (p0.z + p1.z) + (p2.z + p3.z), (p0.w + p1.w) + (p2.w + p3.w));
+    const float k = 1.0f / 49.0f;
+    *reinterpret_cast<float4*>(g + (int64_t)win * C + 4 * c4) =
+        make_float4(d.x * (a.x > 0 ? k : 0.01f * k), d.y * (a.y > 0 ? k : 0.01f * k), d.z * (a.z > 0 ? k : 0.01f * k), d.w * (a.w > 0 ? k : 0.01f * k));
+}
+
 __device__ __forceinline__ uint4 ldg16(const void* p) {
 #if defined(__HIP_DEVICE_COMPILE__)
     typedef __attribute__((ext_vector_type(4))) unsigned int u32x4_t;
diff --git a/mtp_amd/csrc/elementwise.hip b/mtp_amd/csrc/elementwise.hip
--- a/mtp_amd/csrc/elementwise.hip
+++ b/mtp_amd/csrc/elementwise.hip
@@ -1157,39 +1157,14 @@
 
 __global__ __launch_bounds__(256) void rvsa_sampling_bwd_win_kernel(const float* __restrict__ dsamp, const float* __restrict__ w, const float* __restrict__ avg,
                                                                    float* __restrict__ g, int C, int N) {
-    extern __shared__ __attribute__((aligned(16))) float ds[];
     __shared__ float4 part[4][64];
-    const int win = blockIdx.x;
-    const int lane = threadIdx.x & 63, q = threadIdx.x >> 6;
-    const int c4 = blockIdx.y * 64 + lane;
-    const bool live = c4 < C / 4;
-    for (int n = threadIdx.x; n < N; n += 256) ds[n] = dsamp[(int64_t)win * N + n];
-    __syncthreads();
-    const int nq = (N + 3) / 4, n0 = q * nq, n1 = (n0 + nq) < N ? (n0 + nq) : N;
-    float4 d = make_float4(0, 0, 0, 0);
-    if (live) {
-#pragma unroll 10
-        for (int n = n0; n < n1; ++n) {
-            const float4 ww = load4(w + (int64_t)n * C + 4 * c4);
-            const float t = ds[n];
-            d.x += t * ww.x; d.y += t * ww.y; d.z += t * ww.z; d.w += t * ww.w;
-        }
-    }
-    part[q][lane] = d;
-    __syncthreads();
-    if (!live || q) return;
-    const float4 p0 = part[0][lane], p1 = part[1][lane], p2 = part[2][lane], p3 = part[3][lane];
-    d = make_float4((p0.x + p1.x) + (p2.x + p3.x), (p0.y + p1.y) + (p2.y + p3.y), (p0.z + p1.z) + (p2.z + p3.z), (p0.w + p1.w) + (p2.w + p3.w));
-    const float4 a = load4(avg + (int64_t)win * C + 4 * c4);
-    const float k = 1.0f / 49.0f;
-    *reinterpret_cast<float4*>(g + (int64_t)win * C + 4 * c4) =
-        make_float4(d.x * (a.x > 0 ? k : 0.01f * k), d.y * (a.y > 0 ? k : 0.01f * k), d.z * (a.z > 0 ? k : 0.01f * k), d.w * (a.w > 0 ? k : 0.01f * k));
+    rvsa_win_factor(dsamp, w, avg, g, (int)blockIdx.x, (int)blockIdx.y, C, N, part);
 }
 
 extern "C" int mtp_rvsa_sampling_bwd_win(const float* dsamp, const float* w, const float* avg, float* g, int64_t windows, int64_t C, int64_t N, mtp_stream_t stream) {
     if (!dsamp || !w || !avg || !g || windows <= 0 || C <= 0 || (C % 4) || N <= 0 || N > 4096) return MTP_ERR_ARG;
     const dim3 grid((unsigned)windows, (unsigned)((C / 4 + 63) / 64)), block(256);
-    hipLaunchKernelGGL(rvsa_sampling_bwd_win_kernel, grid, block, sizeof(float) * (size_t)N, (hipStream_t)stream, dsamp, w, avg, g, (int)C, (int)N);
+    hipLaunchKernelGGL(rvsa_sampling_bwd_win_kernel, grid, block, 0, (hipStream_t)stream, dsamp, w, avg, g, (int)C, (int)N);
     return mtp_launch_status();
 }
 
diff --git a/mtp_amd/csrc/gemm.hip b/mtp_amd/csrc/gemm.hip
--- a/mtp_amd/csrc/gemm.hip
+++ b/mtp_amd/csrc/gemm.hip
@@ -493,7 +493,7 @@
             float s = 0.f;
 #pragma unroll
             for (int r = 0; r < 16; ++r) s += red[r * BM + tid];
-            if (m0 + tid < p.M) atomicAdd(p.colsum + m0 + tid, s);
+            if (m0 + tid < p.M) atomicAdd(p.colsum + (p.bias_mod > 0 ? (m0 + tid) % p.bias_mod : m0 + tid), s);
         }
     }
     epilogue<float, MTP_EPI_BIAS, 4>(p, acc, m0 + wm * 64, n0 + wn * 64, lane);
@@ -604,8 +604,13 @@
     dim3 grid(tiles_m * k.tiles_n, split), block(NT_THREADS);
     const bool full = (a->K % (8 * E) == 0) && (a->M % BM == 0) && (a->N % BN == 0);
     const bool tr = sizeof(T) == 2 && !(a->variant & 16) && (full || ((a->K % 64 == 0) && (a->M % 8 == 0) && (a->N % 8 == 0) && a->M >= 8 && a->N >= 8 && !(a->variant & 32768)));
+    if (a->colsum && a->bias_mod < 0) return MTP_ERR_ARG;
     if (a->colsum && !tr) {
-        rc = mtp_colsum_acc(a->A, a->in_dtype, a->lda, a->colsum, a->K, a->M, stream);
+        if (a->bias_mod > 0) {
+            if (a->lda != a->M || (a->M % a->bias_mod)) return MTP_ERR_UNSUPPORTED;
+            rc = mtp_colsum_acc(a->A, a->in_dtype, a->bias_mod, a->colsum, a->K * (a->M / a->bias_mod), a->bias_mod, stream);
+        } else
+            rc = mtp_colsum_acc(a->A, a->in_dtype, a->lda, a->colsum, a->K, a->M, stream);
         if (rc) return rc;
     }
     if (tr) {
diff --git a/mtp_amd/csrc/gemm_tn_p8.hip b/mtp_amd/csrc/gemm_tn_p8.hip
--- a/mtp_amd/csrc/gemm_tn_p8.hip
+++ b/mtp_amd/csrc/gemm_tn_p8.hip
@@ -17,7 +17,7 @@
     int tile0, tiles_m, tiles_n;
     int splits;
     int kchunk;
-    int pad_;
+    int cmod;
 };
 struct TnGroup {
     TnProb p[TN_MAX_PROBLEMS];
@@ -210,7 +210,8 @@
             float s = 0.f;
 #pragma unroll 8
             for (int r = 0; r < 32; ++r) s += red[(h * 32 + r) * 128 + x];
-            if (m0 + h * 128 + x < q.M) atomicAdd(q.colsum + m0 + h * 128 + x, s);
+            const int m = m0 + h * 128 + x;
+            if (m < q.M) atomicAdd(q.colsum + (q.cmod > 0 ? m % q.cmod : m), s);
         }
         __syncthreads();
     }
@@ -271,6 +272,8 @@
         if (a.workspace && splits > 1) return MTP_ERR_UNSUPPORTED;
         if (a.workspace && (a.workspace_bytes < 4 || ((uintptr_t)a.workspace & 3))) return MTP_ERR_ARG;
         q.sqn = (float*)a.workspace;
+        if (a.bias_mod < 0 || a.bias_mod > INT32_MAX) return MTP_ERR_ARG;
+        q.cmod = a.colsum ? (int)a.bias_mod : 0;
         q.M = (int)a.M; q.N = (int)a.N; q.K = (int)a.K;
         q.lda = (int)a.lda; q.ldb = (int)a.ldb; q.ldc = (int)a.ldc;
         q.tiles_m = (int)((a.M + P8_BM - 1) / P8_BM); q.tiles_n = (int)((a.N + P8_BN - 1) / P8_BN);
diff --git a/mtp_amd/engine.py b/mtp_amd/engine.py
--- a/mtp_amd/engine.py
+++ b/mtp_amd/engine.py
@@ -122,6 +122,7 @@
     wgrad_side_stream = True
     wgrad_max_jobs = 8
     wgrad_keep = 2
+    fuse_win_factor = True
 
     def _wgrad_stream(self):
         if not self.wgrad_side_stream:
@@ -148,10 +149,6 @@
 
     def _e(self, *shape, dtype=None):
         return torch.empty(*shape, device=self.dev, dtype=dtype or self.act)
-
-    @staticmethod
-    def _colsum(dy, out):
-        return ops.colsum(dy, out, accumulate=True)
 
     def _ln_bwd(self, *args, **kw):
         return ops.layernorm_bwd(*args, accumulate=True, defer=self._ln_parts, **kw)
@@ -245,15 +242,20 @@
                norm_ok=not ls)
         do = ops.gemm_nt(dx1_act, b.wprojT, self._e(T, C))
         dqkv = self._e(T, 3 * C)
+        win_add = None
         if b.window:
             nh, nw = ops.rvsa_windows(Hp, Wp)
             R = B * nh * nw
             H = self.heads
             dsamp = self._e(R, 5 * H, dtype=F32)
+            win_add = self._e(*s["avg"].shape, dtype=F32)
             ops.rvsa_attn_bwd(s["qkv"], s["samp"], s["o"], do, s["lse"], dqkv, dsamp,
                               P[pre + "attn.rel_pos_h"], P[pre + "attn.rel_pos_w"], P[pre + "attn.relative_position_bias_table"],
                               G[pre + "attn.rel_pos_h"], G[pre + "attn.rel_pos_w"], G[pre + "attn.relative_position_bias_table"],
-                              B, Hp, Wp, H, self.scale, accumulate=True, defer=self._ln_parts)
+                              B, Hp, Wp, H, self.scale, accumulate=True, defer=self._ln_parts,
+                              win=(b.wsamp, s["avg"], win_add) if self.fuse_win_factor else None)
+            if not self.fuse_win_factor:
+                ops.rvsa_sampling_bwd_win(dsamp, b.wsamp, s["avg"], win_add)
             names = ("sampling_offsets", "sampling_scales", "sampling_angles")
             self._sl_jobs.append((s["pooled"], dsamp, [G[pre + "attn.%s.2.weight" % n].view(-1, C) for n in names],
                                   [G[pre + "attn.%s.2.bias" % n] for n in names]))
@@ -266,9 +268,6 @@
             ops.full_attn_bwd(s["qkv"], s["o"], do, s["lse"], dqkv, rel_h, rel_w, drel_h, drel_w, B, Hp, Wp, self.heads, self.scale,
                               accumulate=True, defer=self._ln_parts)
         wq.add(dqkv, s["ln1"], G[pre + "attn.qkv.weight"], G[pre + "attn.qkv.bias"])
-        win_add = None
-        if b.window:
-            win_add = ops.rvsa_sampling_bwd_win(dsamp, b.wsamp, s["avg"], self._e(*s["avg"].shape, dtype=F32))
         dln1 = ops.gemm_nt(dqkv, b.wqkvT, self._e(T, C))
         dx0, dx0_act = self._e(T, C, dtype=F32), self._e(T, C)
         self._ln_bwd(dln1, s["x"], s["mean1"], s["rstd1"], P[pre + "norm1.weight"], dx0, G[pre + "norm1.weight"], G[pre + "norm1.bias"],
@@ -377,9 +376,9 @@
             fctx = dict(t0=t0, y1=y1, mean=mean, rstd=rstd, g1=g1, t1=t1, tap3=taps[3])
         return feats, fctx
 
-    def _convt_wgrad(self, dy, x, gw):
+    def _convt_wgrad(self, dy, x, gw, gb):
         dwg = self._e(dy.shape[1], x.shape[1], dtype=F32)
-        self._wq.add(dy, x, dwg, after=lambda: ops.convt_unpack_grad(dwg, gw), norm_of=gw)
+        self._wq.add(dy, x, dwg, colsum=gb, colsum_mod=gb.numel(), after=lambda: ops.convt_unpack_grad(dwg, gw), norm_of=gw)
 
     def _fpn_bwd(self, dfeats, fctx, B, Hp, Wp, G):
         P, C, T, act = self.P, self.C, B * Hp * Wp, self.act
@@ -393,8 +392,7 @@
             H2, W2, H4, W4 = Hp // 2, Wp // 2, Hp // 4, Wp // 4
             if dfeats[0] is not None:
                 dz = ops.nchw_to_tokens(as_in(dfeats[0]), self._e(4 * T, C), B, Hp, Wp, 1)
-                self._convt_wgrad(dz.view(T, 4 * C), fctx["t0"], G["fpn1.0.weight"])
-                self._colsum(dz, G["fpn1.0.bias"])
+                self._convt_wgrad(dz.view(T, 4 * C), fctx["t0"], G["fpn1.0.weight"], G["fpn1.0.bias"])
                 out[0] = ops.gemm_nt(dz.view(T, 4 * C), self._fpn["fpn1.0"][1], self._e(T, C, dtype=F32))
             if dfeats[1] is not None:
                 out[1] = ops.nchw_to_tokens(as_in(dfeats[1]), self._e(T, C, dtype=F32), B, Hp, Wp, 0)
@@ -409,19 +407,16 @@
 
         if dfeats[0] is not None:
             dy2 = ops.nchw_to_tokens(as_in(dfeats[0]), self._e(16 * T, C), B, Hp, Wp, 2)
-            self._convt_wgrad(dy2.view(4 * T, 4 * C), fctx["g1"], G["fpn1.3.weight"])
-            self._colsum(dy2, G["fpn1.3.bias"])
+            self._convt_wgrad(dy2.view(4 * T, 4 * C), fctx["g1"], G["fpn1.3.weight"], G["fpn1.3.bias"])
             dg1 = ops.gemm_nt(dy2.view(4 * T, 4 * C), self._fpn["fpn1.3"][1], self._e(4 * T, C))
             dy1 = self._e(4 * T, C)
             self._ln_bwd(dg1, fctx["y1"].view(4 * T, C), fctx["mean"], fctx["rstd"], P["fpn1.1.ln.weight"], dy1,
                               G["fpn1.1.ln.weight"], G["fpn1.1.ln.bias"], beta=P["fpn1.1.ln.bias"], gelu=True)
-            self._convt_wgrad(dy1.view(T, 4 * C), fctx["t0"], G["fpn1.0.weight"])
-            self._colsum(dy1, G["fpn1.0.bias"])
+            self._convt_wgrad(dy1.view(T, 4 * C), fctx["t0"], G["fpn1.0.weight"], G["fpn1.0.bias"])
             out[0] = ops.gemm_nt(dy1.view(T, 4 * C), self._fpn["fpn1.0"][1], self._e(T, C, dtype=F32))
         if dfeats[1] is not None:
             dz = ops.nchw_to_tokens(as_in(dfeats[1]), self._e(4 * T, C), B, Hp, Wp, 1)
-            self._convt_wgrad(dz.view(T, 4 * C), fctx["t1"], G["fpn2.0.weight"])
-            self._colsum(dz, G["fpn2.0.bias"])
+            self._convt_wgrad(dz.view(T, 4 * C), fctx["t1"], G["fpn2.0.weight"], G["fpn2.0.bias"])
             out[1] = ops.gemm_nt(dz.view(T, 4 * C), self._fpn["fpn2.0"][1], self._e(T, C, dtype=F32))
         if dfeats[2] is not None:
             out[2] = ops.nchw_to_tokens(as_in(dfeats[2]), self._e(T, C, dtype=F32), B, Hp, Wp, 0)
diff --git a/mtp_amd/ops.py b/mtp_amd/ops.py
--- a/mtp_amd/ops.py
+++ b/mtp_amd/ops.py
@@ -96,7 +96,7 @@
     return -(-k_tiles // per)
 
 
-def gemm_tn(a, b, out, split_k=None, use_workspace=True, variant=0, colsum=None, defer=None, m=None):
+def gemm_tn(a, b, out, split_k=None, use_workspace=True, variant=0, colsum=None, defer=None, m=None, colsum_mod=0):
     K, M = a.shape
     lda = M
     if m is not None:
@@ -106,8 +106,8 @@
     assert b.shape[0] == K and out.dtype == torch.float32 and out.numel() == M * N and a.dtype == b.dtype
     g = GemmArgs()
     if colsum is not None:
-        assert colsum.dtype == torch.float32 and colsum.numel() == M and colsum.is_contiguous()
-        g.colsum = _p(colsum)
+        assert colsum.dtype == torch.float32 and colsum.numel() == (colsum_mod or M) and colsum.is_contiguous()
+        g.colsum, g.bias_mod = _p(colsum), colsum_mod
     g.A, g.B, g.C = _p(a), _p(b), _p(out)
     g.M, g.N, g.K = M, N, K
     g.lda, g.ldb, g.ldc = lda, N, N
@@ -189,14 +189,14 @@
         self.after = []
         self.sqn, self.covered = None, []
 
-    def add(self, dy, x, dw, colsum=None, after=None, norm_of=None, norm_ok=True):
+    def add(self, dy, x, dw, colsum=None, after=None, norm_of=None, norm_ok=True, colsum_mod=0):
         K, M = dy.shape
         N = x.shape[1]
         t = grouped_tiles(M, N)
         fits = (K * M * 2 < (1 << 32) and K * N * 2 < (1 << 32) and dy.data_ptr() % 16 == 0 and x.data_ptr() % 16 == 0 and dw.data_ptr() % 16 == 0
                 and dy.is_contiguous() and x.is_contiguous())
         if t == 0 or K % 128 or dy.dtype != torch.bfloat16 or x.dtype != torch.bfloat16 or not fits:
-            gemm_tn(dy, x, dw, colsum=colsum)
+            gemm_tn(dy, x, dw, colsum=colsum, colsum_mod=colsum_mod)
             if after is not None:
                 after()
             return False
@@ -204,7 +204,7 @@
         splits = grouped_splits(K, t)
         part = _scratch((splits, M, N), dw.device, torch.float32) if splits > 1 else None
         use_sqn = self.sqn is not None and splits == 1 and norm_ok
-        self.jobs.append((dy, x, dw, colsum, splits, part, use_sqn))
+        self.jobs.append((dy, x, dw, colsum, splits, part, use_sqn, colsum_mod))
         if use_sqn:
             self.covered.append(dw if norm_of is None else norm_of)
         if after is not None:
@@ -243,7 +243,7 @@
         while self.jobs:
             chunk, self.jobs = self.jobs[:MAX_GROUPED], self.jobs[MAX_GROUPED:]
             arr = (GemmArgs * len(chunk))()
-            for g, (dy, x, dw, cs, splits, part, use_sqn) in zip(arr, chunk):
+            for g, (dy, x, dw, cs, splits, part, use_sqn, cmod) in zip(arr, chunk):
                 K, M = dy.shape
                 N = x.shape[1]
                 g.A, g.B, g.C = _p(dy), _p(x), _p(dw)
@@ -255,8 +255,8 @@
                 if use_sqn:
                     g.workspace, g.workspace_bytes = _p(self.sqn), 4
                 if cs is not None:
-                    assert cs.dtype == torch.float32 and cs.numel() == M and cs.is_contiguous()
-                    g.colsum = _p(cs)
+                    assert cs.dtype == torch.float32 and cs.numel() == (cmod or M) and cs.is_contiguous()
+                    g.colsum, g.bias_mod = _p(cs), cmod
             check(lib().mtp_gemm_tn_grouped(arr, len(chunk), _s()), "mtp_gemm_tn_grouped")
         after, self.after = self.after, []
         for fn in after:
@@ -668,7 +668,8 @@
     return o, lse
 
 
-def rvsa_attn_bwd(qkv, samp, o, dout, lse, dqkv, dsamp, rel_h, rel_w, table, drel_h, drel_w, dtable, B, Hp, Wp, heads, scale, accumulate=False, defer=None):
+def rvsa_attn_bwd(qkv, samp, o, dout, lse, dqkv, dsamp, rel_h, rel_w, table, drel_h, drel_w, dtable, B, Hp, Wp, heads, scale, accumulate=False, defer=None,
+                  win=None):
     hd = qkv.shape[1] // (3 * heads)
     T, C3 = qkv.shape
     Cc = C3 // 3
@@ -678,8 +679,15 @@
     dkv = _scratch((T, 2 * Cc), dev, torch.float32)
     rel_part = _scratch((nblk, 26 * hd), dev, torch.float32)
     tab_part = _scratch((B * nh * nw, heads * 169), dev, torch.float32)
-    check(lib().mtp_rvsa_attn_bwd(_p(qkv), _f32(samp), _p(o), _p(dout), _f32(lse), _p(dqkv), _p(dkv), _f32(dsamp), _p(rel_part), _p(tab_part),
-                                  _dt(qkv), _f32(rel_h), _f32(rel_w), _f32(table), B, Hp, Wp, heads, hd, scale, _s()), "mtp_rvsa_attn_bwd")
+    if win is not None:
+        w, avg, g = win
+        assert tuple(w.shape) == (5 * heads, Cc) and tuple(avg.shape) == (B * nh * nw, Cc) and g.shape == avg.shape
+        check(lib().mtp_rvsa_attn_bwd_win(_p(qkv), _f32(samp), _p(o), _p(dout), _f32(lse), _p(dqkv), _p(dkv), _f32(dsamp), _p(rel_part), _p(tab_part),
+                                          _dt(qkv), _f32(rel_h), _f32(rel_w), _f32(table), B, Hp, Wp, heads, hd, scale, _f32(w), _f32(avg), _f32(g), _s()),
+              "mtp_rvsa_attn_bwd_win")
+    else:
+        check(lib().mtp_rvsa_attn_bwd(_p(qkv), _f32(samp), _p(o), _p(dout), _f32(lse), _p(dqkv), _p(dkv), _f32(dsamp), _p(rel_part), _p(tab_part),
+                                      _dt(qkv), _f32(rel_h), _f32(rel_w), _f32(table), B, Hp, Wp, heads, hd, scale, _s()), "mtp_rvsa_attn_bwd")
     if defer is not None and _adjacent(drel_h, drel_w) and drel_h.numel() == 13 * hd:
         defer.append((rel_part, drel_h, accumulate))
         defer.append((tab_part, dtable, accumulate, (heads, 169)))
```

Result: no change. 1904 images/sec (median of 6 runs) (+0.6%).
